# jamesfer/datafusion-parallelism

Measured on AMD Instinct MI355X. Metric: probe Mrows/s + build ms, 10^8-row int64 inner join; 1/2/4/8 GPUs, higher is better.
Workload: dtype int64; 1 GPU; C2: 10^8-probe x 10^7-build int64 inner equi-join, uniform keys; build_rows=10000000, probe_rows=100000000, matches=49999816, parallelism=single-gpu

## Files before the change

### datafusion-parallelism_amd/csrc/hj_api.cpp

```cpp
#include <hip/hip_runtime.h>
#include <math.h>
#include <stdint.h>
#include <stdio.h>
#include <stdlib.h>
#include <string.h>

#include <algorithm>
#include <atomic>
#include <chrono>
#include <condition_variable>
#include <deque>
#include <map>
#include <mutex>
#include <string>
#include <thread>
#include <tuple>
#include <unordered_map>
#include <vector>

#include "../../include/hj.h"
#include "hj_device.h"
#include "hj_host.h"
#include "hj_launch.h"

using namespace dfp;

struct MultiTable;

namespace {

thread_local std::string g_err;

hj_status fail(hj_status st, const std::string& msg) {
    g_err = msg;
    return st;
}

#define HIP_TRY(expr)                                                                    \
    do {                                                                                 \
        hipError_t e_ = (expr);                                                          \
        if (e_ != hipSuccess)                                                            \
            return fail(HJ_ERR_HIP, std::string(#expr ": ") + hipGetErrorString(e_));    \
    } while (0)

struct ThreadStreams {
    std::unordered_map<int, hipStream_t> m;
    ~ThreadStreams() {
        for (auto& kv : m) (void)hipStreamDestroy(kv.second);
    }
};
thread_local ThreadStreams g_streams;

hipStream_t thread_stream(int dev) {
    auto it = g_streams.m.find(dev);
    if (it != g_streams.m.end()) return it->second;
    hipStream_t s = nullptr;
    if (hipStreamCreateWithFlags(&s, hipStreamNonBlocking) != hipSuccess) return nullptr;
    g_streams.m[dev] = s;
    return s;
}

struct BuildResources {
    hipStream_t stream = nullptr;
    hipEvent_t ev0 = nullptr, ev1 = nullptr;
    hipEvent_t evp = nullptr;
    int64_t* h_minmax = nullptr;
    int64_t* d_mbox = nullptr;
    int64_t mb_seq = 0;
};
std::mutex g_pool_mu;
std::unordered_map<int, std::vector<BuildResources>> g_pool;

int ev_scope() {
    static const int v = [] {
        const char* e = getenv("DFP_HJ_EV_SCOPE");
        return e ? atoi(e) : 0;
    }();
    return v;
}
unsigned probe_ev_flags() { return hipEventDisableTiming | (ev_scope() >= 1 ? hipEventReleaseToDevice : 0u); }
unsigned build_ev_flags() { return ev_scope() >= 2 ? hipEventReleaseToDevice : hipEventDefault; }

bool acquire_resources(int dev, BuildResources* r) {
    {
        std::lock_guard<std::mutex> g(g_pool_mu);
        auto& v = g_pool[dev];
        if (!v.empty()) {
            *r = v.back();
            v.pop_back();
            return true;
        }
    }
    return hipStreamCreateWithFlags(&r->stream, hipStreamNonBlocking) == hipSuccess &&
           hipEventCreateWithFlags(&r->ev0, build_ev_flags()) == hipSuccess &&
           hipEventCreateWithFlags(&r->ev1, build_ev_flags()) == hipSuccess &&
           hipEventCreateWithFlags(&r->evp, probe_ev_flags()) == hipSuccess &&
           hipHostMalloc((void**)&r->h_minmax, 4 * sizeof(int64_t), hipHostMallocCoherent | hipHostMallocMapped) ==
               hipSuccess &&
           hipHostGetDevicePointer((void**)&r->d_mbox, r->h_minmax, 0) == hipSuccess;
}

void release_resources(int dev, const BuildResources& r) {
    std::lock_guard<std::mutex> g(g_pool_mu);
    g_pool[dev].push_back(r);
}

struct DevCache {
    std::mutex mu;
    std::map<uint64_t, std::vector<void*>> bins;
    std::unordered_map<void*, size_t> cls;
    size_t cached_bytes = 0;
};
DevCache g_cache;

size_t size_class(size_t bytes) {
    if (bytes <= 4096) return 4096;
    if (bytes <= (1u << 20)) {
        size_t c = 4096;
        while (c < bytes) c <<= 1;
        return c;
    }
    const size_t step = bytes <= (256u << 20) ? (2u << 20) : (32u << 20);
    return (bytes + step - 1) / step * step;
}

constexpr size_t kBestFitMin = size_t(64) << 20;

void* cache_alloc(int dev, size_t bytes, hipError_t* err) {
    const size_t c = size_class(bytes);
    const uint64_t key = ((uint64_t)dev << 48) | c;
    {
        std::lock_guard<std::mutex> g(g_cache.mu);
        auto it = g_cache.bins.find(key);
        if ((it == g_cache.bins.end() || it->second.empty()) && c >= kBestFitMin) {
            for (it = g_cache.bins.lower_bound(key);
                 it != g_cache.bins.end() && (it->first >> 48) == (uint64_t)dev &&
                 (it->first & ((1ull << 48) - 1)) <= c + c / 4;
                 ++it)
                if (!it->second.empty()) break;
            if (it != g_cache.bins.end() && ((it->first >> 48) != (uint64_t)dev ||
                                             (it->first & ((1ull << 48) - 1)) > c + c / 4))
                it = g_cache.bins.end();
        }
        if (it != g_cache.bins.end() && !it->second.empty()) {
            void* p = it->second.back();
            it->second.pop_back();
            const size_t bc = (size_t)(it->first & ((1ull << 48) - 1));
            g_cache.cached_bytes -= bc;
            g_cache.cls[p] = bc;
            *err = hipSuccess;
            return p;
        }
    }
    void* p = nullptr;
    static const bool alog = [] {
        const char* e = getenv("DFP_HJ_ALLOC_LOG");
        return e != nullptr && e[0] == '1';
    }();
    if (alog) fprintf(stderr, "[dfp alloc] miss dev %d bytes %zu class %zu cached %zu\n", dev, bytes, c, g_cache.cached_bytes);
    *err = hipMalloc(&p, c);
    if (*err != hipSuccess) {
        (void)hipGetLastError();
        std::lock_guard<std::mutex> g(g_cache.mu);
        if (alog) fprintf(stderr, "[dfp alloc] hipMalloc %zu failed with %zu cached bytes\n", c, g_cache.cached_bytes);
        for (auto it = g_cache.bins.lower_bound(key); it != g_cache.bins.end() && (it->first >> 48) == (uint64_t)dev;
             ++it) {
            if (it->second.empty()) continue;
            void* q = it->second.back();
            it->second.pop_back();
            (void)hipFree(q);
            g_cache.cached_bytes -= (size_t)(it->first & ((1ull << 48) - 1));
            *err = hipMalloc(&p, c);
            if (*err == hipSuccess) {
                if (alog) fprintf(stderr, "[dfp alloc] released one cached block of %zu bytes: ok\n",
                                  (size_t)(it->first & ((1ull << 48) - 1)));
                g_cache.cls[p] = c;
                return p;
            }
            (void)hipGetLastError();
            break;
        }
        size_t freed = 0;
        for (;;) {
            auto lo = g_cache.bins.lower_bound((uint64_t)dev << 48);
            auto hi = g_cache.bins.lower_bound((uint64_t)(dev + 1) << 48);
            auto big = g_cache.bins.end();
            for (auto it = hi; it != lo;) {
                --it;
                if (!it->second.empty()) {
                    big = it;
                    break;
                }
            }
            if (big == g_cache.bins.end()) break;
            void* q = big->second.back();
            big->second.pop_back();
            (void)hipFree(q);
            const size_t qc = (size_t)(big->first & ((1ull << 48) - 1));
            g_cache.cached_bytes -= qc;
            freed += qc;
            if (freed >= c) {
                *err = hipMalloc(&p, c);
                if (*err == hipSuccess) break;
                (void)hipGetLastError();
            }
        }
        if (*err != hipSuccess) *err = hipMalloc(&p, c);
        if (alog) fprintf(stderr, "[dfp alloc] released %zu bytes: %s\n", freed, *err == hipSuccess ? "ok" : "failed");
        if (*err == hipSuccess) {
            g_cache.cls[p] = c;
            return p;
        }
    }
    if (*err != hipSuccess) return nullptr;
    std::lock_guard<std::mutex> g(g_cache.mu);
    g_cache.cls[p] = c;
    return p;
}

void cache_free(int dev, void* p, size_t bytes) {
    if (p == nullptr) return;
    std::lock_guard<std::mutex> g(g_cache.mu);
    size_t c = size_class(bytes);
    auto it = g_cache.cls.find(p);
    if (it != g_cache.cls.end()) {
        c = it->second;
        g_cache.cls.erase(it);
    }
    g_cache.bins[((uint64_t)dev << 48) | c].push_back(p);
    g_cache.cached_bytes += c;
}

int device_count() {
    int n = 0;
    if (hipGetDeviceCount(&n) != hipSuccess) return 0;
    return n;
}

bool is_device_ptr(const void* p) {
    if (p == nullptr) return true;
    hipPointerAttribute_t a;
    if (hipPointerGetAttributes(&a, p) != hipSuccess) {
        (void)hipGetLastError();
        return false;
    }
    return a.type == hipMemoryTypeDevice || a.type == hipMemoryTypeManaged;
}

constexpr double kDefaultLoadFactor = 0.5;

std::atomic<int> g_build_mode{-1};
int build_mode_raw() {
    int m = g_build_mode.load(std::memory_order_relaxed);
    if (m < 0) {
        const char* e = getenv("DFP_HJ_DENSE");
        m = (e && e[0] == '0') ? 1 : 0;
        const char* f = getenv("DFP_HJ_FRAG_BUILD");
        if (m == 0 && f && f[0] == '0') m = 2;
        g_build_mode.store(m, std::memory_order_relaxed);
    }
    return m;
}
int build_mode() { return build_mode_raw() == 1 ? 1 : 0; }
bool frag_build_mode() { return build_mode_raw() == 0; }
std::atomic<int64_t> g_budget{-1};
int64_t device_budget() {
    int64_t b = g_budget.load(std::memory_order_relaxed);
    if (b < 0) {
        const char* e = getenv("DFP_HJ_DEVICE_BUDGET_BYTES");
        b = e ? std::max<int64_t>(0, atoll(e)) : 0;
        int64_t unset = -1;
        g_budget.compare_exchange_strong(unset, b, std::memory_order_relaxed);
        b = g_budget.load(std::memory_order_relaxed);
    }
    return b;
}
bool spec_build_on() {
    static const bool v = [] {
        const char* e = getenv("DFP_HJ_SPEC_BUILD");
        return !(e != nullptr && e[0] == '0');
    }();
    return v;
}
double load_factor() {
    const char* e = getenv("DFP_HJ_LOAD_FACTOR");
    double lf = e ? atof(e) : kDefaultLoadFactor;
    if (!(lf > 0.05 && lf <= 0.95)) lf = kDefaultLoadFactor;
    return lf;
}

struct HostSeg {
    const void* keys = nullptr;
    const uint8_t* valid = nullptr;
    int64_t voff = 0;
    const uint64_t* ids = nullptr;
    int64_t n = 0;
    std::vector<void*> owned;
    hipEvent_t ready = nullptr;
};

}

struct hj_table {
    int device = 0;
    int parallelism = 1;
    hj_key_type kt = HJ_INT64;
    int key_bytes = 8;

    std::mutex mu;
    std::condition_variable cv;
    std::vector<std::vector<HostSeg>> parts;
    std::vector<char> finished;
    int arrived = 0;
    bool built = false;
    bool sync_finish = false;
    mutable std::mutex probe_mu;
    mutable std::vector<std::pair<hipStream_t, hipEvent_t>> probe_evs;
    hj_status build_st = HJ_OK;
    std::string build_err;
    bool has_ids = false, has_no_ids = false;
    bool ids_u31 = true;

    std::vector<int64_t> part_off;
    int64_t total_rows = 0;

    Bucket* tbl = nullptr;
    uint32_t nb = 0, clog2 = 10, nchunks = 0;
    uint32_t* dup_rows = nullptr;
    BuildCounters* ctr = nullptr;
    bool wrapped = false;
    uint64_t* row_ids = nullptr;
    uint32_t* dense = nullptr;
    bool packed = false;
    int64_t dmin = 0;
    uint64_t drange = 0;
    bool has_range = false;
    bool force_dense = false;
    int64_t range_lo = 0, range_hi = 0;
    bool has_base = false;
    int64_t key_base = 0;
    BuildResources res;
    hipStream_t bstream = nullptr;
    hipStream_t app_stream = nullptr;
    int app_streams = 0;
    int64_t build_ns = 0;
    std::vector<std::pair<void*, size_t>> allocs;
    std::vector<std::pair<void*, size_t>> scratch;
    MultiTable* multi = nullptr;
    std::vector<std::tuple<int, void*, size_t>> multi_bufs;
    int64_t live_bytes = 0, peak_bytes = 0;
    std::vector<hj_table*> owned_tables;
    hipEvent_t ext_ev0 = nullptr;
    std::atomic<bool> spec_pending{false};
    std::mutex spec_mu;
    int64_t spec_seq = 0;
    uint32_t spec_cap = 0;
    const int64_t* spec_mm = nullptr;
    std::vector<Segment> spec_segs;
    bool mm_known = false;
    int64_t mm_lo = 0, mm_hi = 0;
};

namespace dfp {
namespace host {
hj_status set_error(hj_status st, const std::string& msg) { return fail(st, msg); }
void* dev_block(int dev, size_t bytes) {
    hipError_t e;
    return cache_alloc(dev, bytes ? bytes : 64, &e);
}
void free_block(int dev, void* p, size_t bytes) { cache_free(dev, p, bytes ? bytes : 64); }
void table_adopt_block(hj_table* t, int dev, void* p, size_t bytes) {
    t->multi_bufs.emplace_back(dev, p, bytes ? bytes : 64);
}
void table_adopt_table(hj_table* t, hj_table* other) { t->owned_tables.push_back(other); }
void table_set_start_event(hj_table* t, hipEvent_t ev) {
    if (t->ext_ev0) (void)hipEventDestroy(t->ext_ev0);
    t->ext_ev0 = ev;
    t->build_ns = -1;
}
}
}

namespace {

hipError_t wait_mailbox(int64_t* mm, int64_t seq, const int64_t* d_minmax, hipStream_t s) {
    for (uint32_t i = 1;; ++i) {
        if (__atomic_load_n(&mm[2], __ATOMIC_ACQUIRE) == seq) return hipSuccess;
        if ((i & 4095) == 0) {
            const hipError_t q = hipStreamQuery(s);
            if (q == hipErrorNotReady) continue;
            if (q != hipSuccess) return q;
            if (__atomic_load_n(&mm[2], __ATOMIC_ACQUIRE) == seq) return hipSuccess;
            return hipMemcpy(mm, d_minmax, 2 * sizeof(int64_t), hipMemcpyDeviceToHost);
        }
        __builtin_ia32_pause();
    }
}

hj_status dev_alloc(hj_table* t, std::vector<std::pair<void*, size_t>>& list, void** p, size_t bytes) {
    if (bytes == 0) bytes = 64;
    const int64_t budget = device_budget();
    if (budget > 0 && t->live_bytes + (int64_t)bytes > budget)
        return fail(HJ_ERR_OOM, "device budget: this build needs more than " + std::to_string(budget) +
                                    " bytes of one device (DFP_HJ_DEVICE_BUDGET_BYTES / hj_set_device_budget); "
                                    "shard it over several GPUs (hj_build_begin_multi, radix plan)");
    hipError_t e;
    *p = cache_alloc(t->device, bytes, &e);
    if (*p == nullptr) return fail(HJ_ERR_OOM, std::string("device allocation: ") + hipGetErrorString(e));
    list.emplace_back(*p, bytes);
    t->live_bytes += (int64_t)bytes;
    t->peak_bytes = std::max(t->peak_bytes, t->live_bytes);
    return HJ_OK;
}

void free_list(hj_table* t, std::vector<std::pair<void*, size_t>>& list) {
    for (auto& pb : list) {
        cache_free(t->device, pb.first, pb.second);
        t->live_bytes -= (int64_t)pb.second;
    }
    list.clear();
}

hipDeviceProp_t* device_props(int dev) {
    static std::mutex mu;
    static std::unordered_map<int, hipDeviceProp_t> cache;
    std::lock_guard<std::mutex> g(mu);
    auto it = cache.find(dev);
    if (it == cache.end()) {
        hipDeviceProp_t p;
        if (hipGetDeviceProperties(&p, dev) != hipSuccess) return nullptr;
        it = cache.emplace(dev, p).first;
    }
    return &it->second;
}

hj_status build_attempt(hj_table* t, const std::vector<Segment>& segs, double lf, bool* retry) {
    *retry = false;
    const int64_t total = t->total_rows;
    hj_status st;
    void* p;
    hipStream_t s = t->bstream;
    Segment* d_segs;
    BuildCounters* ctr;
    int64_t* d_minmax;
    if ((st = dev_alloc(t, t->scratch, &p, sizeof(Segment) * std::max<size_t>(segs.size(), 1))) != HJ_OK) return st;
    d_segs = (Segment*)p;
    if ((st = dev_alloc(t, t->allocs, &p, sizeof(BuildCounters))) != HJ_OK) return st;
    ctr = (BuildCounters*)p;
    t->ctr = ctr;
    if ((st = dev_alloc(t, t->scratch, &p, (2 + 2 * kMinmaxMaxBlocks) * sizeof(int64_t))) != HJ_OK) return st;
    d_minmax = (int64_t*)p;
    const bool need_range = total > 0 && build_mode() == 0 && !t->has_range;
    const bool minmax = need_range && !t->mm_known;
    const bool by_arg = minmax && segs.size() <= (size_t)kArgSegs;
    if (!by_arg) {
        if (!segs.empty())
            HIP_TRY(hipMemcpyAsync(d_segs, segs.data(), sizeof(Segment) * segs.size(), hipMemcpyHostToDevice, s));
        HIP_TRY(hipMemsetAsync(ctr, 0, sizeof(BuildCounters), s));
    }

    std::vector<int64_t> seg_n(segs.size());
    for (size_t i = 0; i < segs.size(); ++i) seg_n[i] = segs[i].n;
    const int64_t ftiles = frag_build_tiles(seg_n.data(), (int)segs.size());
    const bool packed_ok = (uint64_t)(2 * total + 2) < (1ull << 27);
    const uint32_t spec_cap =
        (uint32_t)std::min<uint64_t>(kMaxLevel1Bins, (kDenseFactor * (uint64_t)total + kDenseBlockValues - 1) /
                                                         kDenseBlockValues);
    const ChunkGeom spec_g{0, 0, spec_cap << kDenseBlockShift, kDenseShift, 0, 1, packed_ok ? 1 : 0};
    const bool spec = minmax && spec_build_on() && !t->has_base && !t->force_dense && t->multi == nullptr &&
                      device_budget() <= 0 && frag_build_mode() && spec_cap > 0 && frag_build_ok(spec_g, ftiles);
    ChunkGeom g{};
    bool dense = false;
    if (need_range || (t->has_range && total > 0 && (build_mode() == 0 || t->force_dense))) {
        int64_t mm[2] = {t->range_lo, t->range_hi};
        if (t->mm_known) {
            mm[0] = t->mm_lo;
            mm[1] = t->mm_hi;
        }
        if (minmax) {
            int64_t* mb = t->res.h_minmax;
            const int64_t seq = ++t->res.mb_seq;
            HIP_TRY(launch_key_minmax(t->key_bytes, segs.data(), d_segs, (int)segs.size(), by_arg ? ctr : nullptr,
                                      total, d_minmax, t->res.d_mbox, seq, s));
            if (spec) {
                t->spec_seq = seq;
                t->spec_cap = spec_cap;
                t->spec_mm = d_minmax;
                t->spec_segs = segs;
                mm[0] = 1;
                mm[1] = 0;
            } else {
                HIP_TRY(wait_mailbox(mb, seq, d_minmax, s));
                mm[0] = mb[0];
                mm[1] = mb[1];
            }
        }
        if (spec) {
            dense = true;
            g = spec_g;
            t->dmin = 0;
            t->drange = 0;
        } else if (mm[0] <= mm[1]) {
            const uint64_t range = (uint64_t)mm[1] - (uint64_t)mm[0] + 1;
            const uint64_t nch = (range + (1u << kDenseShift) - 1) >> kDenseShift;
            if (range != 0 && (range <= kDenseFactor * (uint64_t)total || t->force_dense) &&
                nch <= (uint64_t)kMaxChunks) {
                dense = true;
                g = ChunkGeom{0, 0, (uint32_t)nch, kDenseShift, mm[0], 1, packed_ok ? 1 : 0};
                t->dmin = mm[0];
                t->drange = range;
            }
        }
    }
    if (!dense && t->has_base && total > 0)
        return fail(HJ_ERR_INVALID, "hj_build_key_base: the build keys do not make a direct-addressed table "
                                    "(key range > 8 x rows); build from int64 keys instead");
    if (!dense) {
        const double want = (double)total / (kSlots * lf);
        uint32_t clog2 = 9;
        uint64_t nchunks = (uint64_t)(want / (1u << clog2)) + 1;
        while (nchunks > (uint64_t)kMaxChunks && clog2 < 11) {
            ++clog2;
            nchunks = (uint64_t)(want / (1u << clog2)) + 1;
        }
        if (nchunks > (uint64_t)kMaxChunks) {
            const double full = (double)kMaxChunks * (1u << clog2) * kSlots;
            if ((double)total / full > 0.8)
                return fail(HJ_ERR_INVALID, "build side too large for one device table; shard it (hj_radix_partition)");
            nchunks = kMaxChunks;
        }
        g = ChunkGeom{(uint32_t)(nchunks << clog2), clog2, (uint32_t)nchunks, 0, 0, 0, 0};
        t->dmin = 0;
        t->drange = 0;
    }
    t->clog2 = g.clog2;
    t->nchunks = g.nchunks;
    t->packed = g.packed != 0;
    t->nb = g.nb;
    const uint64_t nchunks = g.nchunks;
    const bool frag = dense && total > 0 && frag_build_mode() && frag_build_ok(g, ftiles);
    const int64_t hftiles = frag_build_tiles(seg_n.data(), (int)segs.size(), hashed_build_tile_log());
    const bool hfrag = !dense && total > 0 && build_mode_raw() != 2 && hashed_frag_ok(g, hftiles);
    hipDeviceProp_t* prop0 = device_props(t->device);
    const int64_t ntiles = build_tiles(total, prop0 ? prop0->multiProcessorCount : 256);
    const int64_t tile_rows = build_tile_rows(total, ntiles);
    const int64_t hlen = (int64_t)(nchunks + 1) * ntiles;

    t->tbl = nullptr;
    t->dense = nullptr;
    if (dense) {
        const uint64_t dchunks = dense_one_level((uint32_t)nchunks)
                                     ? (uint64_t)dense_blocks((uint32_t)nchunks) << kDenseBlockShift
                                     : nchunks;
        if ((st = dev_alloc(t, t->allocs, &p, sizeof(uint32_t) * (size_t)(dchunks << kDenseShift))) != HJ_OK)
            return st;
        t->dense = (uint32_t*)p;
    } else {
        if ((st = dev_alloc(t, t->allocs, &p, (size_t)(t->nb + 1) * sizeof(Bucket))) != HJ_OK) return st;
        t->tbl = (Bucket*)p;
    }
    if ((st = dev_alloc(t, t->allocs, &p, sizeof(uint32_t) * (size_t)(2 * total + 2))) != HJ_OK) return st;
    t->dup_rows = (uint32_t*)p;
    const bool ids_as_rows = t->has_ids && t->ids_u31;
    if (t->has_ids && !ids_as_rows) {
        if ((st = dev_alloc(t, t->allocs, &p, sizeof(uint64_t) * (size_t)std::max<int64_t>(total, 1))) != HJ_OK)
            return st;
        t->row_ids = (uint64_t*)p;
    }
    if (frag || hfrag) {
        void* fscr;
        uint32_t* d_tb;
        uint64_t* ids32 = nullptr;
        BigSeg* fbig;
        const int64_t fbytes =
            frag ? frag_build_scratch_bytes(g, ftiles, total) : hashed_frag_scratch_bytes(g, hftiles, total);
        if ((st = dev_alloc(t, t->scratch, &fscr, (size_t)fbytes)) != HJ_OK) return st;
        if ((st = dev_alloc(t, t->scratch, &p, sizeof(uint32_t) * (size_t)(frag ? ftiles : hftiles))) != HJ_OK)
            return st;
        d_tb = (uint32_t*)p;
        if ((st = dev_alloc(t, t->scratch, &p, sizeof(BigSeg) * (size_t)(total / (kSmallSeg + 1) + 2))) != HJ_OK)
            return st;
        fbig = (BigSeg*)p;
        if (t->has_ids) {
            uint64_t* dst = t->row_ids;
            if (ids_as_rows && segs.size() == 1) {
                ids32 = const_cast<uint64_t*>(segs[0].ids);
                dst = nullptr;
            } else if (ids_as_rows) {
                if ((st = dev_alloc(t, t->scratch, &p, sizeof(uint64_t) * (size_t)total)) != HJ_OK) return st;
                dst = ids32 = (uint64_t*)p;
            }
            if (dst != nullptr)
                for (const Segment& sg : segs)
                    HIP_TRY(hipMemcpyAsync(dst + sg.row_base, sg.ids, sizeof(uint64_t) * (size_t)sg.n,
                                           hipMemcpyDefault, s));
        }
        hipDeviceProp_t* prop = device_props(t->device);
        const int cus = prop ? prop->multiProcessorCount : 256;
        if (frag) {
            HIP_TRY(launch_build_frag(t->key_bytes, segs.data(), (int)segs.size(), g, ftiles, fscr, d_tb, ids32,
                                      t->dense, t->dup_rows, fbig, ctr, d_segs, total, ids_as_rows, cus,
                                      spec ? SpecGeo{(const long long*)d_minmax, (uint64_t)total, spec_cap}
                                           : SpecGeo{nullptr, 0, 0},
                                      s));
            if (spec) t->spec_pending.store(true, std::memory_order_release);
            return HJ_OK;
        }
        HIP_TRY(launch_build_hashed_frag(t->key_bytes, segs.data(), (int)segs.size(), g, hftiles, fscr, d_tb, ids32,
                                         t->tbl, t->dup_rows, fbig, ctr, d_segs, total, ids_as_rows, cus, s));
        BuildCounters hc;
        HIP_TRY(hipMemcpyAsync(&hc, ctr, sizeof(hc), hipMemcpyDeviceToHost, s));
        HIP_TRY(hipStreamSynchronize(s));
        free_list(t, t->scratch);
        if (hc.err & ~3ull)
            return fail(HJ_ERR_HIP, "hashed build: internal check failed (error bits " + std::to_string(hc.err) + ")");
        if (hc.err) {
            *retry = true;
            free_list(t, t->allocs);
            t->row_ids = nullptr;
        }
        return HJ_OK;
    }
    uint32_t *hist, *hist1, *srows, *trows;
    unsigned long long *skeys, *tkeys;
    BigSeg* big;
    void* scan;
    if ((st = dev_alloc(t, t->scratch, &p, sizeof(uint32_t) * (size_t)std::max<int64_t>(hlen, 1))) != HJ_OK) return st;
    hist = (uint32_t*)p;
    if ((st = dev_alloc(t, t->scratch, &p, sizeof(uint32_t) * (size_t)std::max<int64_t>(kMaxLevel1Bins * ntiles, 1))) !=
        HJ_OK)
        return st;
    hist1 = (uint32_t*)p;
    uint32_t* chunk_starts;
    if ((st = dev_alloc(t, t->scratch, &p, sizeof(uint32_t) * (size_t)(nchunks + 2))) != HJ_OK) return st;
    chunk_starts = (uint32_t*)p;
    if ((st = dev_alloc(t, t->scratch, &p, (size_t)scan_scratch_bytes(std::max<int64_t>(hlen, kMaxLevel1Bins * ntiles)))) !=
        HJ_OK)
        return st;
    scan = p;
    if ((st = dev_alloc(t, t->scratch, &p, 8 * (size_t)std::max<int64_t>(total, 1))) != HJ_OK) return st;
    skeys = (unsigned long long*)p;
    if ((st = dev_alloc(t, t->scratch, &p, 4 * (size_t)std::max<int64_t>(total, 1))) != HJ_OK) return st;
    srows = (uint32_t*)p;
    if ((st = dev_alloc(t, t->scratch, &p, 8 * (size_t)std::max<int64_t>(total, 1))) != HJ_OK) return st;
    tkeys = (unsigned long long*)p;
    if ((st = dev_alloc(t, t->scratch, &p, 4 * (size_t)std::max<int64_t>(total, 1))) != HJ_OK) return st;
    trows = (uint32_t*)p;
    if ((st = dev_alloc(t, t->scratch, &p, sizeof(BigSeg) * (size_t)(total / (kSmallSeg + 1) + 2))) != HJ_OK)
        return st;
    big = (BigSeg*)p;

    if (total == 0) HIP_TRY(hipMemsetAsync(t->tbl, 0, (size_t)(t->nb + 1) * sizeof(Bucket), s));
    hipDeviceProp_t* prop = device_props(t->device);
    const int cus = prop ? prop->multiProcessorCount : 256;
    HIP_TRY(launch_build(t->key_bytes, d_segs, (int)segs.size(), total, g, hist, hist1, chunk_starts, ntiles, tile_rows,
                         scan, tkeys, trows, skeys, srows, t->row_ids, ids_as_rows, t->tbl, t->dense, t->dup_rows, big,
                         ctr, cus, s));
    if (dense) return HJ_OK;
    BuildCounters hc;
    HIP_TRY(hipMemcpyAsync(&hc, ctr, sizeof(hc), hipMemcpyDeviceToHost, s));
    HIP_TRY(hipStreamSynchronize(s));
    free_list(t, t->scratch);
    if (hc.err) {
        *retry = true;
        free_list(t, t->allocs);
        t->row_ids = nullptr;
    }
    return HJ_OK;
}

hj_status run_multi_build_entry(hj_table* t, const std::vector<Segment>& segs, const std::vector<HostSeg*>& hsegs);

hj_status build_attempts(hj_table* t, const std::vector<Segment>& segs) {
    double lf = load_factor();
    for (int attempt = 0;; ++attempt) {
        bool retry = false;
        hj_status st = build_attempt(t, segs, lf, &retry);
        if (st != HJ_OK) return st;
        if (!retry) return HJ_OK;
        if (attempt >= 4) return fail(HJ_ERR_INVALID, "build: a table chunk overflowed at every load factor");
        lf *= 0.5;
        HIP_TRY(hipEventRecord(t->res.ev0, t->bstream));
    }
}

hj_status ensure_geometry(const hj_table* ct) {
    hj_table* t = const_cast<hj_table*>(ct);
    auto settled = [t]() { return t->build_st == HJ_OK ? HJ_OK : fail(t->build_st, t->build_err); };
    if (!t->spec_pending.load(std::memory_order_acquire)) return settled();
    std::lock_guard<std::mutex> g(t->spec_mu);
    if (!t->spec_pending.load(std::memory_order_relaxed)) return settled();
    HIP_TRY(hipSetDevice(t->device));
    int64_t* mb = t->res.h_minmax;
    HIP_TRY(wait_mailbox(mb, t->spec_seq, t->spec_mm, t->bstream));
    const int64_t mn = mb[0], mx = mb[1];
    if (spec_dense_blocks(mn, mx, (uint64_t)t->total_rows, t->spec_cap) != 0) {
        const uint64_t range = (uint64_t)mx - (uint64_t)mn + 1;
        t->dmin = mn;
        t->drange = range;
        t->nchunks = (uint32_t)((range + (1u << kDenseShift) - 1) >> kDenseShift);
        t->spec_pending.store(false, std::memory_order_release);
        return HJ_OK;
    }
    HIP_TRY(hipStreamSynchronize(t->bstream));
    HIP_TRY(hipEventRecord(t->res.ev0, t->bstream));
    free_list(t, t->allocs);
    free_list(t, t->scratch);
    t->dense = nullptr;
    t->tbl = nullptr;
    t->dup_rows = nullptr;
    t->row_ids = nullptr;
    t->ctr = nullptr;
    t->mm_known = true;
    t->mm_lo = mn;
    t->mm_hi = mx;
    hj_status st = build_attempts(t, t->spec_segs);
    if (st == HJ_OK && hipEventRecord(t->res.ev1, t->bstream) != hipSuccess)
        st = fail(HJ_ERR_HIP, "hipEventRecord failed");
    t->build_ns = -1;
    if (st != HJ_OK) {
        (void)hipStreamSynchronize(t->bstream);
        t->build_st = st;
        t->build_err = g_err;
    }
    t->spec_pending.store(false, std::memory_order_release);
    return st;
}

struct Settler {
    std::mutex mu;
    std::condition_variable cv;
    std::deque<hj_table*> q;
    hj_table* busy = nullptr;
};
Settler& settler() {
    static Settler* s = [] {
        Settler* st = new Settler();
        std::thread([st] {
            for (;;) {
                hj_table* t;
                {
                    std::unique_lock<std::mutex> g(st->mu);
                    st->cv.wait(g, [st] { return !st->q.empty(); });
                    t = st->q.front();
                    st->q.pop_front();
                    st->busy = t;
                }
                (void)ensure_geometry(t);
                {
                    std::lock_guard<std::mutex> g(st->mu);
                    st->busy = nullptr;
                }
                st->cv.notify_all();
            }
        }).detach();
        return st;
    }();
    return *s;
}
bool settler_on() {
    static const bool v = [] {
        const char* e = getenv("DFP_HJ_SETTLE");
        return !(e && e[0] == '0');
    }();
    return v;
}
void settler_enqueue(hj_table* t) {
    Settler& st = settler();
    {
        std::lock_guard<std::mutex> g(st.mu);
        st.q.push_back(t);
    }
    st.cv.notify_all();
}
void settler_forget(hj_table* t) {
    if (!settler_on()) return;
    Settler& st = settler();
    std::unique_lock<std::mutex> g(st.mu);
    for (auto it = st.q.begin(); it != st.q.end();)
        it = *it == t ? st.q.erase(it) : it + 1;
    st.cv.wait(g, [&st, t] { return st.busy != t; });
}

hj_status run_build(hj_table* t) {
    HIP_TRY(hipSetDevice(t->device));
    std::vector<Segment> segs;
    std::vector<HostSeg*> hsegs;
    t->part_off.assign(t->parallelism, 0);
    int64_t row = 0;
    for (int p = 0; p < t->parallelism; ++p) {
        t->part_off[p] = row;
        for (auto& hs : t->parts[p]) {
            if (hs.n == 0) continue;
            segs.push_back(Segment{hs.keys, hs.valid, hs.voff, hs.ids, hs.n, row});
            hsegs.push_back(&hs);
            row += hs.n;
        }
    }
    t->total_rows = row;
    if (t->multi) return run_multi_build_entry(t, segs, hsegs);
    if (row > 0x7FFFFFF0ll) return fail(HJ_ERR_INVALID, "build side exceeds 2^31-16 rows on one device; shard it");
    if (t->has_ids && t->has_no_ids)
        return fail(HJ_ERR_INVALID, "explicit build ids must be given for every batch or none");
    t->bstream = t->app_streams == 1 ? t->app_stream : t->res.stream;
    hipStream_t s = t->bstream;
    for (int p = 0; p < t->parallelism; ++p)
        for (auto& hs : t->parts[p])
            if (hs.ready) HIP_TRY(hipStreamWaitEvent(s, hs.ready, 0));
    HIP_TRY(hipEventRecord(t->res.ev0, s));
    hj_status bst = build_attempts(t, segs);
    if (bst != HJ_OK) return bst;
    HIP_TRY(hipEventRecord(t->res.ev1, s));
    t->build_ns = -1;
    if (t->has_base) {
        if (t->dense != nullptr) t->dmin += t->key_base;
        t->kt = HJ_INT64;
        t->key_bytes = 8;
    }
    return HJ_OK;
}

int64_t build_time_ns(hj_table* t) {
    if (t->build_ns < 0) {
        float ms = 0;
        if (hipEventSynchronize(t->res.ev1) != hipSuccess ||
            hipEventElapsedTime(&ms, t->ext_ev0 ? t->ext_ev0 : t->res.ev0, t->res.ev1) != hipSuccess)
            return -1;
        t->build_ns = (int64_t)(ms * 1e6);
    }
    return t->build_ns;
}

hj_status wait_built(const hj_table* t, hipStream_t s) {
    if (s != t->bstream) HIP_TRY(hipStreamWaitEvent(s, t->res.ev1, 0));
    return HJ_OK;
}

hj_status check_table(const hj_table* t) {
    if (t == nullptr) return fail(HJ_ERR_INVALID, "null table");
    if (!t->built) return fail(HJ_ERR_INVALID, "table is not built: every partition must call hj_build_finish");
    if (t->build_st != HJ_OK) return fail(t->build_st, t->build_err);
    return ensure_geometry(t);
}

TableView view_of(const hj_table* t) {
    return TableView{t->tbl, t->dup_rows, t->row_ids, t->nb, t->clog2, t->dense, t->dmin, t->drange,
                     t->packed ? kPackedMask : kFullMask};
}

struct TmpInput {
    void* keys = nullptr;
    uint8_t* valid = nullptr;
    hipStream_t s = nullptr;
    ~TmpInput() {
        if (keys) (void)hipFreeAsync(keys, s);
        if (valid) (void)hipFreeAsync(valid, s);
    }
};

hj_status stage_input(int key_bytes, const void* keys, const uint8_t* valid, int64_t voff, int64_t n, uint32_t flags,
                      hipStream_t s, TmpInput& tmp, const void** dkeys, const uint8_t** dvalid, int64_t* dvoff) {
    if (flags & HJ_INPUT_DEVICE) {
        if (!is_device_ptr(keys) || !is_device_ptr(valid))
            return fail(HJ_ERR_INVALID, "HJ_INPUT_DEVICE given but a pointer is not device memory");
        *dkeys = keys;
        *dvalid = valid;
        *dvoff = voff;
        return HJ_OK;
    }
    tmp.s = s;
    if (n > 0) {
        HIP_TRY(hipMallocAsync(&tmp.keys, (size_t)n * key_bytes, s));
        HIP_TRY(hipMemcpyAsync(tmp.keys, keys, (size_t)n * key_bytes, hipMemcpyDefault, s));
    }
    *dkeys = tmp.keys;
    *dvalid = nullptr;
    *dvoff = 0;
    if (valid && n > 0) {
        const int64_t b0 = voff >> 3;
        const int64_t nbytes = ((voff & 7) + n + 7) >> 3;
        HIP_TRY(hipMallocAsync((void**)&tmp.valid, (size_t)nbytes, s));
        HIP_TRY(hipMemcpyAsync(tmp.valid, valid + b0, (size_t)nbytes, hipMemcpyDefault, s));
        *dvalid = tmp.valid;
        *dvoff = voff & 7;
    }
    return HJ_OK;
}

hj_status note_probe(const hj_table* t, hipStream_t s) {
    std::lock_guard<std::mutex> g(t->probe_mu);
    for (auto& se : t->probe_evs)
        if (se.first == s) {
            HIP_TRY(hipEventRecord(se.second, s));
            return HJ_OK;
        }
    hipEvent_t ev = t->res.evp;
    if (!t->probe_evs.empty()) HIP_TRY(hipEventCreateWithFlags(&ev, probe_ev_flags()));
    t->probe_evs.emplace_back(s, ev);
    HIP_TRY(hipEventRecord(ev, s));
    return HJ_OK;
}

hj_status check_probe_args(int64_t n, uint32_t pbase, int64_t cap, const void* ws) {
    if (n < 0 || n > 0xFFFFFFFFll) return fail(HJ_ERR_INVALID, "probe batch must have < 2^32 rows");
    if ((int64_t)pbase + n > 0x100000000ll) return fail(HJ_ERR_INVALID, "probe_base + rows exceeds 2^32");
    if (cap < 0) return fail(HJ_ERR_INVALID, "negative capacity");
    if (reinterpret_cast<uintptr_t>(ws) & 7) return fail(HJ_ERR_INVALID, "workspace must be 8-byte aligned");
    return HJ_OK;
}

hj_status probe_impl(const hj_table* t, const void* keys, const uint8_t* valid, int64_t voff,
                     const uint32_t* probe_ids, uint32_t pbase, int64_t n, uint64_t* out_b, uint32_t* out_p,
                     int64_t cap, int64_t* d_total, void* ws, hipStream_t s) {
    hj_status st = check_probe_args(n, pbase, cap, ws);
    if (st == HJ_OK) st = ensure_geometry(t);
    if (st != HJ_OK) return st;
    HIP_TRY(launch_probe(t->key_bytes, view_of(t), keys, valid, voff, probe_ids, pbase, n, out_b, out_p, cap, d_total, ws,
                         s != t->bstream ? t->res.ev1 : nullptr, s));
    return note_probe(t, s);
}

}

struct MultiTable {
    int plan = HJ_MULTI_AUTO;
    std::vector<int> devices;
    std::vector<hj_table*> shards;
    std::vector<hipStream_t> streams;
    std::mutex probe_mu;
    int64_t total_rows = 0;
    ~MultiTable() {
        for (size_t g = 0; g < shards.size(); ++g) hj_table_free(shards[g]);
        for (size_t g = 0; g < streams.size(); ++g) {
            (void)hipSetDevice(devices[g]);
            (void)hipStreamDestroy(streams[g]);
        }
    }
};

namespace {

int ptr_device(const void* p, int dflt) {
    hipPointerAttribute_t a;
    if (p == nullptr || hipPointerGetAttributes(&a, p) != hipSuccess) {
        (void)hipGetLastError();
        return dflt;
    }
    return (a.type == hipMemoryTypeDevice || a.type == hipMemoryTypeManaged) ? a.device : dflt;
}

void drain_multi(const MultiTable* m);
struct TmpBufs {
    std::vector<std::tuple<int, void*, size_t>> v;
    const MultiTable* m = nullptr;
    std::vector<std::pair<int, hipStream_t>> streams;
    ~TmpBufs() {
        if (m != nullptr) drain_multi(m);
        for (auto& ds : streams) {
            (void)hipSetDevice(ds.first);
            (void)hipStreamSynchronize(ds.second);
        }
        for (auto& b : v) cache_free(std::get<0>(b), std::get<1>(b), std::get<2>(b));
    }
    void* get(int dev, size_t bytes) {
        hipError_t e;
        (void)hipSetDevice(dev);
        void* p = cache_alloc(dev, bytes ? bytes : 64, &e);
        if (p) v.emplace_back(dev, p, bytes ? bytes : 64);
        return p;
    }
};

#define MT_ALLOC(var, type, dev, bytes)                                                   \
    type var = (type)tmp.get((dev), (bytes));                                             \
    if (var == nullptr) return fail(HJ_ERR_OOM, "multi-GPU table: device allocation failed")

hj_status sync_streams(const MultiTable* m) {
    for (size_t g = 0; g < m->streams.size(); ++g) {
        HIP_TRY(hipSetDevice(m->devices[g]));
        HIP_TRY(hipStreamSynchronize(m->streams[g]));
    }
    return HJ_OK;
}

void drain_multi(const MultiTable* m) {
    for (size_t g = 0; g < m->streams.size(); ++g) {
        (void)hipSetDevice(m->devices[g]);
        (void)hipStreamSynchronize(m->streams[g]);
    }
    for (const hj_table* sh : m->shards)
        if (sh != nullptr && sh->built && sh->build_st == HJ_OK) {
            (void)hipSetDevice(sh->device);
            (void)hipEventSynchronize(sh->res.ev1);
        }
}

bool force_stage() {
    const char* e = getenv("DFP_HJ_MULTI_STAGE");
    return e != nullptr && e[0] == '1';
}

int owner_of(int64_t key, int G) { return (int)(mix64((uint64_t)key) & (uint64_t)(G - 1)); }
// ... 257 lines not shown
            if (!P.ws) P.ws = tmp.get(dev, (size_t)hj_probe_workspace_bytes(P.n));
            if (!P.ob || !P.op || !P.dt || !P.ws) return fail(HJ_ERR_OOM, "multi-GPU probe: device allocation failed");
            st = P.ids ? hj_probe_async_ids(m->shards[g], P.k, P.v, P.voff, P.ids, P.n, P.ob, P.op, P.cap, P.dt, P.ws,
                                            m->streams[g])
                       : hj_probe_async_base(m->shards[g], P.k, P.v, P.voff, P.n, P.base, P.ob, P.op, P.cap, P.dt,
                                             P.ws, m->streams[g]);
            if (st != HJ_OK) return st;
            HIP_TRY(hipMemcpyAsync(&P.total, P.dt, 8, hipMemcpyDeviceToHost, m->streams[g]));
            again = true;
        }
        if (!again) break;
        if ((st = sync_streams(m)) != HJ_OK) return st;
    }
    int64_t total = 0;
    unsigned long long err = 0;
    for (auto& P : parts) {
        total += P.total;
        unsigned long long e = 0;
        HIP_TRY(hipMemcpy(&e, (char*)P.ws + 8, 8, hipMemcpyDeviceToHost));
        err |= e;
    }
    HIP_TRY(hipSetDevice(d));
    if (workspace) HIP_TRY(hipMemcpyAsync((char*)workspace + 8, &err, 8, hipMemcpyHostToDevice, s));
    if (m->plan == HJ_MULTI_BROADCAST) {
        int64_t at = 0;
        for (auto& P : parts) {
            const int64_t c = std::min<int64_t>(P.total, std::max<int64_t>(cap - at, 0));
            HIP_TRY(copy_to(out_b + at, P.ob, 8 * (size_t)c, s));
            HIP_TRY(copy_to(out_p + at, P.op, 4 * (size_t)c, s));
            at += P.total;
        }
    } else if (total > 0) {
        MT_ALLOC(cb, uint64_t*, d, 8 * (size_t)total);
        MT_ALLOC(cp, uint32_t*, d, 4 * (size_t)total);
        int64_t at = 0;
        for (auto& P : parts) {
            HIP_TRY(copy_to(cb + at, P.ob, 8 * (size_t)P.total, s));
            HIP_TRY(copy_to(cp + at, P.op, 4 * (size_t)P.total, s));
            at += P.total;
        }
        MT_ALLOC(mw, void*, d, (size_t)merge_pairs_workspace(n));
        HIP_TRY(launch_merge_pairs(cb, cp, total, n, out_b, out_p, cap, mw, s));
        if (probe_ids)
            HIP_TRY(launch_gather_fixed(probe_ids, nullptr, 0, 4, out_p, 4, std::min(total, cap), out_p, nullptr, s));
        else if (pbase)
            HIP_TRY(launch_add_u32(out_p, std::min(total, cap), pbase, s));
    }
    HIP_TRY(hipMemcpyAsync(d_total, &total, 8, hipMemcpyHostToDevice, s));
    HIP_TRY(hipStreamSynchronize(s));
    return HJ_OK;
}

}

namespace {
hj_status run_multi_build_entry(hj_table* t, const std::vector<Segment>& segs, const std::vector<HostSeg*>& hsegs) {
    return run_multi_build(t, segs, hsegs);
}
}

extern "C" {

const char* hj_last_error(void) { return g_err.c_str(); }

const char* hj_version(void) { return "dfp-hj 0.2 (gfx950)"; }

int hj_device_count(void) { return device_count(); }

hj_status hj_build_begin(int device, int parallelism, hj_key_type key_type, int64_t expected_rows, hj_table** out) {
    (void)expected_rows;
    if (out == nullptr) return fail(HJ_ERR_INVALID, "null out");
    *out = nullptr;
    if (parallelism < 1) return fail(HJ_ERR_INVALID, "parallelism must be >= 1");
    if (key_type != HJ_INT32 && key_type != HJ_INT64) return fail(HJ_ERR_INVALID, "unsupported key type");
    const int nd = device_count();
    if (nd == 0) return fail(HJ_ERR_NO_DEVICE, "no GPU visible: the HIP path cannot run (no CPU fallback)");
    if (device < 0 || device >= nd) return fail(HJ_ERR_INVALID, "bad device ordinal");
    HIP_TRY(hipSetDevice(device));
    hj_table* t = new hj_table();
    t->device = device;
    t->parallelism = parallelism;
    t->kt = key_type;
    t->key_bytes = key_type == HJ_INT64 ? 8 : 4;
    t->parts.resize(parallelism);
    t->finished.assign(parallelism, 0);
    if (!acquire_resources(device, &t->res)) {
        delete t;
        return fail(HJ_ERR_HIP, "stream/event creation failed");
    }
    static std::once_flag pool_once[64];
    if (device < 64)
        std::call_once(pool_once[device], [device] {
            hipMemPool_t pool;
            if (hipDeviceGetDefaultMemPool(&pool, device) == hipSuccess) {
                uint64_t thr = UINT64_MAX;
                (void)hipMemPoolSetAttribute(pool, hipMemPoolAttrReleaseThreshold, &thr);
            }
        });
    *out = t;
    return HJ_OK;
}

hj_status hj_build_begin_multi(int ngpu, const int* devices, int parallelism, hj_key_type key_type,
                               int64_t expected_rows, int plan, hj_table** out) {
    if (out == nullptr) return fail(HJ_ERR_INVALID, "null out");
    *out = nullptr;
    if (ngpu < 1 || ngpu > 64 || devices == nullptr) return fail(HJ_ERR_INVALID, "ngpu must be 1..64 with a device list");
    if (plan != HJ_MULTI_AUTO && plan != HJ_MULTI_BROADCAST && plan != HJ_MULTI_RADIX)
        return fail(HJ_ERR_INVALID, "unknown multi-GPU plan");
    if (plan == HJ_MULTI_RADIX && (ngpu & (ngpu - 1)))
        return fail(HJ_ERR_INVALID, "the radix plan shards over a power-of-two number of GPUs");
    const int nd = device_count();
    if (nd == 0) return fail(HJ_ERR_NO_DEVICE, "no GPU visible: the HIP path cannot run (no CPU fallback)");
    for (int g = 0; g < ngpu; ++g)
        if (devices[g] < 0 || devices[g] >= nd) return fail(HJ_ERR_INVALID, "bad device ordinal");
    hj_status st = hj_build_begin(devices[0], parallelism, key_type, expected_rows, out);
    if (st != HJ_OK) return st;
    hj_table* t = *out;
    MultiTable* m = new MultiTable();
    m->plan = plan;
    m->devices.assign(devices, devices + ngpu);
    for (int g = 0; g < ngpu; ++g) {
        hipStream_t s = nullptr;
        if (hipSetDevice(devices[g]) != hipSuccess || hipStreamCreateWithFlags(&s, hipStreamNonBlocking) != hipSuccess) {
            delete m;
            hj_table_free(t);
            *out = nullptr;
            return fail(HJ_ERR_HIP, "multi-GPU table: stream creation failed");
        }
        m->streams.push_back(s);
        for (int q = 0; q < ngpu; ++q)
            if (devices[q] != devices[g]) {
                (void)hipDeviceEnablePeerAccess(devices[q], 0);
                (void)hipGetLastError();
            }
    }
    (void)hipSetDevice(devices[0]);
    t->multi = m;
    return HJ_OK;
}

hj_status hj_build_append(hj_table* t, int partition, const void* keys, const uint8_t* validity,
                          int64_t validity_offset, const uint64_t* ids, int64_t n, uint32_t flags, void* stream) {
    if (t == nullptr) return fail(HJ_ERR_INVALID, "null table");
    if (partition < 0 || partition >= t->parallelism) return fail(HJ_ERR_INVALID, "bad partition");
    if (n < 0 || validity_offset < 0) return fail(HJ_ERR_INVALID, "negative length/offset");
    if (n > 0 && keys == nullptr) return fail(HJ_ERR_INVALID, "null keys");
    {
        std::lock_guard<std::mutex> g(t->mu);
        if (t->finished[partition])
            return fail(HJ_ERR_INVALID, "State already consumed for partition " + std::to_string(partition));
        if (n > 0) {
            if (ids) {
                t->has_ids = true;
                if (!(flags & HJ_IDS_U31)) t->ids_u31 = false;
            } else {
                t->has_no_ids = true;
            }
        }
    }
    HIP_TRY(hipSetDevice(t->device));
    HostSeg hs;
    hs.n = n;
    if (n == 0) return HJ_OK;
    {
        std::lock_guard<std::mutex> g(t->mu);
        if (t->app_streams == 0) {
            t->app_stream = (hipStream_t)stream;
            t->app_streams = 1;
        } else if (t->app_stream != (hipStream_t)stream) {
            t->app_streams = 2;
        }
    }
    hipStream_t s = (hipStream_t)stream;
    const bool dev_in = (flags & HJ_INPUT_DEVICE) != 0;
    if (dev_in && (!is_device_ptr(keys) || !is_device_ptr(validity) || !is_device_ptr(ids)))
        return fail(HJ_ERR_INVALID, "HJ_INPUT_DEVICE given but a pointer is not device memory");
    if (dev_in && (flags & HJ_BORROW)) {
        if (!(flags & HJ_BORROW_KEEP)) {
            std::lock_guard<std::mutex> g(t->mu);
            t->sync_finish = true;
        }
        HIP_TRY(hipEventCreateWithFlags(&hs.ready, hipEventDisableTiming));
        HIP_TRY(hipEventRecord(hs.ready, s));
        hs.keys = keys;
        hs.valid = validity;
        hs.voff = validity_offset;
        hs.ids = ids;
    } else {
        const int64_t staged = n * t->key_bytes + (validity ? (((validity_offset & 7) + n + 7) >> 3) : 0) +
                               (ids ? n * 8 : 0);
        {
            std::lock_guard<std::mutex> g(t->mu);
            const int64_t budget = device_budget();
            if (budget > 0 && t->live_bytes + staged > budget)
                return fail(HJ_ERR_OOM, "device budget: staging this build input exceeds " + std::to_string(budget) +
                                            " bytes of one device (DFP_HJ_DEVICE_BUDGET_BYTES); shard the build");
            t->live_bytes += staged;
            t->peak_bytes = std::max(t->peak_bytes, t->live_bytes);
        }
        void* dk = nullptr;
        HIP_TRY(hipMalloc(&dk, (size_t)n * t->key_bytes));
        hs.owned.push_back(dk);
        HIP_TRY(hipMemcpyAsync(dk, keys, (size_t)n * t->key_bytes, hipMemcpyDefault, s));
        hs.keys = dk;
        if (validity) {
            const int64_t b0 = validity_offset >> 3;
            const int64_t nbytes = ((validity_offset & 7) + n + 7) >> 3;
            void* dv = nullptr;
            HIP_TRY(hipMalloc(&dv, (size_t)nbytes));
            hs.owned.push_back(dv);
            HIP_TRY(hipMemcpyAsync(dv, validity + b0, (size_t)nbytes, hipMemcpyDefault, s));
            hs.valid = (const uint8_t*)dv;
            hs.voff = validity_offset & 7;
        }
        if (ids) {
            void* di = nullptr;
            HIP_TRY(hipMalloc(&di, (size_t)n * 8));
            hs.owned.push_back(di);
            HIP_TRY(hipMemcpyAsync(di, ids, (size_t)n * 8, hipMemcpyDefault, s));
            hs.ids = (const uint64_t*)di;
        }
        HIP_TRY(hipStreamSynchronize(s));
    }
    std::lock_guard<std::mutex> g(t->mu);
    t->parts[partition].push_back(std::move(hs));
    return HJ_OK;
}

hj_status hj_build_finish(hj_table* t, int partition) {
    if (t == nullptr) return fail(HJ_ERR_INVALID, "null table");
    if (partition < 0 || partition >= t->parallelism) return fail(HJ_ERR_INVALID, "bad partition");
    std::unique_lock<std::mutex> g(t->mu);
    if (t->finished[partition])
        return fail(HJ_ERR_INVALID, "State already consumed for partition " + std::to_string(partition));
    t->finished[partition] = 1;
    t->arrived++;
    if (t->arrived == t->parallelism) {
        hj_status st = run_build(t);
        if (st == HJ_OK && t->sync_finish) st = ensure_geometry(t);
        if (st != HJ_OK) (void)hipStreamSynchronize(t->bstream);
        if (st == HJ_OK && t->sync_finish && hipEventSynchronize(t->res.ev1) != hipSuccess)
            st = fail(HJ_ERR_HIP, "build failed on the device");
        t->build_st = st;
        t->build_err = st == HJ_OK ? "" : g_err;
        t->built = true;
        t->cv.notify_all();
        if (st == HJ_OK && t->spec_pending.load(std::memory_order_acquire) && settler_on()) settler_enqueue(t);
    } else {
        const char* e = getenv("DFP_HJ_BARRIER_TIMEOUT_S");
        const double secs = e ? atof(e) : 300.0;
        if (!t->cv.wait_for(g, std::chrono::duration<double>(secs), [t] { return t->built; }))
            return fail(HJ_ERR_INVALID, "Possible deadlock: partition " + std::to_string(partition) +
                                            " waited for the build barrier; every partition must call "
                                            "hj_build_finish concurrently");
    }
    if (t->build_st != HJ_OK) return fail(t->build_st, t->build_err);
    return HJ_OK;
}

hj_status hj_build_key_range(hj_table* t, int64_t key_lo, int64_t key_hi) {
    if (t == nullptr) return fail(HJ_ERR_INVALID, "null table");
    if (key_lo > key_hi) return fail(HJ_ERR_INVALID, "hj_build_key_range: key_lo > key_hi");
    if (t->key_bytes == 4 && (key_lo < INT32_MIN || key_hi > INT32_MAX))
        return fail(HJ_ERR_INVALID, "hj_build_key_range: outside the int32 key domain");
    std::lock_guard<std::mutex> g(t->mu);
    if (t->built || t->arrived > 0) return fail(HJ_ERR_INVALID, "hj_build_key_range: after the barrier started");
    t->has_range = true;
    t->range_lo = key_lo;
    t->range_hi = key_hi;
    return HJ_OK;
}

hj_status hj_build_dense(hj_table* t) {
    if (t == nullptr) return fail(HJ_ERR_INVALID, "null table");
    if (t->multi != nullptr) return fail(HJ_ERR_INVALID, "hj_build_dense: not for a multi-GPU table");
    std::lock_guard<std::mutex> g(t->mu);
    if (t->built || t->arrived > 0) return fail(HJ_ERR_INVALID, "hj_build_dense: after the barrier started");
    if (!t->has_range) return fail(HJ_ERR_INVALID, "hj_build_dense: needs hj_build_key_range first");
    if ((uint64_t)t->range_hi - (uint64_t)t->range_lo >= ((uint64_t)kMaxChunks << kDenseShift))
        return fail(HJ_ERR_INVALID, "hj_build_dense: key range beyond the direct-addressed layout");
    t->force_dense = true;
    return HJ_OK;
}

hj_status hj_build_key_base(hj_table* t, int64_t key_base) {
    if (t == nullptr) return fail(HJ_ERR_INVALID, "null table");
    if (t->multi != nullptr) return fail(HJ_ERR_INVALID, "hj_build_key_base: not for a multi-GPU table");
    if (t->kt != HJ_INT32) return fail(HJ_ERR_INVALID, "hj_build_key_base: the build keys must be int32 offsets");
    std::lock_guard<std::mutex> g(t->mu);
    if (t->built || t->arrived > 0) return fail(HJ_ERR_INVALID, "hj_build_key_base: after the barrier started");
    t->has_base = true;
    t->key_base = key_base;
    return HJ_OK;
}

hj_status hj_table_dense_piece(const hj_table* t, uint32_t** refs, uint64_t* nvalues, int64_t* key_min,
                               uint32_t** dup_rows, const uint64_t** dup_used, int* packed) {
    hj_status st = check_table(t);
    if (st != HJ_OK) return st;
    if (!refs || !nvalues || !key_min || !dup_rows || !dup_used || !packed) return fail(HJ_ERR_INVALID, "null out");
    if (t->multi != nullptr || t->dense == nullptr || t->ctr == nullptr || t->wrapped)
        return fail(HJ_ERR_INVALID, "hj_table_dense_piece: not a built direct-addressed single-device table");
    *refs = t->dense;
    *nvalues = t->drange;
    *key_min = t->dmin;
    *dup_rows = t->dup_rows;
    *dup_used = reinterpret_cast<const uint64_t*>(&t->ctr->dup_used);
    *packed = t->packed ? 1 : 0;
    return HJ_OK;
}

hj_status hj_table_dense_export(const hj_table* t, uint32_t* refs_dst, uint64_t v0, uint64_t n, uint32_t* dup_dst,
                                uint64_t dup_n, uint64_t* dup_used_dst, void* stream) {
    hj_status st = check_table(t);
    if (st != HJ_OK) return st;
    if (t->multi != nullptr || t->dense == nullptr || t->ctr == nullptr || t->wrapped)
        return fail(HJ_ERR_INVALID, "hj_table_dense_export: not a built direct-addressed single-device table");
    if (refs_dst != nullptr && (v0 > t->drange || n > t->drange - v0))
        return fail(HJ_ERR_INVALID, "hj_table_dense_export: refs range past the table's key range");
    if (dup_dst != nullptr && dup_n > (uint64_t)(2 * t->total_rows + 2))
        return fail(HJ_ERR_INVALID, "hj_table_dense_export: more segment words than the table holds");
    HIP_TRY(hipSetDevice(t->device));
    hipStream_t s = (hipStream_t)stream;
    if (s != t->bstream) HIP_TRY(hipStreamWaitEvent(s, t->res.ev1, 0));
    if (refs_dst != nullptr && n > 0)
        HIP_TRY(hipMemcpyAsync(refs_dst, t->dense + v0, n * sizeof(uint32_t), hipMemcpyDeviceToDevice, s));
    if (dup_dst != nullptr && dup_n > 0)
        HIP_TRY(hipMemcpyAsync(dup_dst, t->dup_rows, dup_n * sizeof(uint32_t), hipMemcpyDeviceToDevice, s));
    if (dup_used_dst != nullptr)
        HIP_TRY(hipMemcpyAsync(dup_used_dst, &t->ctr->dup_used, sizeof(uint64_t), hipMemcpyDeviceToDevice, s));
    return note_probe(t, s);
}

hj_status hj_table_wrap_dense(int device, hj_key_type probe_key_type, int64_t key_min, uint64_t nvalues,
                              const uint32_t* refs, const uint32_t* dup_rows, int packed, void* stream,
                              hj_table** out) {
    if (out == nullptr) return fail(HJ_ERR_INVALID, "null out");
    *out = nullptr;
    if (probe_key_type != HJ_INT32 && probe_key_type != HJ_INT64) return fail(HJ_ERR_INVALID, "unsupported key type");
    if (refs == nullptr || dup_rows == nullptr || nvalues == 0)
        return fail(HJ_ERR_INVALID, "hj_table_wrap_dense: null arrays or an empty key range");
    if (nvalues > ((uint64_t)kMaxChunks << kDenseShift))
        return fail(HJ_ERR_INVALID, "hj_table_wrap_dense: key range beyond the direct-addressed layout");
    const int nd = device_count();
    if (nd == 0) return fail(HJ_ERR_NO_DEVICE, "no GPU visible: the HIP path cannot run (no CPU fallback)");
    if (device < 0 || device >= nd) return fail(HJ_ERR_INVALID, "bad device ordinal");
    HIP_TRY(hipSetDevice(device));
    hj_table* t = new hj_table();
    t->device = device;
    t->kt = probe_key_type;
    t->key_bytes = probe_key_type == HJ_INT64 ? 8 : 4;
    t->parts.resize(1);
    t->finished.assign(1, 1);
    t->arrived = 1;
    if (!acquire_resources(device, &t->res)) {
        delete t;
        return fail(HJ_ERR_HIP, "stream/event creation failed");
    }
    t->wrapped = true;
    t->dense = const_cast<uint32_t*>(refs);
    t->dup_rows = const_cast<uint32_t*>(dup_rows);
    t->dmin = key_min;
    t->drange = nvalues;
    t->packed = packed != 0;
    t->bstream = (hipStream_t)stream;
    if (hipEventRecord(t->res.ev0, t->bstream) != hipSuccess || hipEventRecord(t->res.ev1, t->bstream) != hipSuccess) {
        release_resources(device, t->res);
        delete t;
        return fail(HJ_ERR_HIP, "hipEventRecord failed");
    }
    t->built = true;
    *out = t;
    return HJ_OK;
}

hj_status hj_dense_rebase_dups(uint32_t* refs, uint64_t n, uint32_t base, int packed, void* stream) {
    if (n > 0 && refs == nullptr) return fail(HJ_ERR_INVALID, "null refs");
    if (device_count() == 0) return fail(HJ_ERR_NO_DEVICE, "no GPU visible");
    const uint32_t mask = packed ? kPackedMask : kFullMask;
    if (base > mask) return fail(HJ_ERR_INVALID, "hj_dense_rebase_dups: base beyond the offset field");
    HIP_TRY(launch_dense_rebase(refs, n, base, mask, (hipStream_t)stream));
    return HJ_OK;
}

hj_status hj_build_partition_offset(const hj_table* t, int partition, int64_t* out) {
    hj_status st = check_table(t);
    if (st != HJ_OK) return st;
    if (partition < 0 || partition >= t->parallelism || out == nullptr) return fail(HJ_ERR_INVALID, "bad args");
    *out = t->part_off[partition];
    return HJ_OK;
}

hj_status hj_table_stats_get(const hj_table* t, hj_table_stats* out) {
    hj_status st = check_table(t);
    if (st != HJ_OK) return st;
    if (out == nullptr) return fail(HJ_ERR_INVALID, "null out");
    if (t->multi) {
        const MultiTable* m = t->multi;
        memset(out, 0, sizeof(*out));
        for (size_t g = 0; g < m->shards.size(); ++g) {
            hj_table_stats s;
            if ((st = hj_table_stats_get(m->shards[g], &s)) != HJ_OK) return st;
            if (m->plan == HJ_MULTI_BROADCAST && g > 0) {
                out->build_ns = std::max(out->build_ns, s.build_ns);
                continue;
            }
            out->inserted_rows += s.inserted_rows;
            out->distinct_keys += s.distinct_keys;
            out->dup_keys += s.dup_keys;
            out->dup_rows += s.dup_rows;
            out->max_key_rows = std::max(out->max_key_rows, s.max_key_rows);
            out->buckets += s.buckets;
            out->table_bytes += s.table_bytes;
            out->build_ns = std::max(out->build_ns, s.build_ns);
        }
        out->build_rows = t->total_rows;
        return HJ_OK;
    }
    HIP_TRY(hipSetDevice(t->device));
    hipStream_t s = thread_stream(t->device);
    unsigned long long* d = nullptr;
    HIP_TRY(hipMallocAsync((void**)&d, 4 * sizeof(unsigned long long), s));
    HIP_TRY(hipMemsetAsync(d, 0, 4 * sizeof(unsigned long long), s));
    if (wait_built(t, s) != HJ_OK) return HJ_ERR_HIP;
    HIP_TRY(launch_table_stats(view_of(t), d, s));
    unsigned long long h[4];
    HIP_TRY(hipMemcpyAsync(h, d, sizeof(h), hipMemcpyDeviceToHost, s));
    HIP_TRY(hipFreeAsync(d, s));
    HIP_TRY(hipStreamSynchronize(s));
    out->build_rows = t->total_rows;
    out->distinct_keys = (int64_t)h[0];
    out->dup_keys = (int64_t)h[1];
    out->dup_rows = (int64_t)h[2];
    out->max_key_rows = (int64_t)h[3];
    out->inserted_rows = (int64_t)h[0] - (int64_t)h[1] + (int64_t)h[2];
    out->buckets = t->dense ? 0 : t->nb;
    out->table_bytes = t->dense ? (int64_t)sizeof(uint32_t) * ((int64_t)t->nchunks << kDenseShift)
                                : (int64_t)(t->nb + 1) * (int64_t)sizeof(Bucket);
    out->build_ns = build_time_ns(const_cast<hj_table*>(t));
    return HJ_OK;
}

int64_t hj_table_build_ns(const hj_table* t) {
    if (t == nullptr || !t->built || t->build_st != HJ_OK) return -1;
    if (t->multi == nullptr && ensure_geometry(t) != HJ_OK) return -1;
    if (t->multi) {
        int64_t ns = 0;
        for (hj_table* sh : t->multi->shards) ns = std::max(ns, hj_table_build_ns(sh));
        return ns;
    }
    return build_time_ns(const_cast<hj_table*>(t));
}

int64_t hj_probe_workspace_bytes(int64_t n) { return probe_workspace(n); }

int hj_set_build_mode(int mode) {
    if (mode < 0 || mode > 2) return -1;
    const int old = build_mode_raw();
    g_build_mode.store(mode, std::memory_order_relaxed);
    return old;
}

int64_t hj_set_device_budget(int64_t bytes) {
    const int64_t old = device_budget();
    g_budget.store(bytes < 0 ? 0 : bytes, std::memory_order_relaxed);
    return old;
}

hj_status hj_table_device_bytes(const hj_table* t, int64_t* peak_per_device) {
    if (t == nullptr || peak_per_device == nullptr) return fail(HJ_ERR_INVALID, "null table/out");
    if (t->multi) {
        int64_t mx = 0;
        for (const hj_table* sh : t->multi->shards)
            if (sh != nullptr) mx = std::max(mx, sh->peak_bytes);
        *peak_per_device = mx;
        return HJ_OK;
    }
    *peak_per_device = t->peak_bytes;
    return HJ_OK;
}

int hj_set_probe_mode(int mode) {
    if (mode != 0 && mode != 3 && mode != 4) return -1;
    const int old = get_probe_mode();
    set_probe_mode(mode);
    return old;
}

int hj_set_probe_tile_log(int tile_log) {
    if (tile_log != 0 && tile_log != 14 && tile_log != 15) return -1;
    return set_probe_tile_log(tile_log);
}

hj_status hj_probe_async(const hj_table* t, const void* keys, const uint8_t* validity, int64_t validity_offset,
                         int64_t n, uint64_t* out_build, uint32_t* out_probe, int64_t capacity, int64_t* d_total,
                         void* workspace, void* stream) {
    hj_status st = check_table(t);
    if (st != HJ_OK) return st;
    if (d_total == nullptr || workspace == nullptr) return fail(HJ_ERR_INVALID, "null d_total/workspace");
    if (n > 0 && keys == nullptr) return fail(HJ_ERR_INVALID, "null keys");
    HIP_TRY(hipSetDevice(t->device));
    if (t->multi)
        return multi_probe(t, keys, validity, validity_offset, nullptr, 0, n, out_build, out_probe, capacity, d_total,
                           workspace, (hipStream_t)stream);
    return probe_impl(t, keys, validity, validity_offset, nullptr, 0, n, out_build, out_probe, capacity, d_total,
                      workspace, (hipStream_t)stream );
}

hj_status hj_probe_async_base(const hj_table* t, const void* keys, const uint8_t* validity, int64_t validity_offset,
                              int64_t n, uint32_t probe_base, uint64_t* out_build, uint32_t* out_probe,
                              int64_t capacity, int64_t* d_total, void* workspace, void* stream) {
    hj_status st = check_table(t);
    if (st != HJ_OK) return st;
    if (d_total == nullptr || workspace == nullptr) return fail(HJ_ERR_INVALID, "null d_total/workspace");
    if (n > 0 && keys == nullptr) return fail(HJ_ERR_INVALID, "null keys");
    HIP_TRY(hipSetDevice(t->device));
    if (t->multi)
        return multi_probe(t, keys, validity, validity_offset, nullptr, probe_base, n, out_build, out_probe, capacity,
                           d_total, workspace, (hipStream_t)stream);
    return probe_impl(t, keys, validity, validity_offset, nullptr, probe_base, n, out_build, out_probe, capacity,
                      d_total, workspace, (hipStream_t)stream);
}

hj_status hj_probe_async_ids(const hj_table* t, const void* keys, const uint8_t* validity, int64_t validity_offset,
                             const uint32_t* probe_ids, int64_t n, uint64_t* out_build, uint32_t* out_probe,
                             int64_t capacity, int64_t* d_total, void* workspace, void* stream) {
    hj_status st = check_table(t);
    if (st != HJ_OK) return st;
    if (d_total == nullptr || workspace == nullptr) return fail(HJ_ERR_INVALID, "null d_total/workspace");
    HIP_TRY(hipSetDevice(t->device));
    if (t->multi)
        return multi_probe(t, keys, validity, validity_offset, probe_ids, 0, n, out_build, out_probe, capacity,
                           d_total, workspace, (hipStream_t)stream);
    return probe_impl(t, keys, validity, validity_offset, probe_ids, 0, n, out_build, out_probe, capacity, d_total,
                      workspace, (hipStream_t)stream );
}


namespace {
uint64_t match_claim_bits(const hj_table* t) {
    return t->dense != nullptr ? t->drange : ((uint64_t)(2 * t->total_rows + 2) >> 3) + 1;
}
const char* const kMatchMulti = "the match probe is not defined for a multi-GPU table (probe its pairs instead)";
}

int64_t hj_probe_match_workspace_bytes(const hj_table* t, int64_t n) {
    if (check_table(t) != HJ_OK) return -1;
    if (t->multi) {
        (void)fail(HJ_ERR_INVALID, kMatchMulti);
        return -1;
    }
    if (check_probe_args(n, 0, 0, nullptr) != HJ_OK) return -1;
    return probe_match_workspace(match_claim_bits(t));
}

hj_status hj_probe_match(const hj_table* t, const void* keys, const uint8_t* validity, int64_t validity_offset,
                         int64_t n, uint8_t* out_bitmap, uint32_t* out_counts, uint8_t* build_flags, int64_t nflags,
                         int64_t* d_stats, void* workspace, void* stream) {
    hj_status st = check_table(t);
    if (st != HJ_OK) return st;
    if (t->multi) return fail(HJ_ERR_INVALID, kMatchMulti);
    if (workspace == nullptr) return fail(HJ_ERR_INVALID, "null workspace");
    if ((st = check_probe_args(n, 0, 0, workspace)) != HJ_OK) return st;
    if (n > 0 && keys == nullptr) return fail(HJ_ERR_INVALID, "null keys");
    if (nflags < 0 || (nflags > 0 && build_flags == nullptr)) return fail(HJ_ERR_INVALID, "bad build_flags / nflags");
    if (reinterpret_cast<uintptr_t>(out_bitmap) & 7) return fail(HJ_ERR_INVALID, "out_bitmap must be 8-byte aligned");
    if ((reinterpret_cast<uintptr_t>(out_counts) & 3) || (reinterpret_cast<uintptr_t>(d_stats) & 7))
        return fail(HJ_ERR_INVALID, "out_counts must be 4-byte and d_stats 8-byte aligned");
    HIP_TRY(hipSetDevice(t->device));
    hipStream_t s = (hipStream_t)stream;
    if ((st = wait_built(t, s)) != HJ_OK) return st;
    HIP_TRY(launch_probe_match(t->key_bytes, view_of(t), keys, validity, validity_offset, n, out_bitmap, out_counts,
                               build_flags, nflags, d_stats, workspace, match_claim_bits(t), s));
    return note_probe(t, s);
}

hj_status hj_probe(const hj_table* t, const void* keys, const uint8_t* validity, int64_t validity_offset, int64_t n,
                   uint32_t flags, void* stream, hj_pairs* out) {
    hj_status st = check_table(t);
    if (st != HJ_OK) return st;
    if (out == nullptr) return fail(HJ_ERR_INVALID, "null out");
    memset(out, 0, sizeof(*out));
    if (n < 0) return fail(HJ_ERR_INVALID, "negative length");
    if (n > 0 && keys == nullptr) return fail(HJ_ERR_INVALID, "null keys");
    HIP_TRY(hipSetDevice(t->device));
    hipStream_t s = (hipStream_t)stream;
    TmpInput tmp;
    const void* dk;
    const uint8_t* dv;
    int64_t dvo;
    if ((st = stage_input(t->key_bytes, keys, validity, validity_offset, n, flags, s, tmp, &dk, &dv, &dvo)) != HJ_OK)
        return st;
    void* ws = nullptr;
    int64_t* d_total = nullptr;
    HIP_TRY(hipMallocAsync(&ws, (size_t)hj_probe_workspace_bytes(n), s));
    HIP_TRY(hipMallocAsync((void**)&d_total, sizeof(int64_t), s));
    int64_t cap = std::max<int64_t>(n, 1);
    uint64_t* ob = nullptr;
    uint32_t* op = nullptr;
    int64_t total = 0;
    for (int attempt = 0; attempt < 2; ++attempt) {
        HIP_TRY(hipMalloc((void**)&ob, (size_t)cap * 8));
        HIP_TRY(hipMalloc((void**)&op, (size_t)cap * 4));
        if (t->multi) st = multi_probe(t, dk, dv, dvo, nullptr, 0, n, ob, op, cap, d_total, ws, s);
        else st = probe_impl(t, dk, dv, dvo, nullptr, 0, n, ob, op, cap, d_total, ws, s);
        if (st != HJ_OK) break;
        uint64_t werr = 0;
        HIP_TRY(hipMemcpyAsync(&total, d_total, 8, hipMemcpyDeviceToHost, s));
        HIP_TRY(hipMemcpyAsync(&werr, (char*)ws + 8, 8, hipMemcpyDeviceToHost, s));
        HIP_TRY(hipStreamSynchronize(s));
        if (werr != 0) {
            st = fail(HJ_ERR_HIP, "probe: tile look-back gave up (results invalid)");
            break;
        }
        if (total <= cap) break;
        (void)hipFree(ob);
        (void)hipFree(op);
        ob = nullptr;
        op = nullptr;
        cap = total;
    }
    (void)hipFreeAsync(ws, s);
    (void)hipFreeAsync(d_total, s);
    if (st != HJ_OK) {
        if (ob) (void)hipFree(ob);
        if (op) (void)hipFree(op);
        (void)hipStreamSynchronize(s);
        return st;
    }
// ... 630 lines not shown
```

### datafusion-parallelism_amd/csrc/hj_device.h

```cpp
#pragma once
#include <stdint.h>

namespace dfp {

constexpr uint64_t kSign = 0x8000000000000000ull;
constexpr int kSlots = 5;
constexpr unsigned kDupFlag = 0x80000000u;
constexpr unsigned kMiss = 0xFFFFFFFFu;
constexpr int kSmallSeg = 16;
constexpr unsigned kInlineCount = 63;
constexpr unsigned kCountUnknown = 0xFFFFFFFFu;

struct alignas(64) Bucket {
    unsigned long long key[kSlots];
    unsigned int ref[kSlots];
    unsigned int meta;
};
static_assert(sizeof(Bucket) == 64, "bucket must be one 64-byte line");

struct Segment {
    const void* keys;
    const uint8_t* valid;
    int64_t voff;
    const uint64_t* ids;
    int64_t n;
    int64_t row_base;
};

struct BuildCounters {
    unsigned long long n_valid;
    unsigned long long dup_used;
    unsigned long long n_big;
    unsigned long long err;
    unsigned long long spill_used;
};

struct BigSeg {
    unsigned long long key;
    unsigned int off;
    unsigned int pad;
};

__host__ __device__ inline uint64_t mix64(uint64_t k) {
    k ^= k >> 33;
    k *= 0xff51afd7ed558ccdull;
    k ^= k >> 33;
    k *= 0xc4ceb9fe1a85ec53ull;
    k ^= k >> 33;
    return k;
}

__host__ __device__ constexpr uint64_t inv_odd(uint64_t a) {
    uint64_t x = a;
    for (int i = 0; i < 5; ++i) x *= 2 - a * x;
    return x;
}
__host__ __device__ inline uint64_t unmix64(uint64_t k) {
    k ^= k >> 33;
    k *= inv_odd(0xc4ceb9fe1a85ec53ull);
    k ^= k >> 33;
    k *= inv_odd(0xff51afd7ed558ccdull);
    k ^= k >> 33;
    return k;
}
static_assert(inv_odd(0xff51afd7ed558ccdull) * 0xff51afd7ed558ccdull == 1, "inverse multiplier");

__host__ __device__ inline unsigned long long stored_key(int64_t key) { return mix64((uint64_t)key); }

__host__ __device__ inline uint32_t bucket_of(uint64_t h, uint32_t nbuckets) {
    return (uint32_t)(((h >> 32) * (uint64_t)nbuckets) >> 32);
}

struct TableView {
    const struct Bucket* tbl;
    const uint32_t* dup_rows;
    const uint64_t* row_ids;
    uint32_t nb;
    uint32_t clog2;
    const uint32_t* dense;
    int64_t dmin;
    uint64_t drange;
    uint32_t off_mask;
};
constexpr uint32_t kFullMask = 0x7FFFFFFFu;
constexpr uint32_t kPackedMask = 0x07FFFFFFu;

constexpr uint32_t kRunMaxRows = 9;
__host__ __device__ inline bool run_ref(uint32_t r, uint32_t off_mask) {
    return off_mask == kPackedMask && (r >> 27) == 0x11u;
}
__host__ __device__ inline uint32_t run_ref_count(uint32_t r) { return ((r >> 24) & 7u) + 2u; }
__host__ __device__ inline uint32_t make_run_ref(uint32_t top, uint32_t c) {
    return kDupFlag | (1u << 27) | ((c - 2u) << 24) | top;
}
__host__ __device__ inline uint32_t ref_count_inline(uint32_t r, uint32_t off_mask) {
    const uint32_t c4 = off_mask == kPackedMask ? ((r >> 27) & 15u) : 0u;
    const uint32_t run = 0u - (uint32_t)(c4 == 1u);
    const uint32_t dup = (run_ref_count(r) & run) | ((c4 != 0u ? c4 : kCountUnknown) & ~run);
    const uint32_t c = (r & kDupFlag) ? dup : 1u;
    return r == kMiss ? 0u : c;
}
__host__ __device__ inline uint32_t dup_ref_row(const uint32_t* dup_rows, uint32_t r, uint32_t off_mask, uint32_t j) {
    return run_ref(r, off_mask) ? (r & 0xFFFFFFu) - j : dup_rows[(r & off_mask) + 1 + j];
}

constexpr uint32_t kDenseShift = 11;
struct ChunkGeom {
    uint32_t nb, clog2, nchunks, dshift;
    int64_t dmin;
    int dense;
    int packed;
};

constexpr uint64_t kDenseFactor = 8;
constexpr uint64_t kDenseBlockValues = 8192;

struct SpecGeo {
    const long long* mm;
    uint64_t rows;
    uint32_t cap;
};
__host__ __device__ inline uint32_t spec_dense_blocks(int64_t mn, int64_t mx, uint64_t rows, uint32_t cap) {
    if (mn > mx) return 0u;
    const uint64_t range = (uint64_t)mx - (uint64_t)mn + 1;
    if (range == 0 || range > kDenseFactor * rows) return 0u;
    const uint64_t nblk = (range + kDenseBlockValues - 1) / kDenseBlockValues;
    return nblk <= cap ? (uint32_t)nblk : 0u;
}

}
```

### datafusion-parallelism_amd/csrc/hj_kernels.hip

```cpp
#include <hip/hip_runtime.h>
#include <stdint.h>
#include <stdlib.h>

#include <algorithm>
#include <atomic>
#include <climits>
#include <type_traits>

#include "hj_device.h"
#include "hj_launch.h"
#include "hj_util.h"

namespace dfp {

template <typename K>
__device__ __forceinline__ int64_t ld_key(const void* keys, int64_t i) {
    return (int64_t)(reinterpret_cast<const K*>(keys)[i]);
}

__device__ __forceinline__ int64_t seg_key(const Segment& sg, int64_t i, int key_bytes) {
    return key_bytes == 8 ? ld_key<int64_t>(sg.keys, i) : ld_key<int32_t>(sg.keys, i);
}

__device__ __forceinline__ int find_seg(const Segment* segs, int nseg, int64_t r) {
// ... 870 lines not shown
        int64_t k[4];
        load4<K, NT>(keys, row0, n, vec, k);
        uint32_t r[4];
#pragma unroll
        for (int q = 0; q < 4; ++q) {
            const bool in = (row0 + q < n) && (!HAS_VALID || bit_valid(valid, voff, row0 + q));
            const uint64_t idx = (uint64_t)k[q] - (uint64_t)tv.dmin;
            r[q] = (in && idx < tv.drange) ? tv.dense[idx] : kMiss;
        }
#pragma unroll
        for (int q = 0; q < 4; ++q) {
            ref[q] = r[q];
            cnt[q] = ref_count_inline(r[q], tv.off_mask);
        }
        return;
    }
    const Bucket* __restrict__ tbl = tv.tbl;
    const uint32_t cmask = (1u << tv.clog2) - 1;
    int64_t k[4];
    load4<K, NT>(keys, row0, n, vec, k);
    bool in[4];
    unsigned long long sk[4];
    uint32_t b[4];
    uint4 L0[4], L1[4], L2[4], L3[4];
#pragma unroll
    for (int q = 0; q < 4; ++q) {
        in[q] = (row0 + q < n) && (!HAS_VALID || bit_valid(valid, voff, row0 + q));
        sk[q] = stored_key(k[q]);
        b[q] = (in[q] && sk[q] != 0) ? stored_bucket(sk[q], tv.nb) : tv.nb;
    }
#pragma unroll
    for (int q = 0; q < 4; ++q) {
        const uint4* p = reinterpret_cast<const uint4*>(tbl + b[q]);
        L0[q] = p[0]; L1[q] = p[1]; L2[q] = p[2]; L3[q] = p[3];
    }
    bool more[4];
#pragma unroll
    for (int q = 0; q < 4; ++q) {
        ref[q] = scan_line(L0[q], L1[q], L2[q], L3[q], sk[q], &more[q], &cnt[q]);
        if (sk[q] == 0) {
            ref[q] = L3[q].w ? L2[q].z : kMiss;
            cnt[q] = L3[q].w;
            more[q] = false;
        }
        if (!in[q]) { ref[q] = kMiss; cnt[q] = 0; more[q] = false; }
    }
#pragma unroll
    for (int q = 0; q < 4; ++q) {
        uint32_t bb = b[q];
        for (uint32_t probes = 0; more[q] && probes < cmask; ++probes) {
            bb = (bb & ~cmask) | ((bb + 1) & cmask);
            const uint4* p = reinterpret_cast<const uint4*>(tbl + bb);
            ref[q] = scan_line(p[0], p[1], p[2], p[3], sk[q], &more[q], &cnt[q]);
        }
    }
}

__device__ __forceinline__ uint32_t resolve_count(const uint32_t* dup_rows, uint32_t ref, uint32_t cnt,
                                                  uint32_t off_mask) {
    return cnt == kCountUnknown ? dup_rows[ref & off_mask] : cnt;
}

template <bool HAS_ROW_IDS, bool HAS_PROBE_IDS>
__device__ __forceinline__ void emit4(const TableView& tv, const uint32_t* __restrict__ probe_ids, uint32_t pbase,
                                      int64_t row0,
                                      const uint32_t (&ref)[4], const uint32_t (&cnt)[4], unsigned long long pos,
                                      uint64_t* __restrict__ out_b, uint32_t* __restrict__ out_p, int64_t cap) {
#pragma unroll
    for (int q = 0; q < 4; ++q) {
        const uint32_t c = cnt[q];
        if (c == 0) continue;
        const int64_t prow = row0 + q;
        const uint32_t pidx = HAS_PROBE_IDS ? probe_ids[prow] : (uint32_t)prow + pbase;
        const uint32_t r = ref[q];
        if (c == 1) {
            if (pos < (unsigned long long)cap) {
                const uint32_t br = (r & kDupFlag) ? dup_ref_row(tv.dup_rows, r, tv.off_mask, 0) : r;
                out_b[pos] = HAS_ROW_IDS ? tv.row_ids[br] : (uint64_t)br;
                out_p[pos] = pidx;
            }
        } else {
            for (uint32_t t = 0; t < c; ++t) {
                if (pos + t < (unsigned long long)cap) {
                    const uint32_t br = dup_ref_row(tv.dup_rows, r, tv.off_mask, t);
                    out_b[pos + t] = HAS_ROW_IDS ? tv.row_ids[br] : (uint64_t)br;
                    out_p[pos + t] = pidx;
                }
            }
        }
        pos += c;
    }
}

constexpr unsigned long long kFlagAgg = 1ull << 62;
constexpr unsigned long long kFlagIncl = 2ull << 62;
constexpr unsigned long long kFlagVal = (1ull << 62) - 1;
constexpr unsigned kLookbackSpinLimit = 1u << 22;
constexpr int kStage = 2048;
constexpr int kStageMaxWindows = 8;

__device__ __forceinline__ unsigned long long flag_load(const unsigned long long* p) {
    return __hip_atomic_load(p, __ATOMIC_RELAXED, __HIP_MEMORY_SCOPE_AGENT);
}
__device__ __forceinline__ void flag_store(unsigned long long* p, unsigned long long v) {
    __hip_atomic_store(p, v, __ATOMIC_RELAXED, __HIP_MEMORY_SCOPE_AGENT);
}

__device__ unsigned long long lookback(unsigned long long* flags, int64_t t, unsigned long long* err) {
    const int lane = threadIdx.x & 63;
    unsigned long long excl = 0;
    int64_t j = t - 1;
    unsigned spins = 0;
    while (true) {
        const int64_t idx = j - lane;
        const unsigned long long f = idx >= 0 ? flag_load(flags + idx) : kFlagIncl;
        const unsigned long long st = f >> 62;
        const unsigned long long incl_mask = __ballot(st == 2);
        const unsigned long long zero_mask = __ballot(st == 0);
        const int first = incl_mask ? __ffsll((long long)incl_mask) - 1 : 63;
        const unsigned long long need = (2ull << first) - 1;
        if (zero_mask & need) {
            if (++spins > kLookbackSpinLimit) {
                if (lane == 0) atomicOr(err, 1ull);
                return excl;
            }
            __builtin_amdgcn_s_sleep(1);
            continue;
        }
        excl += wave_sum<unsigned long long>(lane <= first ? (f & kFlagVal) : 0ull);
        if (incl_mask) return excl;
        j -= 64;
    }
}

template <typename K, bool HAS_VALID, bool HAS_ROW_IDS, bool HAS_PROBE_IDS>
__global__ void __launch_bounds__(kProbeThreads)
probe_fused_kernel(TableView tv, const void* __restrict__ keys, const uint8_t* __restrict__ valid, int64_t voff,
                   const uint32_t* __restrict__ probe_ids, uint32_t pbase, int64_t n, bool vec,
                   unsigned long long* flags, unsigned long long* err, uint64_t* __restrict__ out_b,
                   uint32_t* __restrict__ out_p, int64_t cap, int64_t* __restrict__ d_total, int nt) {
    __shared__ __attribute__((aligned(16))) uint32_t s_ref[kProbeTile];
    __shared__ uint64_t s_b[kStage];
    __shared__ unsigned long long s_w[kGroups][kProbeThreads / 64];
    __shared__ unsigned long long s_excl;
    const int lane = threadIdx.x & 63, wave = threadIdx.x >> 6;
    const int64_t tile0 = (int64_t)blockIdx.x * kProbeTile;
#pragma unroll
    for (int g = 0; g < kGroups; ++g) {
        const int64_t row0 = tile0 + (int64_t)g * (kProbeThreads * 4) + (int64_t)threadIdx.x * 4;
        uint32_t ref[4] = {kMiss, kMiss, kMiss, kMiss}, cnt[4] = {0, 0, 0, 0};
        if (row0 < n) {
            if (nt & 1) lookup4<K, HAS_VALID, true>(tv, keys, valid, voff, n, vec, row0, ref, cnt);
            else lookup4<K, HAS_VALID, false>(tv, keys, valid, voff, n, vec, row0, ref, cnt);
        }
        *reinterpret_cast<uint4*>(s_ref + g * (kProbeThreads * 4) + threadIdx.x * 4) =
            make_uint4(ref[0], ref[1], ref[2], ref[3]);
        unsigned long long s = 0;
#pragma unroll
        for (int q = 0; q < 4; ++q) s += resolve_count(tv.dup_rows, ref[q], cnt[q], tv.off_mask);
        const unsigned long long ws = wave_sum<unsigned long long>(s);
        if (lane == 0) s_w[g][wave] = ws;
    }
    __syncthreads();
    if (wave == 0) {
        unsigned long long tile_total = 0;
#pragma unroll
        for (int g = 0; g < kGroups; ++g)
            for (int w = 0; w < kProbeThreads / 64; ++w) tile_total += s_w[g][w];
        unsigned long long excl = 0;
        if (blockIdx.x == 0) {
            if (lane == 0) flag_store(flags, kFlagIncl | tile_total);
        } else {
            if (lane == 0) flag_store(flags + blockIdx.x, kFlagAgg | tile_total);
            excl = lookback(flags, blockIdx.x, err);
            if (lane == 0) flag_store(flags + blockIdx.x, kFlagIncl | (excl + tile_total));
        }
        if (lane == 0) {
            s_excl = excl;
            if (blockIdx.x == gridDim.x - 1) *d_total = (int64_t)(excl + tile_total);
        }
    }
    __syncthreads();
    uint32_t ref[kGroups][4];
#pragma unroll
    for (int g = 0; g < kGroups; ++g) {
        const uint4 r4 = *reinterpret_cast<const uint4*>(s_ref + g * (kProbeThreads * 4) + threadIdx.x * 4);
        ref[g][0] = r4.x; ref[g][1] = r4.y; ref[g][2] = r4.z; ref[g][3] = r4.w;
    }
    __syncthreads();
    uint32_t* s_p = s_ref;
    unsigned long long gbase = s_excl;
#pragma unroll
    for (int g = 0; g < kGroups; ++g) {
        const int64_t row0 = tile0 + (int64_t)g * (kProbeThreads * 4) + (int64_t)threadIdx.x * 4;
        uint32_t cnt[4];
        unsigned long long c_sum = 0;
#pragma unroll
        for (int q = 0; q < 4; ++q) {
            cnt[q] = ref_count(tv.dup_rows, ref[g][q], tv.off_mask);
            c_sum += cnt[q];
        }
        unsigned long long lpos = wave_incl_scan<unsigned long long>(c_sum) - c_sum;
        unsigned long long gt = 0;
        for (int w = 0; w < kProbeThreads / 64; ++w) {
            if (w < wave) lpos += s_w[g][w];
            gt += s_w[g][w];
        }
        if (gt > (unsigned long long)kStage * kStageMaxWindows) {
            if (row0 < n)
                emit4<HAS_ROW_IDS, HAS_PROBE_IDS>(tv, probe_ids, pbase, row0, ref[g], cnt, gbase + lpos, out_b, out_p, cap);
        } else {
            for (unsigned long long w0 = 0; w0 < gt; w0 += kStage) {
                const unsigned long long w1 = w0 + kStage;
                unsigned long long p = lpos;
#pragma unroll
                for (int q = 0; q < 4; ++q) {
                    const uint32_t c = cnt[q];
                    const unsigned long long a = p > w0 ? p : w0;
                    const unsigned long long b = (p + c) < w1 ? (p + c) : w1;
                    if (a < b) {
                        const uint32_t r = ref[g][q];
                        const uint32_t pidx = HAS_PROBE_IDS ? probe_ids[row0 + q] : (uint32_t)(row0 + q) + pbase;
                        const bool dup = (r & kDupFlag) != 0;
                        for (unsigned long long t = a; t < b; ++t) {
                            const uint32_t br = dup ? dup_ref_row(tv.dup_rows, r, tv.off_mask, (uint32_t)(t - p)) : r;
                            s_b[t - w0] = HAS_ROW_IDS ? tv.row_ids[br] : (uint64_t)br;
                            s_p[t - w0] = pidx;
                        }
                    }
                    p += c;
                }
                __syncthreads();
                const unsigned long long len = (gt - w0) < (unsigned long long)kStage ? (gt - w0) : kStage;
                const unsigned long long o = gbase + w0;
                for (unsigned i = threadIdx.x; i < len; i += kProbeThreads) {
                    if (o + i < (unsigned long long)cap) {
                        if (nt & 2) {
                            __builtin_nontemporal_store(s_b[i], out_b + o + i);
                            __builtin_nontemporal_store(s_p[i], out_p + o + i);
                        } else {
                            out_b[o + i] = s_b[i];
                            out_p[o + i] = s_p[i];
                        }
                    }
                }
                __syncthreads();
            }
        }
        gbase += gt;
    }
}

constexpr int kSlThreads = 1024;
constexpr int kSlTileLog = 14;
constexpr int kSlTile = 1 << kSlTileLog;
constexpr int kSlGroups = kSlTile / (kSlThreads * 4);
constexpr int kSlWidthLogMax = 15;
constexpr int kSlHistBins = 4096;
constexpr int kSlMaxSlices = kSlHistBins - 1;
constexpr int kSlOwnWin = 2048;
constexpr int kSlOwnWinHashed = 1024;
constexpr int kSlOwnWinHashed15 = 1152;
template <int TL> constexpr int hs_own_win() { return TL == 15 ? kSlOwnWinHashed15 : kSlOwnWinHashed; }
constexpr int kSlRanges = 8;
constexpr int kSlRangeRows = kSlTile / kSlRanges;
template <int TL> struct SlT {
    static_assert(TL == 14 || TL == 15, "probe tiles of 2^14 or 2^15 rows");
    static constexpr int kRows = 1 << TL;
    static constexpr int kGroups = kRows / (kSlThreads * 4);
    static constexpr int kRanges = kRows / kSlRangeRows;
    static constexpr int kEmitThreads = kRanges * 64;
};
static_assert(kSlWidthLogMax + kSlTileLog <= 32, "entry = offset << tile bits | row");
static_assert(kSlWidthLogMax <= 16 && kSlTileLog <= 16, "key offsets and rows leave as u16");

static_assert(kSlHistBins == 4 * kSlThreads, "four bins per thread");
__device__ __forceinline__ void hist_excl_scan(uint32_t* s_hist, uint32_t* s_w, uint32_t* tot) {
    const uint32_t b0 = threadIdx.x * 4;
    const uint4 h = *reinterpret_cast<const uint4*>(s_hist + b0);
    const uint32_t ex = block_excl_scan<uint32_t>(h.x + h.y + h.z + h.w, s_w, tot);
    *reinterpret_cast<uint4*>(s_hist + b0) = make_uint4(ex, ex + h.x, ex + h.x + h.y, ex + h.x + h.y + h.z);
    __syncthreads();
}

constexpr int kSlPrefetch15 = 3;
__device__ __forceinline__ void hist_excl_scan_lanes(uint32_t* s_hist, uint32_t* s_w, uint32_t* tot) {
    static_assert(kSlThreads / 64 <= 64, "wave totals in one wave's lanes");
    const uint32_t b0 = threadIdx.x * 4;
    const uint4 h = *reinterpret_cast<const uint4*>(s_hist + b0);
    const uint32_t v = h.x + h.y + h.z + h.w;
    const uint32_t incl = wave_incl_scan_dpp(v);
    const int lane = threadIdx.x & 63;
    const int wave = __builtin_amdgcn_readfirstlane((int)(threadIdx.x >> 6));
    if (lane == 63) s_w[wave] = incl;
    __syncthreads();
    const uint32_t wt = wave_incl_scan_dpp(lane < kSlThreads / 64 ? s_w[lane] : 0u);
    const uint32_t off = wave > 0 ? (uint32_t)__builtin_amdgcn_readlane((int)wt, wave - 1) : 0u;
    *tot = (uint32_t)__builtin_amdgcn_readlane((int)wt, kSlThreads / 64 - 1);
    const uint32_t ex = off + incl - v;
    *reinterpret_cast<uint4*>(s_hist + b0) = make_uint4(ex, ex + h.x, ex + h.x + h.y, ex + h.x + h.y + h.z);
    __syncthreads();
}

template <typename K, bool HAS_VALID, int TL = kSlTileLog>
__global__ void __launch_bounds__(kSlThreads, TL == 14 ? 8 : 4)
sl_partition_kernel(int64_t dmin, uint64_t drange, uint32_t wlog, uint32_t nslices, const void* __restrict__ keys,
                    const uint8_t* __restrict__ valid, int64_t voff, int64_t n, bool vec,
                    uint16_t* __restrict__ ko, uint16_t* __restrict__ rl, uint16_t* __restrict__ toff, int nt,
                    int64_t tile_off, int64_t row_base, uint32_t* __restrict__ tile_base,
                    unsigned long long* __restrict__ hdr,
                    unsigned long long* __restrict__ tcnt,
                    uint32_t* __restrict__ tent,
                    uint16_t* __restrict__ wcnt,
                    SpecGeo sg) {
    using T = SlT<TL>;
    __shared__ __attribute__((aligned(16))) uint32_t s_ent[T::kRows];
    if (sg.mm != nullptr) {
        const long long mn = sg.mm[0], mx = sg.mm[1];
        const uint32_t nb = spec_dense_blocks(mn, mx, sg.rows, sg.cap);
        if (nb == 0) return;
        dmin = mn;
        nslices = nb;
        drange = (uint64_t)nb << wlog;
    }
    __shared__ __attribute__((aligned(16))) uint32_t s_hist[kSlHistBins];
    uint32_t* s_w = s_ent;
    uint32_t* s_wc = s_ent + kSlThreads / 64;
    const int64_t tile = blockIdx.x;
    const int64_t gtile = tile + tile_off;
    const int64_t tile0 = tile * T::kRows;
    const uint32_t nbins = nslices + 1;
    const uint32_t ebase = (tent != nullptr && hdr == nullptr) ? tent[gtile] : 0u;
    for (uint32_t b = threadIdx.x; b < kSlHistBins; b += kSlThreads) s_hist[b] = 0;
    if (threadIdx.x < T::kRanges) s_wc[threadIdx.x] = 0;
    if (hdr != nullptr && blockIdx.x == 0 && threadIdx.x == 0) {
        hdr[0] = hdr[1] = 0;
        tcnt[gridDim.x] = 0;
    }
    __syncthreads();
    uint32_t e[T::kGroups][4], sr[T::kGroups][4];
    auto groups = [&](auto full_tag) {
        constexpr bool FULL = decltype(full_tag)::value;
        auto load_group = [&](int g, int64_t (&dst)[4]) {
            const int loc0 = g * (kSlThreads * 4) + threadIdx.x * 4;
            if constexpr (FULL && sizeof(K) == 8) {
                const v2i64* p = reinterpret_cast<const v2i64*>(reinterpret_cast<const K*>(keys) + tile0 + loc0);
                const v2i64 a = p[0], b = p[1];
                dst[0] = a.x; dst[1] = a.y; dst[2] = b.x; dst[3] = b.y;
            } else if constexpr (FULL) {
                const int4 a = *reinterpret_cast<const int4*>(reinterpret_cast<const K*>(keys) + tile0 + loc0);
                dst[0] = a.x; dst[1] = a.y; dst[2] = a.z; dst[3] = a.w;
            } else if (nt & 1) {
                load4<K, true>(keys, tile0 + loc0, n, vec, dst);
            } else {
                load4<K>(keys, tile0 + loc0, n, vec, dst);
            }
        };
        constexpr int D = TL == 14 ? 1 : kSlPrefetch15;
        int64_t kr[D + 1][4];
#pragma unroll
        for (int g = 0; g < D && g < T::kGroups; ++g) load_group(g, kr[g]);
#pragma unroll
        for (int g = 0; g < T::kGroups; ++g) {
            const int loc0 = g * (kSlThreads * 4) + threadIdx.x * 4;
            int64_t k[4];
#pragma unroll
            for (int q = 0; q < 4; ++q) k[q] = kr[g % (D + 1)][q];
            if (g + D < T::kGroups) load_group(g + D, kr[(g + D) % (D + 1)]);
#pragma unroll
            for (int q = 0; q < 4; ++q) {
                const int64_t row = tile0 + loc0 + q;
                const uint64_t idx = (uint64_t)k[q] - (uint64_t)dmin;
                const bool ok = row < n && (!HAS_VALID || bit_valid(valid, voff, row)) && idx < drange;
                const uint32_t sl = (uint32_t)(idx >> wlog);
                e[g][q] = ((uint32_t)(idx & ((1u << wlog) - 1)) << TL) | (uint32_t)(loc0 + q);
                sr[g][q] = ok ? (sl << TL) | atomicAdd(&s_hist[sl], 1u) : 0xFFFFFFFFu;
            }
            if (wcnt != nullptr) {
                uint32_t ws = 0;
#pragma unroll
                for (int q = 0; q < 4; ++q) ws += (uint32_t)__popcll(__ballot(sr[g][q] != 0xFFFFFFFFu));
                if ((threadIdx.x & 63) == 0 && ws) atomicAdd(&s_wc[(g * (kSlThreads * 4) + threadIdx.x * 4) / kSlRangeRows], ws);
            }
        }
    };
    if (vec && tile0 + T::kRows <= n && !(nt & 1)) groups(std::true_type{});
    else groups(std::false_type{});
    __syncthreads();
    const uint32_t my_wc = (wcnt != nullptr && threadIdx.x < T::kRanges) ? s_wc[threadIdx.x] : 0u;
    uint32_t tot;
    hist_excl_scan(s_hist, s_w, &tot);
    if (wcnt != nullptr && threadIdx.x < T::kRanges) {
        uint16_t* wc = wcnt + gtile * T::kRanges + threadIdx.x;
        *wc = (uint16_t)((ebase ? *wc : 0u) + my_wc);
    }
    uint16_t* to = toff + gtile * (int64_t)nbins;
    for (uint32_t b = threadIdx.x; b < nbins; b += kSlThreads) to[b] = (uint16_t)(ebase + s_hist[b]);
    if (tile_base != nullptr && threadIdx.x == 0) tile_base[gtile] = (uint32_t)(row_base + tile0);
    if (tcnt != nullptr && threadIdx.x == 0) tcnt[gtile] = (ebase ? tcnt[gtile] : 0ull) + tot;
    if (tent != nullptr && threadIdx.x == 0) tent[gtile] = ebase + tot;
#pragma unroll
    for (int g = 0; g < T::kGroups; ++g)
#pragma unroll
        for (int q = 0; q < 4; ++q)
            if (sr[g][q] != 0xFFFFFFFFu)
                s_ent[s_hist[sr[g][q] >> TL] + (sr[g][q] & (T::kRows - 1))] = e[g][q];
    __syncthreads();
    uint16_t* dst = ko + gtile * T::kRows;
    uint16_t* dsr = rl + gtile * T::kRows;
    if (ebase != 0) {
        for (uint32_t i = threadIdx.x; i < tot; i += kSlThreads) {
            const uint32_t v = s_ent[i];
            dst[ebase + i] = (uint16_t)(v >> TL);
            dsr[ebase + i] = (uint16_t)(v & (T::kRows - 1));
        }
        return;
    }
    const uint32_t n4 = tot & ~3u;
    for (uint32_t i = threadIdx.x * 4; i < n4; i += kSlThreads * 4) {
        const uint4 v = *reinterpret_cast<const uint4*>(s_ent + i);
        constexpr uint32_t m = T::kRows - 1;
        *reinterpret_cast<uint2*>(dst + i) = make_uint2((v.x >> TL) | ((v.y >> TL) << 16),
                                                        (v.z >> TL) | ((v.w >> TL) << 16));
        *reinterpret_cast<uint2*>(dsr + i) = make_uint2((v.x & m) | ((v.y & m) << 16), (v.z & m) | ((v.w & m) << 16));
    }
    if (threadIdx.x < (tot & 3u)) {
        const uint32_t v = s_ent[n4 + threadIdx.x];
        dst[n4 + threadIdx.x] = (uint16_t)(v >> TL);
        dsr[n4 + threadIdx.x] = (uint16_t)(v & (T::kRows - 1));
    }
}

constexpr int kSlTrChunk = 64;
__global__ void __launch_bounds__(256)
sl_toff_transpose_kernel(const uint16_t* __restrict__ toff, uint32_t nbins, int64_t ntiles,
                         uint16_t* __restrict__ toffT, SpecGeo sg) {
    __shared__ uint16_t s_t[64][kSlTrChunk + 2];
    if (sg.mm != nullptr) {
        const uint32_t nb = spec_dense_blocks(sg.mm[0], sg.mm[1], sg.rows, sg.cap);
        if (nb == 0) return;
        nbins = nb + 1;
    }
    const uint32_t nch = (nbins + kSlTrChunk - 1) / kSlTrChunk;
    const int64_t b = blockIdx.x / nch;
    if (b * 64 >= ntiles) return;
    const uint32_t c0 = (blockIdx.x % nch) * kSlTrChunk;
    const uint32_t cw = min<uint32_t>(kSlTrChunk, nbins - c0);
    for (uint32_t i = threadIdx.x; i < 64 * kSlTrChunk; i += 256) {
        const uint32_t j = i / kSlTrChunk, c = i % kSlTrChunk;
        const int64_t t = b * 64 + j;
        if (c < cw) s_t[j][c] = t < ntiles ? toff[t * nbins + c0 + c] : (uint16_t)0;
    }
    __syncthreads();
    for (uint32_t i = threadIdx.x; i < 64 * kSlTrChunk; i += 256) {
        const uint32_t c = i / 64, j = i % 64;
        if (c < cw) toffT[(b * nbins + c0 + c) * 64 + j] = s_t[j][c];
    }
}

__device__ __forceinline__ uint32_t xcd_item(uint32_t b, uint32_t grid) {
    const uint32_t x = b & 7, local = b >> 3, q = grid >> 3, r = grid & 7;
    return x < r ? x * (q + 1) + local : r * (q + 1) + (x - r) * q + local;
}

constexpr int kFragMaxTiles = 2048;
static_assert(kSlTile == kFragTileRows, "build tiles are the probe's tiles");

template <int T, int RR>
__global__ void __launch_bounds__(T)
dense_frag_build_kernel(ChunkGeom g, uint32_t nblk, int64_t ntiles, const uint16_t* __restrict__ toffT,
                        const uint16_t* __restrict__ ko, const uint16_t* __restrict__ rl,
                        const uint32_t* __restrict__ tile_base, const uint64_t* __restrict__ ids32,
                        uint32_t* __restrict__ dense, uint32_t* __restrict__ dup_rows, BigSeg* __restrict__ big,
                        BuildCounters* ctr, unsigned long long* __restrict__ spill, uint32_t run, SpecGeo sg) {
    constexpr uint32_t GV = kDenseSub << kDenseBlockShift;
    static_assert(GV == kDenseBlockValues, "frag-build blocks");
    constexpr uint32_t NSUB = GV / kDenseSub;
    __shared__ uint32_t refs[GV];
    if (sg.mm != nullptr) {
        const uint32_t nb = spec_dense_blocks(sg.mm[0], sg.mm[1], sg.rows, sg.cap);
        if (blockIdx.x >= nb) return;
        g.dmin = sg.mm[0];
        nblk = nb;
    }
    __shared__ uint32_t d_off[kDenseSub], d_cur[kDenseSub], d_cnt[kDenseSub];
    __shared__ uint32_t s_to[kFragMaxTiles + 1];
    __shared__ uint32_t s_pb[kFragMaxTiles];
    __shared__ unsigned s_ndup, s_dup[NSUB];
    __shared__ unsigned long long s_w[T / 64];
    __shared__ unsigned long long s_base, s_sp;
    __shared__ uint32_t s_carry;
    __shared__ uint32_t s_qo[NSUB + 1], s_qc[NSUB];
    const uint32_t c = [&] {
        const uint32_t b = blockIdx.x, grp = 8u * run;
        if (run <= 1 || b >= nblk / grp * grp) return b;
        const uint32_t l = b >> 3;
        return (l / run) * grp + (b & 7u) * run + l % run;
    }();
    const uint64_t cbase = (uint64_t)c * GV;
    const uint32_t nbins = nblk + 1;
    for (uint32_t i = threadIdx.x; i < GV; i += T) refs[i] = kMiss;
    if (threadIdx.x == 0) s_carry = 0;
    __syncthreads();
    for (int64_t t0 = 0; t0 < ntiles; t0 += T) {
        const int64_t t = t0 + threadIdx.x;
        uint32_t st = 0, len = 0;
        if (t < ntiles) {
            const uint16_t* to = toffT + ((t >> 6) * nbins + c) * 64 + (t & 63);
            st = to[0];
            len = (uint32_t)to[64] - st;
        }
        uint32_t tot;
        const uint32_t ex = block_excl_scan<uint32_t>(len, reinterpret_cast<uint32_t*>(s_w), &tot) + s_carry;
        if (t < ntiles) {
            s_to[t] = ex;
            s_pb[t] = (uint32_t)t * kSlTile + st - ex;
        }
        __syncthreads();
        if (threadIdx.x == 0) s_carry += tot;
        __syncthreads();
    }
    const uint32_t R = s_carry;
    if (threadIdx.x == 0) {
        s_to[ntiles] = R;
        if (R) atomicAdd(&ctr->n_valid, (unsigned long long)R);
    }
    __syncthreads();
    auto gather = [&](uint32_t r0, int (&gi)[RR], uint32_t (&gr)[RR]) {
        int own[RR];
#pragma unroll
        for (int u = 0; u < RR; ++u) own[u] = 0;
        int top = 1;
        while (top < (int)ntiles) top <<= 1;
        for (int step = top >> 1; step > 0; step >>= 1) {
#pragma unroll
            for (int u = 0; u < RR; ++u) {
                const uint32_t r = r0 + u * T + threadIdx.x;
                const int cand = own[u] + step;
                const uint32_t v = s_to[min(cand, (int)ntiles)];
                own[u] = v <= r ? cand : own[u];
            }
        }
        uint32_t pos[RR], tb[RR];
#pragma unroll
        for (int u = 0; u < RR; ++u) {
            const uint32_t r = r0 + u * T + threadIdx.x;
            const uint32_t in = 0u - (uint32_t)(r < R);
            const int o = (int)((uint32_t)own[u] & in);
            pos[u] = (s_pb[o] + r) & in;
            tb[u] = tile_base[o];
        }
#pragma unroll
        for (int u = 0; u < RR; ++u) {
            const uint32_t r = r0 + u * T + threadIdx.x;
            const int i = (int)ko[pos[u]];
            const uint32_t rw = tb[u] + rl[pos[u]];
            gi[u] = r < R ? i : -1;
            gr[u] = rw;
        }
        if (ids32 != nullptr) {
#pragma unroll
            for (int u = 0; u < RR; ++u) gr[u] = gi[u] >= 0 ? (uint32_t)ids32[gr[u]] : 0u;
        }
    };
    const bool in_regs = R <= (uint32_t)(T * RR);
    if (threadIdx.x < NSUB) s_dup[threadIdx.x] = in_regs ? 0u : 1u;
    if (threadIdx.x == 0 && !in_regs) s_sp = atomicAdd(&ctr->spill_used, 2ull * R);
    if (threadIdx.x <= NSUB) s_qo[threadIdx.x] = 0;
    __syncthreads();
    unsigned long long* sp = spill + (in_regs ? 0ull : s_sp);
    if (!in_regs) {
        const int lane = threadIdx.x & 63;
        uint32_t qn[NSUB];
#pragma unroll
        for (uint32_t q = 0; q < NSUB; ++q) qn[q] = 0;
        for (uint32_t r0 = 0; r0 < R; r0 += T * RR) {
            int gi[RR];
            uint32_t gr[RR];
            gather(r0, gi, gr);
#pragma unroll
            for (int u = 0; u < RR; ++u) {
                if (gi[u] >= 0) sp[r0 + u * T + threadIdx.x] = ((unsigned long long)(uint32_t)gi[u] << 32) | gr[u];
#pragma unroll
                for (uint32_t q = 0; q < NSUB; ++q) qn[q] += (uint32_t)(gi[u] >= 0 && (uint32_t)gi[u] / kDenseSub == q);
            }
        }
#pragma unroll
        for (uint32_t q = 0; q < NSUB; ++q)
            if (qn[q]) atomicAdd(&s_qo[q + 1], qn[q]);
        __syncthreads();
        if (threadIdx.x == 0) {
            for (uint32_t q = 0; q < NSUB; ++q) {
                s_qo[q + 1] += s_qo[q];
                s_qc[q] = s_qo[q];
            }
        }
        __syncthreads();
        unsigned long long* sp2 = sp + R;
        for (uint32_t r0 = 0; r0 < R; r0 += T) {
            const uint32_t r = r0 + threadIdx.x;
            const unsigned long long v = r < R ? sp[r] : 0ull;
            const uint32_t q = (uint32_t)(v >> 32) / kDenseSub;
#pragma unroll
            for (uint32_t qq = 0; qq < NSUB; ++qq) {
                const unsigned long long m = __ballot(r < R && q == qq);
                if (m == 0) continue;
                uint32_t base = 0;
                if (lane == 0) base = atomicAdd(&s_qc[qq], (uint32_t)__popcll(m));
                base = (uint32_t)__shfl((int)base, 0, 64);
                if (r < R && q == qq)
                    sp2[base + __builtin_amdgcn_mbcnt_hi((uint32_t)(m >> 32), __builtin_amdgcn_mbcnt_lo((uint32_t)m, 0u))] = v;
            }
        }
        __syncthreads();
        sp = sp2;
    }
    uint32_t rrow[RR];
    int ridx[RR];
    if (in_regs) {
        gather(0, ridx, rrow);
#pragma unroll
        for (int u = 0; u < RR; ++u)
            if (ridx[u] >= 0 && atomicExch(&refs[ridx[u]], rrow[u]) != kMiss) s_dup[ridx[u] / kDenseSub] = 1u;
    }
    __syncthreads();
    for (uint32_t q = 0; q < NSUB; ++q) {
        if (!s_dup[q]) continue;
        const int lo = (int)(q * kDenseSub), hi = lo + (int)kDenseSub;
        uint32_t* img = refs + lo;
        if (threadIdx.x == 0) s_ndup = 0;
        for (uint32_t i = threadIdx.x; i < kDenseSub; i += T) img[i] = 0;
        __syncthreads();
        if (in_regs) {
#pragma unroll
            for (int u = 0; u < RR; ++u)
                if (ridx[u] >= lo && ridx[u] < hi) atomicAdd(&refs[ridx[u]], 1u);
        } else {
            for (uint32_t r = s_qo[q] + threadIdx.x; r < s_qo[q + 1]; r += T) atomicAdd(&refs[(int)(sp[r] >> 32)], 1u);
        }
        __syncthreads();
        for (uint32_t i = threadIdx.x; i < kDenseSub; i += T) {
            const uint32_t cnt = img[i];
            if (cnt == 0) {
                img[i] = kMiss;
            } else if (cnt > 1) {
                const unsigned li = atomicAdd(&s_ndup, 1u);
                d_cnt[li] = cnt;
                d_cur[li] = 0;
                img[i] = kDupFlag | li;
            }
        }
        __syncthreads();
        const unsigned ndup = s_ndup;
        unsigned long long carry = 0;
        for (unsigned b0 = 0; b0 < ndup; b0 += T) {
            const unsigned li = b0 + threadIdx.x;
            const unsigned long long v = li < ndup ? (unsigned long long)d_cnt[li] + 1 : 0;
            unsigned long long tot;
            const unsigned long long ex = block_excl_scan<unsigned long long>(v, s_w, &tot);
            if (li < ndup) d_off[li] = (uint32_t)(carry + ex);
            carry += tot;
        }
        if (threadIdx.x == 0) s_base = carry ? atomicAdd(&ctr->dup_used, carry) : 0;
        __syncthreads();
        for (unsigned li = threadIdx.x; li < ndup; li += T) {
            d_off[li] += (uint32_t)s_base;
            dup_rows[d_off[li]] = d_cnt[li];
        }
        __syncthreads();
        auto place = [&](int i, uint32_t row) {
            const uint32_t rv = refs[i];
            if (rv & kDupFlag) {
                const unsigned li = rv & ~kDupFlag;
                dup_rows[d_off[li] + 1 + atomicAdd(&d_cur[li], 1u)] = row;
            } else {
                refs[i] = row;
            }
        };
        if (in_regs) {
#pragma unroll
            for (int u = 0; u < RR; ++u)
                if (ridx[u] >= lo && ridx[u] < hi) place(ridx[u], rrow[u]);
        } else {
            for (uint32_t r = s_qo[q] + threadIdx.x; r < s_qo[q + 1]; r += T) {
                const unsigned long long v = sp[r];
                place((int)(v >> 32), (uint32_t)v);
            }
        }
        __syncthreads();
        for (unsigned li = threadIdx.x; li < ndup; li += T) {
            const unsigned n = d_cnt[li], off = d_off[li];
            d_cur[li] = 0;
            if (n <= (unsigned)kSmallSeg) {
                uint32_t v[16];
#pragma unroll
                for (int i = 0; i < 16; ++i) v[i] = (i < (int)n) ? dup_rows[off + 1 + i] : 0u;
                sort16_desc(v);
#pragma unroll
                for (int i = 0; i < 16; ++i)
                    if (i < (int)n) dup_rows[off + 1 + i] = v[i];
                bool run = g.packed && n <= kRunMaxRows && v[0] < (1u << 24);
#pragma unroll
                for (int i = 1; i < (int)kRunMaxRows; ++i) run &= i >= (int)n || v[i] == v[0] - (uint32_t)i;
                if (run) d_cur[li] = make_run_ref(v[0], n);
            }
        }
        __syncthreads();
        for (uint32_t i = threadIdx.x; i < kDenseSub; i += T) {
            const uint32_t rv = img[i];
            if (rv != kMiss && (rv & kDupFlag)) {
                const unsigned li = rv & ~kDupFlag;
                if (d_cnt[li] > (unsigned)kSmallSeg) {
                    const unsigned bi = (unsigned)atomicAdd(&ctr->n_big, 1ull);
                    big[bi] = BigSeg{(unsigned long long)((uint64_t)g.dmin + cbase + lo + i), d_off[li], 0u};
                }
                const uint32_t c4 = (g.packed && d_cnt[li] <= 15u) ? d_cnt[li] : 0u;
                img[i] = d_cur[li] ? d_cur[li] : kDupFlag | (c4 << 27) | d_off[li];
            }
        }
        __syncthreads();
    }
    uint4* dst = reinterpret_cast<uint4*>(dense + cbase);
    const uint4* src = reinterpret_cast<const uint4*>(refs);
    for (uint32_t i = threadIdx.x; i < GV / 4; i += T) dst[i] = src[i];
}

constexpr int kHbSliceLog = 10;
constexpr uint32_t kHbSideSlot = (1u << kHbSliceLog) * kSlots;

template <int T, int RR, int TL = kSlTileLog>
__global__ void __launch_bounds__(T)
hashed_frag_build_kernel(uint32_t nb, uint32_t clog2, uint32_t s0, uint32_t nsl, int64_t ntiles,
                         const uint16_t* __restrict__ toffT, const unsigned long long* __restrict__ ko,
                         const uint16_t* __restrict__ rl, const uint32_t* __restrict__ tile_base,
                         const uint64_t* __restrict__ ids32, Bucket* __restrict__ tbl, uint32_t* __restrict__ dup_rows,
                         BigSeg* __restrict__ big, BuildCounters* ctr, unsigned long long* __restrict__ spill,
                         uint32_t dupcap, uint64_t dup_cap, uint64_t spill_cap) {
    constexpr uint32_t SB = 1u << kHbSliceLog;
    extern __shared__ __attribute__((aligned(16))) unsigned char smem[];
    Bucket* img = reinterpret_cast<Bucket*>(smem);
    uint32_t* s_to = reinterpret_cast<uint32_t*>(smem + (size_t)(SB + 1) * sizeof(Bucket));
    uint32_t* s_pb = s_to + ntiles + 1;
    uint32_t* s_dir = s_pb + ntiles;
    __shared__ unsigned s_ndup, s_dup;
    __shared__ uint32_t* s_dirp;
    __shared__ unsigned long long s_w[T / 64];
    __shared__ unsigned long long s_base, s_sp;
    __shared__ uint32_t s_carry;
    const uint32_t c = blockIdx.x;
    const uint32_t b0 = (s0 + c) << kHbSliceLog;
    const uint32_t nimg = min(SB, nb - b0);
    const uint32_t cmask = (1u << clog2) - 1;
    const uint32_t nbins = nsl + 1;
    const bool has_side = (s0 + c) == 0;
    {
        uint4* p = reinterpret_cast<uint4*>(img);
        for (uint32_t k = threadIdx.x; k < (SB + 1) * 4; k += T) p[k] = make_uint4(0, 0, 0, 0);
        if (threadIdx.x == 0) {
            s_ndup = 0;
            s_dup = 0;
            s_carry = 0;
        }
    }
    __syncthreads();
    for (int64_t t0 = 0; t0 < ntiles; t0 += T) {
        const int64_t t = t0 + threadIdx.x;
        uint32_t st = 0, len = 0;
        if (t < ntiles) {
            const uint16_t* to = toffT + ((t >> 6) * nbins + c) * 64 + (t & 63);
            st = to[0];
            len = (uint32_t)to[64] - st;
        }
        uint32_t tot;
        const uint32_t ex = block_excl_scan<uint32_t>(len, reinterpret_cast<uint32_t*>(s_w), &tot) + s_carry;
        if (t < ntiles) {
            s_to[t] = ex;
            s_pb[t] = (uint32_t)t * SlT<TL>::kRows + st - ex;
        }
        __syncthreads();
        if (threadIdx.x == 0) s_carry += tot;
        __syncthreads();
    }
    const uint32_t R = s_carry;
    if (threadIdx.x == 0) {
        s_to[ntiles] = R;
// ... 1491 lines not shown

__device__ __forceinline__ uint64_t splitmix64(uint64_t x) {
    uint64_t z = x + 0x9E3779B97F4A7C15ull;
    z = (z ^ (z >> 30)) * 0xBF58476D1CE4E5B9ull;
    z = (z ^ (z >> 27)) * 0x94D049BB133111EBull;
    return z ^ (z >> 31);
}

__global__ void gen_perm_kernel(int64_t* out, int64_t n, int64_t mul, int64_t range) {
    for (int64_t i = (int64_t)blockIdx.x * blockDim.x + threadIdx.x; i < n; i += (int64_t)gridDim.x * blockDim.x)
        out[i] = (int64_t)(((uint64_t)i * (uint64_t)mul) % (uint64_t)range);
}

__global__ void gen_uniform_kernel(int64_t* out, int64_t n, uint64_t seed, int64_t range) {
    for (int64_t i = (int64_t)blockIdx.x * blockDim.x + threadIdx.x; i < n; i += (int64_t)gridDim.x * blockDim.x)
        out[i] = (int64_t)(splitmix64(seed + (uint64_t)i) % (uint64_t)range);
}

int64_t build_tiles(int64_t total, int cus) {
    const int64_t by_rows = (total + kMinBuildTile - 1) / kMinBuildTile;
    return std::max<int64_t>(std::min<int64_t>(by_rows, std::max(cus, 1)), total > 0 ? 1 : 0);
}
int64_t build_tile_rows(int64_t total, int64_t ntiles) { return ntiles ? (total + ntiles - 1) / ntiles : 0; }

int64_t scan_scratch_bytes(int64_t len) { return 8 * ((len + kScanSeg - 1) / kScanSeg + 2); }

template <typename T>
static hipError_t launch_scan(T* a, int64_t len, unsigned long long* bsum, unsigned long long* total,
                              hipStream_t s) {
    const int64_t nblk = (len + kScanSeg - 1) / kScanSeg;
    if (nblk == 0) return hipSuccess;
    scan_reduce_kernel<T><<<(unsigned)nblk, kScanThreads, 0, s>>>(a, len, bsum);
    scan_top_kernel<<<1, 1024, 0, s>>>(bsum, nblk, total);
    scan_down_kernel<T><<<(unsigned)nblk, kScanThreads, 0, s>>>(a, len, bsum);
    return hipGetLastError();
}

static hipError_t set_stage_lds() {
    static const bool lds_ok = [] {
        return hipFuncSetAttribute((const void*)coarse_scatter_staged_kernel<int64_t>,
                                   hipFuncAttributeMaxDynamicSharedMemorySize, (int)kStageLds) == hipSuccess &&
               hipFuncSetAttribute((const void*)coarse_scatter_staged_kernel<int32_t>,
                                   hipFuncAttributeMaxDynamicSharedMemorySize, (int)kStageLds) == hipSuccess &&
               hipFuncSetAttribute((const void*)fine_scatter_staged_kernel,
                                   hipFuncAttributeMaxDynamicSharedMemorySize, (int)kStageLds) == hipSuccess;
    }();
    return lds_ok ? hipSuccess : hipErrorInvalidConfiguration;
}

uint32_t dense_blocks(uint32_t nchunks) { return (nchunks + (1u << kDenseBlockShift) - 1) >> kDenseBlockShift; }
bool dense_one_level(uint32_t nchunks) { return dense_blocks(nchunks) <= (uint32_t)kMaxLevel1Bins; }

uint32_t coarse_shift(uint32_t nchunks) {
    uint32_t sh = 0;
    while ((nchunks >> sh) + 1 > (uint32_t)kCoarseBins) ++sh;
    return sh;
}

hipError_t launch_scan_u64(unsigned long long* a, int64_t len, void* scratch, unsigned long long* total,
                           hipStream_t s) {
    if (len <= 0) return total ? hipMemsetAsync(total, 0, 8, s) : hipSuccess;
    return launch_scan<unsigned long long>(a, len, (unsigned long long*)scratch, total, s);
}

#ifndef DFP_MM_THREADS
#define DFP_MM_THREADS 1024
#endif
#ifndef DFP_MM_BLOCKS
#define DFP_MM_BLOCKS 256
#endif
constexpr int kMinmaxThreads = DFP_MM_THREADS;
constexpr unsigned kMinmaxBlocks = DFP_MM_BLOCKS;
__device__ __forceinline__ unsigned long long mm_ord(long long v) { return (unsigned long long)v ^ (1ull << 63); }
__device__ __forceinline__ long long mm_val(unsigned long long u) { return (long long)(u ^ (1ull << 63)); }
template <typename K>
__global__ void __launch_bounds__(kMinmaxThreads)
key_minmax_kernel(const Segment* __restrict__ segs, SegArgs sa, int nseg, int64_t total, long long* out,
                  BuildCounters* __restrict__ ctr, unsigned long long* acc, long long* mbox, long long seq,
                  long long* res) {
    __shared__ long long s_mn[kMinmaxThreads / 64], s_mx[kMinmaxThreads / 64];
    long long mn = LLONG_MAX, mx = LLONG_MIN;
    const bool by_arg = ctr != nullptr;
    if (by_arg && blockIdx.x == 0) {
        if (threadIdx.x < (unsigned)nseg) const_cast<Segment*>(segs)[threadIdx.x] = sa.s[threadIdx.x];
        if (threadIdx.x == 0) *ctr = BuildCounters{};
    }
    for (int si = 0; si < nseg; ++si) {
        const Segment sg = by_arg ? sa.s[si] : segs[si];
        const int64_t stride = (int64_t)gridDim.x * blockDim.x;
        if (sizeof(K) == 8 && sg.valid == nullptr && (reinterpret_cast<uintptr_t>(sg.keys) & 15) == 0) {
            const v2i64* kp = reinterpret_cast<const v2i64*>(sg.keys);
            const int64_t n2 = sg.n >> 1;
            for (int64_t j0 = (int64_t)blockIdx.x * blockDim.x + threadIdx.x; j0 < n2; j0 += 16 * stride) {
                v2i64 v[16];
                bool in[16];
#pragma unroll
                for (int u = 0; u < 16; ++u) {
                    const int64_t j = j0 + u * stride;
                    in[u] = j < n2;
                    v[u] = in[u] ? kp[j] : v2i64{0, 0};
                }
#pragma unroll
                for (int u = 0; u < 16; ++u) {
                    if (!in[u]) continue;
                    const long long a = v[u].x, b = v[u].y;
                    mn = min(mn, min(a, b));
                    mx = max(mx, max(a, b));
                }
            }
            if ((sg.n & 1) && blockIdx.x == 0 && threadIdx.x == 0) {
                const long long k = (long long)ld_key<K>(sg.keys, sg.n - 1);
                mn = min(mn, k);
                mx = max(mx, k);
            }
            continue;
        }
        for (int64_t i0 = (int64_t)blockIdx.x * blockDim.x + threadIdx.x; i0 < sg.n; i0 += 4 * stride) {
            long long k[4];
            bool ok[4];
#pragma unroll
            for (int u = 0; u < 4; ++u) {
                const int64_t i = i0 + u * stride;
                ok[u] = i < sg.n && bit_valid(sg.valid, sg.voff, i);
                k[u] = i < sg.n ? (long long)ld_key<K>(sg.keys, i) : 0;
            }
#pragma unroll
            for (int u = 0; u < 4; ++u) {
                if (!ok[u]) continue;
                mn = k[u] < mn ? k[u] : mn;
                mx = k[u] > mx ? k[u] : mx;
            }
        }
    }
    auto block_reduce = [&]() {
#pragma unroll
        for (int d = 32; d >= 1; d >>= 1) {
            const long long x = __shfl_xor(mn, d, 64), y = __shfl_xor(mx, d, 64);
            mn = x < mn ? x : mn;
            mx = y > mx ? y : mx;
        }
        if ((threadIdx.x & 63) == 0) {
            s_mn[threadIdx.x >> 6] = mn;
            s_mx[threadIdx.x >> 6] = mx;
        }
        __syncthreads();
        for (int w = 0; w < kMinmaxThreads / 64; ++w) {
            mn = s_mn[w] < mn ? s_mn[w] : mn;
            mx = s_mx[w] > mx ? s_mx[w] : mx;
        }
    };
    block_reduce();
    if (threadIdx.x != 0) return;
    const unsigned long long r0 = atomicMax(&acc[0], ~mm_ord(mn));
    const unsigned long long r1 = atomicMax(&acc[1], mm_ord(mx));
    asm volatile("" ::"v"(r0), "v"(r1));
    if (atomicAdd(&acc[2], 1ull) != (unsigned long long)gridDim.x - 1) return;
    const long long rmn = mm_val(~atomicExch(&acc[0], 0ull));
    const long long rmx = mm_val(atomicExch(&acc[1], 0ull));
    atomicExch(&acc[2], 0ull);
    out[0] = rmn;
    out[1] = rmx;
    if (res != nullptr) {
        res[0] = rmn;
        res[1] = rmx;
    }
    if (mbox != nullptr) {
        mbox[0] = rmn;
        mbox[1] = rmx;
        __hip_atomic_store(&mbox[2], seq, __ATOMIC_RELEASE, __HIP_MEMORY_SCOPE_SYSTEM);
    }
}

hipError_t launch_key_minmax_one(int key_bytes, const Segment* h_segs, Segment* d_segs, int nseg, BuildCounters* ctr,
                                 int64_t total, int64_t* out, unsigned long long* done, int64_t* mbox, int64_t seq,
                                 hipStream_t s, int64_t* res) {
    const int64_t cap = total <= (int64_t)1 << 24 ? kMinmaxBlocks / 2 : kMinmaxBlocks;
    const unsigned grid = (unsigned)std::max<int64_t>(1, std::min<int64_t>((total + 4095) / 4096, cap));
    SegArgs sa{};
    if (ctr != nullptr) {
        if (nseg > kArgSegs) return hipErrorInvalidValue;
        for (int i = 0; i < nseg; ++i) sa.s[i] = h_segs[i];
    }
    if (key_bytes == 8)
        key_minmax_kernel<int64_t><<<grid, kMinmaxThreads, 0, s>>>(d_segs, sa, nseg, total, (long long*)out, ctr, done,
                                                                   (long long*)mbox, (long long)seq, (long long*)res);
    else
        key_minmax_kernel<int32_t><<<grid, kMinmaxThreads, 0, s>>>(d_segs, sa, nseg, total, (long long*)out, ctr, done,
                                                                   (long long*)mbox, (long long)seq, (long long*)res);
    return hipGetLastError();
}

template <typename K>
__global__ void __launch_bounds__(256)
key_minmax_part_kernel(const Segment* __restrict__ segs, SegArgs sa, int nseg, int64_t total, long long* out,
                  BuildCounters* __restrict__ ctr) {
    __shared__ long long s_mn[4], s_mx[4];
    long long mn = LLONG_MAX, mx = LLONG_MIN;
    const bool by_arg = ctr != nullptr;
    if (by_arg && blockIdx.x == 0) {
        if (threadIdx.x < (unsigned)nseg) const_cast<Segment*>(segs)[threadIdx.x] = sa.s[threadIdx.x];
        if (threadIdx.x == 0) *ctr = BuildCounters{};
    }
    for (int si = 0; si < nseg; ++si) {
        const Segment sg = by_arg ? sa.s[si] : segs[si];
        const int64_t stride = (int64_t)gridDim.x * blockDim.x;
        if (sizeof(K) == 8 && sg.valid == nullptr && (reinterpret_cast<uintptr_t>(sg.keys) & 15) == 0) {
            const v2i64* kp = reinterpret_cast<const v2i64*>(sg.keys);
            const int64_t n2 = sg.n >> 1;
            for (int64_t j0 = (int64_t)blockIdx.x * blockDim.x + threadIdx.x; j0 < n2; j0 += 8 * stride) {
                v2i64 v[8];
                bool in[8];
#pragma unroll
                for (int u = 0; u < 8; ++u) {
                    const int64_t j = j0 + u * stride;
                    in[u] = j < n2;
                    v[u] = in[u] ? kp[j] : v2i64{0, 0};
                }
#pragma unroll
                for (int u = 0; u < 8; ++u) {
                    if (!in[u]) continue;
                    const long long a = v[u].x, b = v[u].y;
                    mn = min(mn, min(a, b));
                    mx = max(mx, max(a, b));
                }
            }
            if ((sg.n & 1) && blockIdx.x == 0 && threadIdx.x == 0) {
                const long long k = (long long)ld_key<K>(sg.keys, sg.n - 1);
                mn = min(mn, k);
                mx = max(mx, k);
            }
            continue;
        }
        for (int64_t i0 = (int64_t)blockIdx.x * blockDim.x + threadIdx.x; i0 < sg.n; i0 += 4 * stride) {
            long long k[4];
            bool ok[4];
#pragma unroll
            for (int u = 0; u < 4; ++u) {
                const int64_t i = i0 + u * stride;
                ok[u] = i < sg.n && bit_valid(sg.valid, sg.voff, i);
                k[u] = i < sg.n ? (long long)ld_key<K>(sg.keys, i) : 0;
            }
#pragma unroll
            for (int u = 0; u < 4; ++u) {
                if (!ok[u]) continue;
                mn = k[u] < mn ? k[u] : mn;
                mx = k[u] > mx ? k[u] : mx;
            }
        }
    }
#pragma unroll
    for (int d = 32; d >= 1; d >>= 1) {
        const long long a = __shfl_xor(mn, d, 64), b = __shfl_xor(mx, d, 64);
        mn = a < mn ? a : mn;
        mx = b > mx ? b : mx;
    }
    if ((threadIdx.x & 63) == 0) {
        s_mn[threadIdx.x >> 6] = mn;
        s_mx[threadIdx.x >> 6] = mx;
    }
    __syncthreads();
    if (threadIdx.x == 0) {
        for (int w = 1; w < 4; ++w) {
            mn = s_mn[w] < mn ? s_mn[w] : mn;
            mx = s_mx[w] > mx ? s_mx[w] : mx;
        }
        out[2 + 2 * blockIdx.x] = mn;
        out[3 + 2 * blockIdx.x] = mx;
    }
}

__global__ void __launch_bounds__(1024) minmax_final_kernel(long long* out, unsigned nblk, long long* mbox,
                                                            long long seq) {
    __shared__ long long s_mn[16], s_mx[16];
    long long mn = LLONG_MAX, mx = LLONG_MIN;
    for (unsigned b = threadIdx.x; b < nblk; b += blockDim.x) {
        mn = min(mn, out[2 + 2 * b]);
        mx = max(mx, out[3 + 2 * b]);
    }
#pragma unroll
    for (int d = 32; d >= 1; d >>= 1) {
        mn = min(mn, (long long)__shfl_xor(mn, d, 64));
        mx = max(mx, (long long)__shfl_xor(mx, d, 64));
    }
    if ((threadIdx.x & 63) == 0) {
        s_mn[threadIdx.x >> 6] = mn;
        s_mx[threadIdx.x >> 6] = mx;
    }
    __syncthreads();
    if (threadIdx.x == 0) {
        for (int w = 1; w < (int)(blockDim.x >> 6); ++w) {
            mn = min(mn, s_mn[w]);
            mx = max(mx, s_mx[w]);
        }
        out[0] = mn;
        out[1] = mx;
        if (mbox != nullptr) {
            mbox[0] = mn;
            mbox[1] = mx;
            __hip_atomic_store(&mbox[2], seq, __ATOMIC_RELEASE, __HIP_MEMORY_SCOPE_SYSTEM);
        }
    }
}

hipError_t launch_key_minmax(int key_bytes, const Segment* h_segs, Segment* d_segs, int nseg, BuildCounters* ctr,
                             int64_t total, int64_t* out, int64_t* mbox, int64_t seq, hipStream_t s) {
    const unsigned grid =
        (unsigned)std::max<int64_t>(1, std::min<int64_t>((total + 4095) / 4096, kMinmaxMaxBlocks));
    SegArgs sa{};
    if (ctr != nullptr) {
        if (nseg > kArgSegs) return hipErrorInvalidValue;
        for (int i = 0; i < nseg; ++i) sa.s[i] = h_segs[i];
    }
    if (key_bytes == 8)
        key_minmax_part_kernel<int64_t><<<grid, 256, 0, s>>>(d_segs, sa, nseg, total, (long long*)out, ctr);
    else
        key_minmax_part_kernel<int32_t><<<grid, 256, 0, s>>>(d_segs, sa, nseg, total, (long long*)out, ctr);
    minmax_final_kernel<<<1, 1024, 0, s>>>((long long*)out, grid, (long long*)mbox, (long long)seq);
    return hipGetLastError();
}

int64_t frag_build_tiles(const int64_t* seg_n, int nseg, int tl) {
    const int64_t tile = (int64_t)1 << tl;
    int64_t t = 0;
    for (int i = 0; i < nseg; ++i) t += (seg_n[i] + tile - 1) / tile;
    return t;
}
int hashed_build_tile_log() {
    static const int v = [] {
        const char* e = getenv("DFP_HJ_HB_TILE_LOG");
        return e && atoi(e) == 14 ? 14 : 15;
    }();
    return v;
}
bool frag_build_ok(const ChunkGeom& g, int64_t ftiles) {
    return g.dense && dense_one_level(g.nchunks) && dense_blocks(g.nchunks) <= (uint32_t)kSlMaxSlices &&
           ftiles <= kFragMaxTiles;
}
int64_t frag_build_scratch_bytes(const ChunkGeom& g, int64_t ftiles, int64_t total) {
    const int64_t nbins = dense_blocks(g.nchunks) + 1;
    return 2 * ftiles * kSlTile + 2 * ftiles * kSlTile + 2 * ftiles * nbins + 2 * ((ftiles + 63) & ~(int64_t)63) * nbins +
           16 * total + 6 * 256;
}

uint32_t frag_run() {
    static const uint32_t v = [] {
        const char* e = getenv("DFP_HJ_FRAG_RUN");
        return e ? (uint32_t)std::max(1, atoi(e)) : 4u;
    }();
    return v;
}
uint32_t frag_threads() {
    const char* e = getenv("DFP_HJ_FRAG_T");
    return e && atoi(e) == 1024 ? 1024u : 512u;
}
hipError_t launch_build_frag(int key_bytes, const Segment* h_segs, int nseg, const ChunkGeom& g, int64_t ftiles,
                             void* scratch, uint32_t* tile_base, const uint64_t* ids32, uint32_t* dense,
                             uint32_t* dup_rows, BigSeg* big, BuildCounters* ctr, const Segment* d_segs, int64_t total,
                             bool ids_as_rows, int big_grid, const SpecGeo& spec, hipStream_t s) {
    const uint32_t nblk = dense_blocks(g.nchunks), nbins = nblk + 1;
    constexpr uint32_t GV = kDenseSub << kDenseBlockShift;
    const uint32_t wlog = 31 - __builtin_clz(GV);
    auto a256 = [](uintptr_t x) { return (x + 255) & ~(uintptr_t)255; };
    uintptr_t p = a256((uintptr_t)scratch);
    uint16_t* ko = (uint16_t*)p;   p = a256(p + 2 * ftiles * kSlTile);
    uint16_t* rl = (uint16_t*)p;   p = a256(p + 2 * ftiles * kSlTile);
    uint16_t* toff = (uint16_t*)p; p = a256(p + 2 * ftiles * nbins);
    uint16_t* toffT = (uint16_t*)p; p = a256(p + 2 * ((ftiles + 63) & ~(int64_t)63) * nbins);
    unsigned long long* spill = (unsigned long long*)p;
    int64_t t0 = 0;
    for (int i = 0; i < nseg; ++i) {
        const Segment& sg = h_segs[i];
        const int64_t nt = (sg.n + kSlTile - 1) / kSlTile;
        if (nt == 0) continue;
        const bool vec = (reinterpret_cast<uintptr_t>(sg.keys) & 15) == 0;
        const uint64_t drange = (uint64_t)nblk * GV;
#define DFP_BLP(KT, HV)                                                                                          \
    sl_partition_kernel<KT, HV><<<(unsigned)nt, kSlThreads, 0, s>>>(g.dmin, drange, wlog, nblk, sg.keys, sg.valid, \
                                                                   sg.voff, sg.n, vec, ko, rl, toff, 0, t0,          \
                                                                   sg.row_base, tile_base, nullptr, nullptr, nullptr, \
                                                                   nullptr, spec)
        if (key_bytes == 8) {
            if (sg.valid) DFP_BLP(int64_t, true); else DFP_BLP(int64_t, false);
        } else {
            if (sg.valid) DFP_BLP(int32_t, true); else DFP_BLP(int32_t, false);
        }
#undef DFP_BLP
        t0 += nt;
    }
    sl_toff_transpose_kernel<<<(unsigned)((ftiles + 63) / 64 * ((nblk + kSlTrChunk) / kSlTrChunk)), 256, 0, s>>>(
        toff, nbins, ftiles, toffT, spec);
    if (frag_threads() != 1024)
        dense_frag_build_kernel<512, 16><<<nblk, 512, 0, s>>>(g, nblk, ftiles, toffT, ko, rl, tile_base,
                                                             ids_as_rows ? ids32 : nullptr, dense, dup_rows, big, ctr,
                                                             spill, frag_run(), spec);
    else
        dense_frag_build_kernel<1024, 8><<<nblk, 1024, 0, s>>>(g, nblk, ftiles, toffT, ko, rl, tile_base,
                                                               ids_as_rows ? ids32 : nullptr, dense, dup_rows, big, ctr,
                                                               spill, frag_run(), spec);
    dup_sort_big_kernel<<<big_grid, kBigThreads, 0, s>>>(dup_rows, big, ctr, d_segs, nseg, total, key_bytes,
                                                         ids_as_rows);
    return hipGetLastError();
}

bool hashed_frag_ok(const ChunkGeom& g, int64_t ftiles) {
    return !g.dense && g.clog2 <= (uint32_t)kHbSliceLog && ftiles <= kFragMaxTiles && ftiles > 0;
}
uint32_t hashed_frag_slices(const ChunkGeom& g) { return (g.nb + (1u << kHbSliceLog) - 1) >> kHbSliceLog; }
int64_t hashed_frag_scratch_bytes(const ChunkGeom& g, int64_t ftiles, int64_t total) {
    const int64_t nbins = std::min<uint32_t>(hashed_frag_slices(g), (uint32_t)kSlMaxSlices) + 1;
    const int64_t kSlTile = (int64_t)1 << hashed_build_tile_log();
    return 8 * ftiles * kSlTile + 2 * ftiles * kSlTile + 2 * ftiles * nbins + 2 * ((ftiles + 63) & ~(int64_t)63) * nbins +
           32 * total + 6 * 256;
}
template <int TL>
hipError_t launch_build_hashed_frag_tl(int key_bytes, const Segment* h_segs, int nseg, const ChunkGeom& g, int64_t ftiles,
                                    void* scratch, uint32_t* tile_base, const uint64_t* ids32, Bucket* tbl,
                                    uint32_t* dup_rows, BigSeg* big, BuildCounters* ctr, const Segment* d_segs,
                                    int64_t total, bool ids_as_rows, int cus, hipStream_t s) {
    constexpr int T = 512, RR = 8;
    constexpr int64_t kSlTile = SlT<TL>::kRows;
    const uint32_t nsl_all = hashed_frag_slices(g);
    const int64_t nbins_max = std::min<uint32_t>(nsl_all, (uint32_t)kSlMaxSlices) + 1;
    auto a256 = [](uintptr_t x) { return (x + 255) & ~(uintptr_t)255; };
    uintptr_t p = a256((uintptr_t)scratch);
    unsigned long long* ko = (unsigned long long*)p; p = a256(p + 8 * ftiles * kSlTile);
    uint16_t* rl = (uint16_t*)p;   p = a256(p + 2 * ftiles * kSlTile);
    uint16_t* toff = (uint16_t*)p; p = a256(p + 2 * ftiles * nbins_max);
    uint16_t* toffT = (uint16_t*)p; p = a256(p + 2 * ((ftiles + 63) & ~(int64_t)63) * nbins_max);
    unsigned long long* spill = (unsigned long long*)p;
    const size_t img = (size_t)((1u << kHbSliceLog) + 1) * sizeof(Bucket) + 8 * (size_t)ftiles + 4;
    const size_t budget = 80 * 1024 - 256;
    const uint32_t dupcap = img < budget ? (uint32_t)((budget - img) / 12) : 0u;
    const size_t lds = img + (size_t)dupcap * 12;
    const void* kfn = (const void*)hashed_frag_build_kernel<T, RR, TL>;
    hipError_t e = hipFuncSetAttribute(kfn, hipFuncAttributeMaxDynamicSharedMemorySize, (int)lds);
    if (e != hipSuccess) return e;
    static const bool dbg_sync = getenv("DFP_HJ_DEBUG_SYNC") != nullptr;
    auto chk = [&](const char* what) -> hipError_t {
        if (!dbg_sync) return hipSuccess;
        const hipError_t q = hipStreamSynchronize(s);
        if (q != hipSuccess) fprintf(stderr, "dfp-hj: %s failed: %s\n", what, hipGetErrorString(q));
        return q;
    };
    for (uint32_t s0 = 0; s0 < nsl_all; s0 += (uint32_t)kSlMaxSlices) {
        const uint32_t nsl = std::min<uint32_t>(nsl_all - s0, (uint32_t)kSlMaxSlices), nbins = nsl + 1;
        int64_t t0 = 0;
        for (int i = 0; i < nseg; ++i) {
            const Segment& sg = h_segs[i];
            const int64_t nt = (sg.n + kSlTile - 1) / kSlTile;
            if (nt == 0) continue;
            const bool vec = (reinterpret_cast<uintptr_t>(sg.keys) & 15) == 0;
            const unsigned pgrid = (unsigned)std::min<int64_t>(nt, cus);
#define DFP_HBP(KT, HV)                                                                                             \
    if (TL == 15)                                                                                                   \
        hs_partition32_kernel<KT, HV><<<pgrid, kSlThreads, 0, s>>>(g.nb, kHbSliceLog, s0, nsl, sg.keys, sg.valid,     \
                                                                  sg.voff, sg.n, nt, vec, ko, rl, toff, nullptr,     \
                                                                  nullptr, nullptr, t0, sg.row_base, tile_base);     \
    else                                                                                                            \
        hs_partition_kernel<KT, HV><<<pgrid, kSlThreads, 0, s>>>(g.nb, kHbSliceLog, s0, nsl, sg.keys, sg.valid,       \
                                                                sg.voff, sg.n, nt, vec, ko, rl, toff, nullptr, nullptr, \
                                                                nullptr, t0, sg.row_base, tile_base)
            if (key_bytes == 8) {
                if (sg.valid) DFP_HBP(int64_t, true); else DFP_HBP(int64_t, false);
            } else {
                if (sg.valid) DFP_HBP(int32_t, true); else DFP_HBP(int32_t, false);
            }
#undef DFP_HBP
            if ((e = chk("hs_partition (build)")) != hipSuccess) return e;
            t0 += nt;
        }
        sl_toff_transpose_kernel<<<(unsigned)((ftiles + 63) / 64 * ((nbins + kSlTrChunk - 1) / kSlTrChunk)), 256, 0,
                                   s>>>(toff, nbins, ftiles, toffT, SpecGeo{});
        if ((e = chk("toff transpose")) != hipSuccess) return e;
        hashed_frag_build_kernel<T, RR, TL><<<nsl, T, lds, s>>>(g.nb, g.clog2, s0, nsl, ftiles, toffT, ko, rl, tile_base,
                                                           ids_as_rows ? ids32 : nullptr, tbl, dup_rows, big, ctr,
                                                           spill, dupcap, (uint64_t)(2 * total + 2),
                                                           (uint64_t)(4 * total));
        if ((e = chk("hashed_frag_build")) != hipSuccess) return e;
    }
    dup_sort_big_kernel<<<cus, kBigThreads, 0, s>>>(dup_rows, big, ctr, d_segs, nseg, total, key_bytes, ids_as_rows);
    return hipGetLastError();
}

hipError_t launch_build_hashed_frag(int key_bytes, const Segment* h_segs, int nseg, const ChunkGeom& g, int64_t ftiles,
                                    void* scratch, uint32_t* tile_base, const uint64_t* ids32, Bucket* tbl,
                                    uint32_t* dup_rows, BigSeg* big, BuildCounters* ctr, const Segment* d_segs,
                                    int64_t total, bool ids_as_rows, int cus, hipStream_t s) {
    return hashed_build_tile_log() == 15
               ? launch_build_hashed_frag_tl<15>(key_bytes, h_segs, nseg, g, ftiles, scratch, tile_base, ids32, tbl,
                                                 dup_rows, big, ctr, d_segs, total, ids_as_rows, cus, s)
               : launch_build_hashed_frag_tl<14>(key_bytes, h_segs, nseg, g, ftiles, scratch, tile_base, ids32, tbl,
                                                 dup_rows, big, ctr, d_segs, total, ids_as_rows, cus, s);
}

hipError_t launch_build(int key_bytes, const Segment* d_segs, int nseg, int64_t total, const ChunkGeom& g,
                        uint32_t* hist, uint32_t* hist1, uint32_t* chunk_starts, int64_t ntiles,
                        int64_t tile_rows, void* scan_scratch,
                        unsigned long long* tkeys, uint32_t* trows, unsigned long long* skeys, uint32_t* srows,
                        uint64_t* row_ids, bool ids_as_rows, Bucket* tbl, uint32_t* dense, uint32_t* dup_rows,
                        BigSeg* big, BuildCounters* ctr, int big_grid, hipStream_t s) {
    const uint32_t nb = g.nb, clog2 = g.clog2, nchunks = g.nchunks;
    const int64_t hlen = (int64_t)(nchunks + 1) * ntiles;
    if (g.dense && dense_one_level(nchunks)) {
        const uint32_t gshift = kDenseBlockShift;
        const uint32_t nblk = dense_blocks(nchunks);
        if (ntiles > 0) {
            unsigned long long* scr = (unsigned long long*)scan_scratch;
            if (key_bytes == 8)
                coarse_hist_kernel<int64_t, kStageMaxBins, 4><<<(unsigned)ntiles, kHistThreads, 0, s>>>(
                    d_segs, nseg, total, g, gshift, nblk, hist1, ntiles, tile_rows);
            else
                coarse_hist_kernel<int32_t, kStageMaxBins, 4><<<(unsigned)ntiles, kHistThreads, 0, s>>>(
                    d_segs, nseg, total, g, gshift, nblk, hist1, ntiles, tile_rows);
            hipError_t e = launch_scan(hist1, (int64_t)nblk * ntiles, scr, &ctr->n_valid, s);
            if (e != hipSuccess) return e;
            if ((e = set_stage_lds()) != hipSuccess) return e;
            chunk_starts_kernel<<<(unsigned)std::min<uint32_t>((nblk + 1 + 255) / 256, 4096), 256, 0, s>>>(
                hist1, ntiles, nblk - 1, ctr, chunk_starts);
            if (key_bytes == 8)
                coarse_scatter_staged_kernel<int64_t><<<(unsigned)ntiles, kHistThreads, kStageLds, s>>>(
                    d_segs, nseg, total, g, gshift, nblk, hist1, ntiles, tkeys, trows, row_ids, ids_as_rows,
                    tile_rows);
            else
                coarse_scatter_staged_kernel<int32_t><<<(unsigned)ntiles, kHistThreads, kStageLds, s>>>(
                    d_segs, nseg, total, g, gshift, nblk, hist1, ntiles, tkeys, trows, row_ids, ids_as_rows,
                    tile_rows);
            dense_chunk_build_kernel<kDenseSub << kDenseBlockShift, 1024, 8><<<nblk, 1024, 0, s>>>(
                g, chunk_starts, tkeys, trows, dense, dup_rows, big, ctr);
            dup_sort_big_kernel<<<big_grid, kBigThreads, 0, s>>>(dup_rows, big, ctr, d_segs, nseg, total, key_bytes,
                                                                 ids_as_rows);
        }
        return hipGetLastError();
    }
    const uint32_t gshift = coarse_shift(nchunks);
    const uint32_t ngroups = (nchunks >> gshift) + 1;
    if (ntiles > 0) {
        unsigned long long* scr = (unsigned long long*)scan_scratch;
        if (key_bytes == 8)
            coarse_hist_kernel<int64_t, kCoarseBins, kHistThreads / 64><<<(unsigned)ntiles, kHistThreads, 0, s>>>(
                d_segs, nseg, total, g, gshift, ngroups, hist1, ntiles, tile_rows);
        else
            coarse_hist_kernel<int32_t, kCoarseBins, kHistThreads / 64><<<(unsigned)ntiles, kHistThreads, 0, s>>>(
                d_segs, nseg, total, g, gshift, ngroups, hist1, ntiles, tile_rows);
        hipError_t e = launch_scan(hist1, (int64_t)ngroups * ntiles, scr, &ctr->n_valid, s);
        if (e != hipSuccess) return e;
        if ((e = set_stage_lds()) != hipSuccess) return e;
        if (key_bytes == 8)
            coarse_scatter_staged_kernel<int64_t><<<(unsigned)ntiles, kHistThreads, kStageLds, s>>>(
                d_segs, nseg, total, g, gshift, ngroups, hist1, ntiles, tkeys, trows, row_ids,
                ids_as_rows, tile_rows);
        else
            coarse_scatter_staged_kernel<int32_t><<<(unsigned)ntiles, kHistThreads, kStageLds, s>>>(
                d_segs, nseg, total, g, gshift, ngroups, hist1, ntiles, tkeys, trows, row_ids,
                ids_as_rows, tile_rows);
        if ((e = hipMemsetAsync(hist, 0, sizeof(uint32_t) * (size_t)hlen, s)) != hipSuccess) return e;
        fine_hist_kernel<<<(unsigned)ntiles, kHistThreads, sizeof(uint32_t) * kFineLdsBins, s>>>(tkeys, ctr, g, gshift,
                                                                                         hist, ntiles, tile_rows);
        if ((e = launch_scan(hist, hlen, scr, &ctr->n_valid, s)) != hipSuccess) return e;
        chunk_starts_kernel<<<(unsigned)std::min<uint32_t>((nchunks + 2 + 255) / 256, 4096), 256, 0, s>>>(
            hist, ntiles, nchunks, ctr, chunk_starts);
        fine_scatter_staged_kernel<<<(unsigned)ntiles, kHistThreads, kStageLds, s>>>(
            tkeys, trows, ctr, g, gshift, hist, ntiles, skeys, srows, tile_rows);
    }
    if (g.dense) {
        if (ntiles > 0) {
            dense_chunk_build_kernel<kDenseSub, 512, 4><<<nchunks, 512, 0, s>>>(g, chunk_starts, skeys, srows, dense,
                                                                                dup_rows, big, ctr);
            dup_sort_big_kernel<<<big_grid, kBigThreads, 0, s>>>(dup_rows, big, ctr, d_segs, nseg, total, key_bytes,
                                                                 ids_as_rows);
        }
        return hipGetLastError();
    }
    const uint32_t CB = 1u << clog2;
    const size_t img = (size_t)CB * sizeof(Bucket);
    const size_t lds_cap = (CB <= 512 ? 40 * 1024 : CB <= 1024 ? 80 * 1024 : 160 * 1024) - 2048;
    uint32_t dupcap = (uint32_t)std::min<size_t>((size_t)CB * kSlots, (lds_cap - img) / 12);
    const size_t lds = img + (size_t)dupcap * 12;
    const void* kfn = CB <= 512 ? (const void*)chunk_build_kernel<512> : (const void*)chunk_build_kernel<1024>;
    hipError_t e = hipFuncSetAttribute(kfn, hipFuncAttributeMaxDynamicSharedMemorySize, (int)lds);
    if (e != hipSuccess) return e;
    if (ntiles > 0) {
        if (CB <= 512)
            chunk_build_kernel<512><<<nchunks + 1, 512, lds, s>>>(nb, clog2, nchunks, chunk_starts, skeys, srows,
                                                                 tbl, dup_rows, big, ctr, dupcap);
        else
            chunk_build_kernel<1024><<<nchunks + 1, 1024, lds, s>>>(nb, clog2, nchunks, chunk_starts, skeys, srows,
                                                                   tbl, dup_rows, big, ctr, dupcap);
        dup_sort_big_kernel<<<big_grid, kBigThreads, 0, s>>>(dup_rows, big, ctr, d_segs, nseg, total, key_bytes,
                                                             ids_as_rows);
    }
    return hipGetLastError();
}

int64_t probe_tiles(int64_t n) { return (n + kProbeTile - 1) / kProbeTile; }

namespace {
struct ProbeWs {
    unsigned long long* tcnt;
    int64_t bytes;
};
inline uintptr_t al256(uintptr_t x) { return (x + 255) & ~(uintptr_t)255; }
ProbeWs probe_ws_layout(void* base, int64_t n) {
    const int64_t nt = probe_tiles(n > 0 ? n : 0);
    ProbeWs w;
    uintptr_t p = (uintptr_t)base + 256;
    w.tcnt = (unsigned long long*)p; p = al256(p + 8 * (nt + 2));
    w.bytes = (int64_t)(p - (uintptr_t)base) + 256;
    return w;
}

struct SlicedWs {
    unsigned long long* tcnt;
    uint32_t* tent;
    uint16_t* toff;
    void* ko;
    uint16_t* rl;
    uint32_t* res;
    uint16_t* wcnt;
    int64_t bytes;
};
SlicedWs sliced_ws_layout(void* base, int64_t n, int tl) {
    const int64_t tile = (int64_t)1 << tl;
    const int64_t nt = (n + tile - 1) / tile;
    SlicedWs w;
    uintptr_t p = (uintptr_t)base + 256;
    w.tcnt = (unsigned long long*)p;  p = al256(p + 8 * (nt + 2));
    w.tent = (uint32_t*)p;            p = al256(p + 4 * (nt + 2));
    w.toff = (uint16_t*)p;            p = al256(p + 2 * nt * (kSlMaxSlices + 1));
    w.ko = (void*)p;                  p = al256(p + 8 * nt * tile);
    w.rl = (uint16_t*)p;              p = al256(p + 2 * nt * tile);
    w.res = (uint32_t*)p;             p = al256(p + 4 * nt * tile);
    w.wcnt = (uint16_t*)p;            p = al256(p + 2 * (tile / kSlRangeRows) * (nt + 2));
    w.bytes = (int64_t)(p - (uintptr_t)base) + 256;
    return w;
}

int env_probe_mode() {
    const char* e = getenv("DFP_HJ_PROBE_MODE");
    if (!e) return 0;
    if (e[0] == 'f') return 3;
    if (e[0] == 's') return 4;
    return 0;
}
std::atomic<int> g_probe_mode{-1};
int probe_mode() {
    int m = g_probe_mode.load(std::memory_order_relaxed);
    if (m < 0) {
        m = env_probe_mode();
        g_probe_mode.store(m, std::memory_order_relaxed);
    }
    return m;
}
}

void set_probe_mode(int mode) {
    g_probe_mode.store(mode == 3 || mode == 4 ? mode : 0, std::memory_order_relaxed);
}
int get_probe_mode() { return probe_mode(); }

int64_t probe_workspace(int64_t n) {
    return std::max(probe_ws_layout(nullptr, n).bytes,
                    std::max(sliced_ws_layout(nullptr, n, 14).bytes, sliced_ws_layout(nullptr, n, 15).bytes));
}

namespace {
uint32_t sl_wlog() {
    static const uint32_t w = [] {
        const char* e = getenv("DFP_HJ_SLICE_LOG");
        const int v = e ? atoi(e) : 15;
        return (uint32_t)std::min(std::max(v, 10), kSlWidthLogMax);
    }();
    return w;
}
int sl_num_cus() {
    static const int c = [] {
        int d = 0, v = 0;
        if (hipGetDevice(&d) != hipSuccess || hipDeviceGetAttribute(&v, hipDeviceAttributeMultiprocessorCount, d) !=
                                                  hipSuccess || v < 1)
            v = 256;
        return v;
    }();
    return c;
}
int sl_env_int(const char* name, int dflt) {
    const char* e = getenv(name);
    return e ? std::max(1, atoi(e)) : dflt;
}
int sl_emit_wgs_per_cu() {
    static const int v = sl_env_int("DFP_HJ_SL_EMIT_WGS", 2);
    return v;
// ... 547 lines not shown
```

### datafusion-parallelism_amd/csrc/hj_launch.h

```cpp
#pragma once
#include <hip/hip_runtime.h>
#include "hj_device.h"

namespace dfp {

constexpr int kMinBuildTile = 4096;
constexpr int kMaxChunks = 131071;

int64_t build_tiles(int64_t total, int cus);
int64_t build_tile_rows(int64_t total, int64_t ntiles);
int64_t scan_scratch_bytes(int64_t len);

constexpr int kCoarseBins = 128;
constexpr int kMaxLevel1Bins = 2048;
constexpr uint32_t kDenseBlockShift = 2;
uint32_t dense_blocks(uint32_t nchunks);
bool dense_one_level(uint32_t nchunks);

hipError_t launch_build(int key_bytes, const Segment* d_segs, int nseg, int64_t total,
                        const ChunkGeom& g, uint32_t* hist, uint32_t* hist1, uint32_t* chunk_starts,
                        int64_t ntiles, int64_t tile_rows, void* scan_scratch,
                        unsigned long long* tkeys, uint32_t* trows, unsigned long long* skeys,
                        uint32_t* srows, uint64_t* row_ids, bool ids_as_rows, Bucket* tbl,
                        uint32_t* dense, uint32_t* dup_rows, BigSeg* big, BuildCounters* ctr,
                        int big_grid, hipStream_t s);
constexpr int64_t kFragTileRows = 16384;
int64_t frag_build_tiles(const int64_t* seg_n, int nseg, int tile_log = 14);
int hashed_build_tile_log();
bool frag_build_ok(const ChunkGeom& g, int64_t ftiles);
int64_t frag_build_scratch_bytes(const ChunkGeom& g, int64_t ftiles, int64_t total);
hipError_t launch_build_frag(int key_bytes, const Segment* h_segs, int nseg, const ChunkGeom& g, int64_t ftiles,
                             void* scratch, uint32_t* tile_base, const uint64_t* ids32, uint32_t* dense,
                             uint32_t* dup_rows, BigSeg* big, BuildCounters* ctr, const Segment* d_segs, int64_t total,
                             bool ids_as_rows, int big_grid, const SpecGeo& spec, hipStream_t s);
bool hashed_frag_ok(const ChunkGeom& g, int64_t ftiles);
int64_t hashed_frag_scratch_bytes(const ChunkGeom& g, int64_t ftiles, int64_t total);
hipError_t launch_build_hashed_frag(int key_bytes, const Segment* h_segs, int nseg, const ChunkGeom& g, int64_t ftiles,
                                    void* scratch, uint32_t* tile_base, const uint64_t* ids32, Bucket* tbl,
                                    uint32_t* dup_rows, BigSeg* big, BuildCounters* ctr, const Segment* d_segs,
                                    int64_t total, bool ids_as_rows, int cus, hipStream_t s);
constexpr int kMinmaxMaxBlocks = 4096;
constexpr int kArgSegs = 16;
struct SegArgs {
    Segment s[kArgSegs];
};
hipError_t launch_key_minmax(int key_bytes, const Segment* h_segs, Segment* d_segs, int nseg, BuildCounters* ctr,
                             int64_t total, int64_t* out, int64_t* mbox, int64_t seq, hipStream_t s);
hipError_t launch_key_minmax_one(int key_bytes, const Segment* h_segs, Segment* d_segs, int nseg, BuildCounters* ctr,
                                 int64_t total, int64_t* out, unsigned long long* done, int64_t* mbox, int64_t seq,
                                 hipStream_t s, int64_t* res = nullptr);

void set_probe_mode(int mode);
int get_probe_mode();
int set_probe_tile_log(int tl);
int64_t probe_tiles(int64_t n);
int64_t probe_workspace(int64_t n);
hipError_t launch_probe(int key_bytes, const TableView& tv, const void* keys, const uint8_t* valid,
                        int64_t voff, const uint32_t* probe_ids, uint32_t probe_base, int64_t n, uint64_t* out_b,
                        uint32_t* out_p, int64_t cap, int64_t* d_total, void* workspace,
                        hipEvent_t built, hipStream_t s);

constexpr int64_t kMatchWsHeader = 16;
int64_t probe_match_workspace(uint64_t claim_bits);
hipError_t launch_probe_match(int key_bytes, const TableView& tv, const void* keys, const uint8_t* valid, int64_t voff,
                              int64_t n, uint8_t* out_bitmap, uint32_t* out_counts, uint8_t* flags, int64_t nflags,
                              int64_t* d_stats, void* workspace, uint64_t claim_bits, hipStream_t s);

hipError_t launch_dense_rebase(uint32_t* refs, uint64_t n, uint32_t base, uint32_t mask, hipStream_t s);
hipError_t launch_table_stats(const TableView& tv,
                              unsigned long long* out ,
                              hipStream_t s);
hipError_t launch_chain_links(const TableView& tv, int64_t* prev, int64_t nrows, hipStream_t s);

struct PartSpec {
    int64_t lo, hi;
    uint64_t mul;
    int by_range;
};
hipError_t launch_radix_partition(int key_bytes, const void* keys, const uint8_t* valid,
                                  int64_t voff, const uint64_t* ids, uint64_t id_base,
                                  int64_t n, int nparts, const PartSpec& spec, void* out_keys,
                                  int out_key_bytes, int64_t key_offset, void* out_ids, int id_bytes,
                                  int64_t* counts, void* workspace, hipStream_t s);
int64_t radix_partition_workspace(int64_t n, int nparts);
int64_t radix_regions_workspace(int64_t n, int nparts);
hipError_t launch_radix_regions(int key_bytes, const void* keys, const uint8_t* valid, int64_t voff,
                                const uint64_t* ids, uint64_t id_base, int64_t n, int nparts, const PartSpec& spec,
                                void* out_keys, int out_key_bytes, int64_t key_offset, void* out_ids, int id_bytes,
                                int64_t cap, int64_t* counts, void* workspace, hipStream_t s);

hipError_t launch_scan_u64(unsigned long long* a, int64_t len, void* scratch, unsigned long long* total,
                           hipStream_t s);

hipError_t launch_mark_rows(const void* idx, int idx_bytes, int64_t n, uint8_t* flags, int64_t nflags,
                            hipStream_t s);
int64_t select_workspace(int64_t n);
hipError_t launch_select_rows(const uint8_t* flags, int64_t n, uint8_t want, uint64_t* out, int64_t* d_count,
                              void* workspace, hipStream_t s);
int64_t select_bitmap_workspace(int64_t n);
hipError_t launch_select_bitmap(const uint8_t* bitmap, int64_t bit_offset, int64_t n, int want, uint32_t base,
                                uint32_t* out, int64_t* d_count, void* workspace, hipStream_t s);
hipError_t launch_gather_fixed(const void* src, const uint8_t* src_valid, int64_t src_voff, int elem_bytes,
                               const void* idx, int idx_bytes, int64_t n, void* dst, uint8_t* dst_valid,
                               hipStream_t s);
int64_t gather_var_workspace(int64_t n);
hipError_t launch_gather_var(const void* offsets, int offset_bytes, const uint8_t* values, const uint8_t* src_valid,
                             int64_t src_voff, const void* idx, int idx_bytes, int64_t n, void* out_offsets,
                             uint8_t* out_values, int64_t values_cap, uint8_t* dst_valid, int64_t* d_values_len,
                             void* workspace, hipStream_t s);

struct FilterView {
    unsigned long long* words;
    uint64_t nwords;
    int64_t lo;
    uint64_t span;
    bool range;
};
hipError_t launch_filter_add(const FilterView& f, int key_bytes, const void* keys, const uint8_t* valid, int64_t voff,
                             int64_t n, unsigned long long* dropped, hipStream_t s);
hipError_t launch_filter_test(const FilterView& f, int key_bytes, const void* keys, const uint8_t* valid, int64_t voff,
                              int64_t n, uint8_t* out_bitmap, int64_t* d_count, hipStream_t s);
int64_t filter_select_workspace(int64_t n);
hipError_t launch_filter_select(const FilterView& f, int key_bytes, const void* keys, const uint8_t* valid,
                                int64_t voff, int64_t n, uint32_t probe_base, void* out_keys, uint32_t* out_ids,
                                int64_t* d_count, void* workspace, hipStream_t s);

hipError_t launch_iota_u32(uint32_t* out, int64_t n, uint32_t base, hipStream_t s);
hipError_t launch_add_u32(uint32_t* a, int64_t n, uint32_t base, hipStream_t s);
hipError_t launch_widen_u32(const uint32_t* in, int64_t n, uint64_t* out, hipStream_t s);
int64_t merge_pairs_workspace(int64_t nrows);
hipError_t launch_merge_pairs(const uint64_t* b, const uint32_t* p, int64_t m, int64_t nrows, uint64_t* out_b,
                              uint32_t* out_p, int64_t cap, void* ws, hipStream_t s);

struct KeyCol {
    const void* values;
    const void* offsets;
    const uint8_t* valid;
    int64_t voff;
    int width;
    int offset_bytes;
};
constexpr int kMaxKeyCols = 16;
struct KeyCols {
    KeyCol c[kMaxKeyCols];
    int n;
};
hipError_t launch_composite_keys(const KeyCols& cols, int64_t n, int64_t* out_keys, uint64_t* out_valid,
                                 hipStream_t s);
int64_t equal_pairs_workspace(int64_t n);
hipError_t launch_equal_pairs(const KeyCols& bc, const KeyCols& pc, const uint64_t* bidx, const uint32_t* pidx,
                              int64_t n, uint64_t* out_b, uint32_t* out_p, int64_t* d_count, void* ws,
                              hipStream_t s);

hipError_t launch_gen_perm(int64_t* out, int64_t n, int64_t mul, int64_t range, hipStream_t s);
hipError_t launch_gen_uniform(int64_t* out, int64_t n, uint64_t seed, int64_t range,
                              hipStream_t s);

}
```

Measured before the change: 168,200 Mrows/s.

## Fuse build key min/max into partition pass via first-key anchored dense blocks

Removes the separate key min/max kernel before the speculative dense build. The partition kernel now bins keys into 8192-value blocks relative to an anchor taken from the first key, and records per-tile min/max as it goes. A single-block fold kernel then reduces the tile ranges and publishes them to the host mailbox. If any key falls outside the anchor window, a flag is set and the remaining tiles only compute min/max, falling back to the old path. The dense table is aligned to a block boundary, and a skip offset corrects the exported views. This saves one full read of the build keys in exchange for a more complex partition kernel and a slightly larger table.

```diff
diff --git a/datafusion-parallelism_amd/csrc/hj_api.cpp b/datafusion-parallelism_amd/csrc/hj_api.cpp
--- a/datafusion-parallelism_amd/csrc/hj_api.cpp
+++ b/datafusion-parallelism_amd/csrc/hj_api.cpp
@@ -67,6 +67,7 @@
     int64_t* h_minmax = nullptr;
     int64_t* d_mbox = nullptr;
     int64_t mb_seq = 0;
+    unsigned long long* d_aflag = nullptr;
 };
 std::mutex g_pool_mu;
 std::unordered_map<int, std::vector<BuildResources>> g_pool;
@@ -97,7 +98,9 @@
            hipEventCreateWithFlags(&r->evp, probe_ev_flags()) == hipSuccess &&
            hipHostMalloc((void**)&r->h_minmax, 4 * sizeof(int64_t), hipHostMallocCoherent | hipHostMallocMapped) ==
                hipSuccess &&
-           hipHostGetDevicePointer((void**)&r->d_mbox, r->h_minmax, 0) == hipSuccess;
+           hipHostGetDevicePointer((void**)&r->d_mbox, r->h_minmax, 0) == hipSuccess &&
+           hipMalloc((void**)&r->d_aflag, 64) == hipSuccess && hipMemset(r->d_aflag, 0, 64) == hipSuccess &&
+           hipStreamSynchronize(nullptr) == hipSuccess;
 }
 
 void release_resources(int dev, const BuildResources& r) {
@@ -282,6 +285,13 @@
     }();
     return v;
 }
+bool anchor_build_on() {
+    static const bool v = [] {
+        const char* e = getenv("DFP_HJ_ANCHOR_BUILD");
+        return !(e != nullptr && e[0] == '0');
+    }();
+    return v;
+}
 double load_factor() {
     const char* e = getenv("DFP_HJ_LOAD_FACTOR");
     double lf = e ? atof(e) : kDefaultLoadFactor;
@@ -334,6 +344,7 @@
     bool packed = false;
     int64_t dmin = 0;
     uint64_t drange = 0;
+    uint64_t dskip = 0;
     bool has_range = false;
     bool force_dense = false;
     int64_t range_lo = 0, range_hi = 0;
@@ -355,6 +366,7 @@
     std::mutex spec_mu;
     int64_t spec_seq = 0;
     uint32_t spec_cap = 0;
+    bool spec_anchor = false;
     const int64_t* spec_mm = nullptr;
     std::vector<Segment> spec_segs;
     bool mm_known = false;
@@ -469,6 +481,14 @@
     const ChunkGeom spec_g{0, 0, spec_cap << kDenseBlockShift, kDenseShift, 0, 1, packed_ok ? 1 : 0};
     const bool spec = minmax && spec_build_on() && !t->has_base && !t->force_dense && t->multi == nullptr &&
                       device_budget() <= 0 && frag_build_mode() && spec_cap > 0 && frag_build_ok(spec_g, ftiles);
+    const Segment* aseg = nullptr;
+    for (const Segment& sg : segs)
+        if (sg.n > 0) {
+            aseg = &sg;
+            break;
+        }
+    const bool anchor = spec && anchor_build_on() && aseg != nullptr && aseg->valid == nullptr;
+    t->dskip = 0;
     ChunkGeom g{};
     bool dense = false;
     if (need_range || (t->has_range && total > 0 && (build_mode() == 0 || t->force_dense))) {
@@ -480,11 +500,13 @@
         if (minmax) {
             int64_t* mb = t->res.h_minmax;
             const int64_t seq = ++t->res.mb_seq;
-            HIP_TRY(launch_key_minmax(t->key_bytes, segs.data(), d_segs, (int)segs.size(), by_arg ? ctr : nullptr,
-                                      total, d_minmax, t->res.d_mbox, seq, s));
+            if (!anchor)
+                HIP_TRY(launch_key_minmax(t->key_bytes, segs.data(), d_segs, (int)segs.size(), by_arg ? ctr : nullptr,
+                                          total, d_minmax, t->res.d_mbox, seq, s));
             if (spec) {
                 t->spec_seq = seq;
                 t->spec_cap = spec_cap;
+                t->spec_anchor = anchor;
                 t->spec_mm = d_minmax;
                 t->spec_segs = segs;
                 mm[0] = 1;
@@ -573,7 +595,7 @@
         uint64_t* ids32 = nullptr;
         BigSeg* fbig;
         const int64_t fbytes =
-            frag ? frag_build_scratch_bytes(g, ftiles, total) : hashed_frag_scratch_bytes(g, hftiles, total);
+            frag ? frag_build_scratch_bytes(g, ftiles, total, anchor) : hashed_frag_scratch_bytes(g, hftiles, total);
         if ((st = dev_alloc(t, t->scratch, &fscr, (size_t)fbytes)) != HJ_OK) return st;
         if ((st = dev_alloc(t, t->scratch, &p, sizeof(uint32_t) * (size_t)(frag ? ftiles : hftiles))) != HJ_OK)
             return st;
@@ -600,9 +622,13 @@
         if (frag) {
             HIP_TRY(launch_build_frag(t->key_bytes, segs.data(), (int)segs.size(), g, ftiles, fscr, d_tb, ids32,
                                       t->dense, t->dup_rows, fbig, ctr, d_segs, total, ids_as_rows, cus,
-                                      spec ? SpecGeo{(const long long*)d_minmax, (uint64_t)total, spec_cap}
+                                      spec ? SpecGeo{(const long long*)d_minmax, (uint64_t)total, spec_cap,
+                                                     anchor ? 1u : 0u}
                                            : SpecGeo{nullptr, 0, 0},
-                                      s));
+                                      s,
+                                      anchor ? AnchorArgs{aseg->keys, t->res.d_aflag, (long long*)d_minmax}
+                                             : AnchorArgs{},
+                                      t->res.d_mbox, t->spec_seq, by_arg));
             if (spec) t->spec_pending.store(true, std::memory_order_release);
             return HJ_OK;
         }
@@ -694,10 +720,11 @@
     int64_t* mb = t->res.h_minmax;
     HIP_TRY(wait_mailbox(mb, t->spec_seq, t->spec_mm, t->bstream));
     const int64_t mn = mb[0], mx = mb[1];
-    if (spec_dense_blocks(mn, mx, (uint64_t)t->total_rows, t->spec_cap) != 0) {
+    if (spec_dense_blocks(mn, mx, (uint64_t)t->total_rows, t->spec_cap, t->spec_anchor) != 0) {
         const uint64_t range = (uint64_t)mx - (uint64_t)mn + 1;
-        t->dmin = mn;
-        t->drange = range;
+        t->dskip = t->spec_anchor ? (uint64_t)mn - (uint64_t)dense_block_base(mn) : 0;
+        t->dmin = (int64_t)((uint64_t)mn - t->dskip);
+        t->drange = range + t->dskip;
         t->nchunks = (uint32_t)((range + (1u << kDenseShift) - 1) >> kDenseShift);
         t->spec_pending.store(false, std::memory_order_release);
         return HJ_OK;
@@ -1561,9 +1588,9 @@
     if (!refs || !nvalues || !key_min || !dup_rows || !dup_used || !packed) return fail(HJ_ERR_INVALID, "null out");
     if (t->multi != nullptr || t->dense == nullptr || t->ctr == nullptr || t->wrapped)
         return fail(HJ_ERR_INVALID, "hj_table_dense_piece: not a built direct-addressed single-device table");
-    *refs = t->dense;
-    *nvalues = t->drange;
-    *key_min = t->dmin;
+    *refs = t->dense + t->dskip;
+    *nvalues = t->drange - t->dskip;
+    *key_min = (int64_t)((uint64_t)t->dmin + t->dskip);
     *dup_rows = t->dup_rows;
     *dup_used = reinterpret_cast<const uint64_t*>(&t->ctr->dup_used);
     *packed = t->packed ? 1 : 0;
@@ -1576,7 +1603,8 @@
     if (st != HJ_OK) return st;
     if (t->multi != nullptr || t->dense == nullptr || t->ctr == nullptr || t->wrapped)
         return fail(HJ_ERR_INVALID, "hj_table_dense_export: not a built direct-addressed single-device table");
-    if (refs_dst != nullptr && (v0 > t->drange || n > t->drange - v0))
+    const uint64_t xrange = t->drange - t->dskip;
+    if (refs_dst != nullptr && (v0 > xrange || n > xrange - v0))
         return fail(HJ_ERR_INVALID, "hj_table_dense_export: refs range past the table's key range");
     if (dup_dst != nullptr && dup_n > (uint64_t)(2 * t->total_rows + 2))
         return fail(HJ_ERR_INVALID, "hj_table_dense_export: more segment words than the table holds");
@@ -1584,7 +1612,7 @@
     hipStream_t s = (hipStream_t)stream;
     if (s != t->bstream) HIP_TRY(hipStreamWaitEvent(s, t->res.ev1, 0));
     if (refs_dst != nullptr && n > 0)
-        HIP_TRY(hipMemcpyAsync(refs_dst, t->dense + v0, n * sizeof(uint32_t), hipMemcpyDeviceToDevice, s));
+        HIP_TRY(hipMemcpyAsync(refs_dst, t->dense + t->dskip + v0, n * sizeof(uint32_t), hipMemcpyDeviceToDevice, s));
     if (dup_dst != nullptr && dup_n > 0)
         HIP_TRY(hipMemcpyAsync(dup_dst, t->dup_rows, dup_n * sizeof(uint32_t), hipMemcpyDeviceToDevice, s));
     if (dup_used_dst != nullptr)
diff --git a/datafusion-parallelism_amd/csrc/hj_device.h b/datafusion-parallelism_amd/csrc/hj_device.h
--- a/datafusion-parallelism_amd/csrc/hj_device.h
+++ b/datafusion-parallelism_amd/csrc/hj_device.h
@@ -115,11 +115,25 @@
 constexpr uint64_t kDenseFactor = 8;
 constexpr uint64_t kDenseBlockValues = 8192;
 
+constexpr uint32_t kDenseBlockLog = 13;
+static_assert((1ull << kDenseBlockLog) == kDenseBlockValues, "block shift");
+constexpr int64_t kAnchorBias = 2047;
+constexpr int kAnchorHdr = 4;
+struct AnchorArgs {
+    const void* keys;
+    unsigned long long* flag;
+    long long* part;
+};
 struct SpecGeo {
     const long long* mm;
     uint64_t rows;
     uint32_t cap;
+    uint32_t anchor;
 };
+static_assert(sizeof(SpecGeo) == 24, "the probe's kernels take the same arguments as before the anchor build");
+__host__ __device__ inline int64_t dense_block_base(int64_t key) {
+    return (int64_t)((uint64_t)(key >> kDenseBlockLog) << kDenseBlockLog);
+}
 __host__ __device__ inline uint32_t spec_dense_blocks(int64_t mn, int64_t mx, uint64_t rows, uint32_t cap) {
     if (mn > mx) return 0u;
     const uint64_t range = (uint64_t)mx - (uint64_t)mn + 1;
@@ -127,5 +141,12 @@
     const uint64_t nblk = (range + kDenseBlockValues - 1) / kDenseBlockValues;
     return nblk <= cap ? (uint32_t)nblk : 0u;
 }
+__host__ __device__ inline uint32_t spec_dense_blocks(int64_t mn, int64_t mx, uint64_t rows, uint32_t cap,
+                                                      bool aligned) {
+    if (!aligned) return spec_dense_blocks(mn, mx, rows, cap);
+    if (spec_dense_blocks(mn, mx, rows, ~0u) == 0u) return 0u;
+    const uint64_t nblk = (uint64_t)((mx >> kDenseBlockLog) - (mn >> kDenseBlockLog)) + 1;
+    return nblk <= cap ? (uint32_t)nblk : 0u;
+}
 
 }
diff --git a/datafusion-parallelism_amd/csrc/hj_kernels.hip b/datafusion-parallelism_amd/csrc/hj_kernels.hip
--- a/datafusion-parallelism_amd/csrc/hj_kernels.hip
+++ b/datafusion-parallelism_amd/csrc/hj_kernels.hip
@@ -1196,7 +1196,40 @@
     __syncthreads();
 }
 
-template <typename K, bool HAS_VALID, int TL = kSlTileLog>
+template <typename K, bool HAS_VALID, int ROWS>
+__device__ __forceinline__ void anchor_tile_range(const void* __restrict__ keys, const uint8_t* __restrict__ valid,
+                                               int64_t voff, int64_t n, int64_t tile0, long long* s_red,
+                                               long long* __restrict__ part) {
+    long long mn = LLONG_MAX, mx = LLONG_MIN;
+    for (int i = threadIdx.x; i < ROWS; i += kSlThreads) {
+        const int64_t row = tile0 + i;
+        if (row < n && (!HAS_VALID || bit_valid(valid, voff, row))) {
+            const long long k = (long long)ld_key<K>(keys, row);
+            mn = min(mn, k);
+            mx = max(mx, k);
+        }
+    }
+#pragma unroll
+    for (int d = 32; d >= 1; d >>= 1) {
+        mn = min(mn, (long long)__shfl_xor(mn, d, 64));
+        mx = max(mx, (long long)__shfl_xor(mx, d, 64));
+    }
+    if ((threadIdx.x & 63) == 0) {
+        s_red[2 * (threadIdx.x >> 6)] = mn;
+        s_red[2 * (threadIdx.x >> 6) + 1] = mx;
+    }
+    __syncthreads();
+    if (threadIdx.x == 0) {
+        for (int w = 1; w < kSlThreads / 64; ++w) {
+            mn = min(mn, s_red[2 * w]);
+            mx = max(mx, s_red[2 * w + 1]);
+        }
+        part[0] = mn;
+        part[1] = mx;
+    }
+}
+
+template <typename K, bool HAS_VALID, int TL = kSlTileLog, bool ANCHOR = false>
 __global__ void __launch_bounds__(kSlThreads, TL == 14 ? 8 : 4)
 sl_partition_kernel(int64_t dmin, uint64_t drange, uint32_t wlog, uint32_t nslices, const void* __restrict__ keys,
                     const uint8_t* __restrict__ valid, int64_t voff, int64_t n, bool vec,
@@ -1209,7 +1242,27 @@
                     SpecGeo sg) {
     using T = SlT<TL>;
     __shared__ __attribute__((aligned(16))) uint32_t s_ent[T::kRows];
-    if (sg.mm != nullptr) {
+    static_assert(!ANCHOR || (TL == kSlTileLog && 2 * kAnchorBias + 2 == kSlHistBins), "anchor bins fill the histogram");
+    int64_t ablk = 0;
+    const AnchorArgs aa{ANCHOR ? (const void*)tent : nullptr, ANCHOR ? hdr : nullptr,
+                        ANCHOR ? reinterpret_cast<long long*>(tcnt) : nullptr};
+    if constexpr (ANCHOR) {
+        hdr = nullptr;
+        tcnt = nullptr;
+        tent = nullptr;
+        wcnt = nullptr;
+        const int64_t a0 = ((int64_t)ld_key<K>(aa.keys, 0) >> kDenseBlockLog) - kAnchorBias;
+        ablk = (int64_t)(((uint64_t)(uint32_t)__builtin_amdgcn_readfirstlane((int)(a0 >> 32)) << 32) |
+                         (uint32_t)__builtin_amdgcn_readfirstlane((int)a0));
+        nslices = kSlHistBins - 1;
+        if (__hip_atomic_load(aa.flag, __ATOMIC_RELAXED, __HIP_MEMORY_SCOPE_AGENT) != 0) {
+            anchor_tile_range<K, HAS_VALID, T::kRows>(keys, valid, voff, n, (int64_t)blockIdx.x * T::kRows,
+                                                      reinterpret_cast<long long*>(s_ent),
+                                                      aa.part + kAnchorHdr + 2 * ((int64_t)blockIdx.x + tile_off));
+            return;
+        }
+    }
+    if (!ANCHOR && sg.mm != nullptr) {
         const long long mn = sg.mm[0], mx = sg.mm[1];
         const uint32_t nb = spec_dense_blocks(mn, mx, sg.rows, sg.cap);
         if (nb == 0) return;
@@ -1227,6 +1280,12 @@
     const uint32_t ebase = (tent != nullptr && hdr == nullptr) ? tent[gtile] : 0u;
     for (uint32_t b = threadIdx.x; b < kSlHistBins; b += kSlThreads) s_hist[b] = 0;
     if (threadIdx.x < T::kRanges) s_wc[threadIdx.x] = 0;
+    uint32_t* s_code = s_ent + 64;
+    if (ANCHOR && threadIdx.x == 0) {
+        s_code[0] = 0xFFFFFFFFu;
+        s_code[1] = 0u;
+        s_code[2] = 0u;
+    }
     if (hdr != nullptr && blockIdx.x == 0 && threadIdx.x == 0) {
         hdr[0] = hdr[1] = 0;
         tcnt[gridDim.x] = 0;
@@ -1264,6 +1323,16 @@
 #pragma unroll
             for (int q = 0; q < 4; ++q) {
                 const int64_t row = tile0 + loc0 + q;
+                if constexpr (ANCHOR) {
+                    const uint64_t bin = (uint64_t)((k[q] >> kDenseBlockLog) - ablk);
+                    const bool valid_row = row < n && (!HAS_VALID || bit_valid(valid, voff, row));
+                    const bool ok = valid_row && bin <= (uint64_t)(2 * kAnchorBias);
+                    const uint32_t sl = (uint32_t)bin;
+                    const uint32_t off = (uint32_t)k[q] & (uint32_t)(kDenseBlockValues - 1);
+                    e[g][q] = (off << TL) | (uint32_t)(loc0 + q);
+                    sr[g][q] = ok ? (sl << TL) | atomicAdd(&s_hist[sl], 1u) : 0xFFFFFFFFu - (uint32_t)valid_row;
+                    continue;
+                }
                 const uint64_t idx = (uint64_t)k[q] - (uint64_t)dmin;
                 const bool ok = row < n && (!HAS_VALID || bit_valid(valid, voff, row)) && idx < drange;
                 const uint32_t sl = (uint32_t)(idx >> wlog);
@@ -1280,7 +1349,47 @@
     };
     if (vec && tile0 + T::kRows <= n && !(nt & 1)) groups(std::true_type{});
     else groups(std::false_type{});
-    __syncthreads();
+    if constexpr (ANCHOR) {
+        uint32_t cmin = 0xFFFFFFFFu, cmax = 0u;
+        bool far = false;
+#pragma unroll
+        for (int g = 0; g < T::kGroups; ++g)
+#pragma unroll
+            for (int q = 0; q < 4; ++q) {
+                const uint32_t code = ((sr[g][q] >> TL) << kDenseBlockLog) | (e[g][q] >> TL);
+                const bool ok = sr[g][q] < 0xFFFFFFFEu;
+                far |= sr[g][q] == 0xFFFFFFFEu;
+                cmin = min(cmin, ok ? code : 0xFFFFFFFFu);
+                cmax = max(cmax, ok ? code : 0u);
+            }
+        if (far) s_code[2] = 1u;
+#pragma unroll
+        for (int d = 32; d >= 1; d >>= 1) {
+            cmin = min(cmin, (uint32_t)__shfl_xor((int)cmin, d, 64));
+            cmax = max(cmax, (uint32_t)__shfl_xor((int)cmax, d, 64));
+        }
+        if ((threadIdx.x & 63) == 0) {
+            atomicMin(&s_code[0], cmin);
+            atomicMax(&s_code[1], cmax);
+        }
+    }
+    __syncthreads();
+    if constexpr (ANCHOR) {
+        long long* part = aa.part + kAnchorHdr + 2 * gtile;
+        if (s_code[2] != 0) {
+            if (threadIdx.x == 0) __hip_atomic_store(aa.flag, 1ull, __ATOMIC_RELAXED, __HIP_MEMORY_SCOPE_AGENT);
+            __syncthreads();
+            anchor_tile_range<K, HAS_VALID, T::kRows>(keys, valid, voff, n, tile0, reinterpret_cast<long long*>(s_hist),
+                                                      part);
+            return;
+        }
+        if (threadIdx.x == 0) {
+            const uint32_t lo = s_code[0], hi = s_code[1];
+            const uint64_t org = (uint64_t)ablk << kDenseBlockLog;
+            part[0] = lo <= hi ? (long long)(org + lo) : LLONG_MAX;
+            part[1] = lo <= hi ? (long long)(org + hi) : LLONG_MIN;
+        }
+    }
     const uint32_t my_wc = (wcnt != nullptr && threadIdx.x < T::kRanges) ? s_wc[threadIdx.x] : 0u;
     uint32_t tot;
     hist_excl_scan(s_hist, s_w, &tot);
@@ -1289,7 +1398,12 @@
         *wc = (uint16_t)((ebase ? *wc : 0u) + my_wc);
     }
     uint16_t* to = toff + gtile * (int64_t)nbins;
-    for (uint32_t b = threadIdx.x; b < nbins; b += kSlThreads) to[b] = (uint16_t)(ebase + s_hist[b]);
+    if constexpr (ANCHOR) {
+        const uint4 h = *reinterpret_cast<const uint4*>(s_hist + threadIdx.x * 4);
+        *reinterpret_cast<uint2*>(to + threadIdx.x * 4) = make_uint2(h.x | (h.y << 16), h.z | (h.w << 16));
+    } else {
+        for (uint32_t b = threadIdx.x; b < nbins; b += kSlThreads) to[b] = (uint16_t)(ebase + s_hist[b]);
+    }
     if (tile_base != nullptr && threadIdx.x == 0) tile_base[gtile] = (uint32_t)(row_base + tile0);
     if (tcnt != nullptr && threadIdx.x == 0) tcnt[gtile] = (ebase ? tcnt[gtile] : 0ull) + tot;
     if (tent != nullptr && threadIdx.x == 0) tent[gtile] = ebase + tot;
@@ -1330,10 +1444,15 @@
 sl_toff_transpose_kernel(const uint16_t* __restrict__ toff, uint32_t nbins, int64_t ntiles,
                          uint16_t* __restrict__ toffT, SpecGeo sg) {
     __shared__ uint16_t s_t[64][kSlTrChunk + 2];
+    uint32_t sbins = nbins, lo = 0;
     if (sg.mm != nullptr) {
-        const uint32_t nb = spec_dense_blocks(sg.mm[0], sg.mm[1], sg.rows, sg.cap);
+        const uint32_t nb = spec_dense_blocks(sg.mm[0], sg.mm[1], sg.rows, sg.cap, sg.anchor != 0);
         if (nb == 0) return;
-        nbins = nb + 1;
+        sbins = nbins = nb + 1;
+        if (sg.anchor) {
+            sbins = kSlHistBins;
+            lo = (uint32_t)sg.mm[2];
+        }
     }
     const uint32_t nch = (nbins + kSlTrChunk - 1) / kSlTrChunk;
     const int64_t b = blockIdx.x / nch;
@@ -1343,7 +1462,7 @@
     for (uint32_t i = threadIdx.x; i < 64 * kSlTrChunk; i += 256) {
         const uint32_t j = i / kSlTrChunk, c = i % kSlTrChunk;
         const int64_t t = b * 64 + j;
-        if (c < cw) s_t[j][c] = t < ntiles ? toff[t * nbins + c0 + c] : (uint16_t)0;
+        if (c < cw) s_t[j][c] = t < ntiles ? toff[t * sbins + lo + c0 + c] : (uint16_t)0;
     }
     __syncthreads();
     for (uint32_t i = threadIdx.x; i < 64 * kSlTrChunk; i += 256) {
@@ -1372,9 +1491,9 @@
     constexpr uint32_t NSUB = GV / kDenseSub;
     __shared__ uint32_t refs[GV];
     if (sg.mm != nullptr) {
-        const uint32_t nb = spec_dense_blocks(sg.mm[0], sg.mm[1], sg.rows, sg.cap);
+        const uint32_t nb = spec_dense_blocks(sg.mm[0], sg.mm[1], sg.rows, sg.cap, sg.anchor != 0);
         if (blockIdx.x >= nb) return;
-        g.dmin = sg.mm[0];
+        g.dmin = sg.anchor ? dense_block_base(sg.mm[0]) : sg.mm[0];
         nblk = nb;
     }
     __shared__ uint32_t d_off[kDenseSub], d_cur[kDenseSub], d_cnt[kDenseSub];
@@ -3472,6 +3591,48 @@
     }
 }
 
+template <typename K>
+__global__ void __launch_bounds__(1024)
+anchor_fold_kernel(long long* mm, unsigned ntiles, const void* __restrict__ akeys, unsigned long long* aflag,
+                   long long* mbox, long long seq, Segment* segs, SegArgs sa, int nseg, BuildCounters* ctr) {
+    __shared__ long long s_mn[16], s_mx[16];
+    if (ctr != nullptr) {
+        if (threadIdx.x < (unsigned)nseg) segs[threadIdx.x] = sa.s[threadIdx.x];
+        if (threadIdx.x == 0) *ctr = BuildCounters{};
+    }
+    long long mn = LLONG_MAX, mx = LLONG_MIN;
+    for (unsigned b = threadIdx.x; b < ntiles; b += blockDim.x) {
+        mn = min(mn, mm[kAnchorHdr + 2 * b]);
+        mx = max(mx, mm[kAnchorHdr + 2 * b + 1]);
+    }
+#pragma unroll
+    for (int d = 32; d >= 1; d >>= 1) {
+        mn = min(mn, (long long)__shfl_xor(mn, d, 64));
+        mx = max(mx, (long long)__shfl_xor(mx, d, 64));
+    }
+    if ((threadIdx.x & 63) == 0) {
+        s_mn[threadIdx.x >> 6] = mn;
+        s_mx[threadIdx.x >> 6] = mx;
+    }
+    __syncthreads();
+    if (threadIdx.x == 0) {
+        for (int w = 1; w < (int)(blockDim.x >> 6); ++w) {
+            mn = min(mn, s_mn[w]);
+            mx = max(mx, s_mx[w]);
+        }
+        const long long ablk = (long long)ld_key<K>(akeys, 0) >> kDenseBlockLog;
+        mm[0] = mn;
+        mm[1] = mx;
+        mm[2] = (mn >> kDenseBlockLog) - ablk + kAnchorBias;
+        *aflag = 0ull;
+        if (mbox != nullptr) {
+            mbox[0] = mn;
+            mbox[1] = mx;
+            __hip_atomic_store(&mbox[2], seq, __ATOMIC_RELEASE, __HIP_MEMORY_SCOPE_SYSTEM);
+        }
+    }
+}
+
 hipError_t launch_key_minmax(int key_bytes, const Segment* h_segs, Segment* d_segs, int nseg, BuildCounters* ctr,
                              int64_t total, int64_t* out, int64_t* mbox, int64_t seq, hipStream_t s) {
     const unsigned grid =
@@ -3506,9 +3667,10 @@
     return g.dense && dense_one_level(g.nchunks) && dense_blocks(g.nchunks) <= (uint32_t)kSlMaxSlices &&
            ftiles <= kFragMaxTiles;
 }
-int64_t frag_build_scratch_bytes(const ChunkGeom& g, int64_t ftiles, int64_t total) {
+int64_t frag_build_scratch_bytes(const ChunkGeom& g, int64_t ftiles, int64_t total, bool anchor) {
     const int64_t nbins = dense_blocks(g.nchunks) + 1;
-    return 2 * ftiles * kSlTile + 2 * ftiles * kSlTile + 2 * ftiles * nbins + 2 * ((ftiles + 63) & ~(int64_t)63) * nbins +
+    const int64_t tbins = anchor ? kSlHistBins : nbins;
+    return 2 * ftiles * kSlTile + 2 * ftiles * kSlTile + 2 * ftiles * tbins + 2 * ((ftiles + 63) & ~(int64_t)63) * nbins +
            16 * total + 6 * 256;
 }
 
@@ -3526,7 +3688,9 @@
 hipError_t launch_build_frag(int key_bytes, const Segment* h_segs, int nseg, const ChunkGeom& g, int64_t ftiles,
                              void* scratch, uint32_t* tile_base, const uint64_t* ids32, uint32_t* dense,
                              uint32_t* dup_rows, BigSeg* big, BuildCounters* ctr, const Segment* d_segs, int64_t total,
-                             bool ids_as_rows, int big_grid, const SpecGeo& spec, hipStream_t s) {
+                             bool ids_as_rows, int big_grid, const SpecGeo& spec, hipStream_t s, const AnchorArgs& aa,
+                             int64_t* mbox, int64_t seq, bool publish) {
+    const bool anchor = spec.mm != nullptr && spec.anchor != 0;
     const uint32_t nblk = dense_blocks(g.nchunks), nbins = nblk + 1;
     constexpr uint32_t GV = kDenseSub << kDenseBlockShift;
     const uint32_t wlog = 31 - __builtin_clz(GV);
@@ -3534,7 +3698,7 @@
     uintptr_t p = a256((uintptr_t)scratch);
     uint16_t* ko = (uint16_t*)p;   p = a256(p + 2 * ftiles * kSlTile);
     uint16_t* rl = (uint16_t*)p;   p = a256(p + 2 * ftiles * kSlTile);
-    uint16_t* toff = (uint16_t*)p; p = a256(p + 2 * ftiles * nbins);
+    uint16_t* toff = (uint16_t*)p; p = a256(p + 2 * ftiles * (anchor ? (uint32_t)kSlHistBins : nbins));
     uint16_t* toffT = (uint16_t*)p; p = a256(p + 2 * ((ftiles + 63) & ~(int64_t)63) * nbins);
     unsigned long long* spill = (unsigned long long*)p;
     int64_t t0 = 0;
@@ -3549,13 +3713,39 @@
                                                                    sg.voff, sg.n, vec, ko, rl, toff, 0, t0,          \
                                                                    sg.row_base, tile_base, nullptr, nullptr, nullptr, \
                                                                    nullptr, spec)
-        if (key_bytes == 8) {
+#define DFP_BLPA(KT, HV)                                                                                        \
+    sl_partition_kernel<KT, HV, kSlTileLog, true><<<(unsigned)nt, kSlThreads, 0, s>>>(                          \
+        0, 0, wlog, 0, sg.keys, sg.valid, sg.voff, sg.n, vec, ko, rl, toff, 0, t0, sg.row_base, tile_base, aa.flag, \
+        reinterpret_cast<unsigned long long*>(aa.part), (uint32_t*)const_cast<void*>(aa.keys), nullptr, spec)
+        if (anchor) {
+            if (key_bytes == 8) {
+                if (sg.valid) DFP_BLPA(int64_t, true); else DFP_BLPA(int64_t, false);
+            } else {
+                if (sg.valid) DFP_BLPA(int32_t, true); else DFP_BLPA(int32_t, false);
+            }
+        } else if (key_bytes == 8) {
             if (sg.valid) DFP_BLP(int64_t, true); else DFP_BLP(int64_t, false);
         } else {
             if (sg.valid) DFP_BLP(int32_t, true); else DFP_BLP(int32_t, false);
         }
 #undef DFP_BLP
+#undef DFP_BLPA
         t0 += nt;
+    }
+    if (anchor) {
+        SegArgs sa{};
+        if (publish) {
+            if (nseg > kArgSegs) return hipErrorInvalidValue;
+            for (int i = 0; i < nseg; ++i) sa.s[i] = h_segs[i];
+        }
+        if (key_bytes == 8)
+            anchor_fold_kernel<int64_t><<<1, 1024, 0, s>>>(aa.part, (unsigned)ftiles, aa.keys, aa.flag,
+                                                           (long long*)mbox, (long long)seq,
+                                                           const_cast<Segment*>(d_segs), sa, nseg, publish ? ctr : nullptr);
+        else
+            anchor_fold_kernel<int32_t><<<1, 1024, 0, s>>>(aa.part, (unsigned)ftiles, aa.keys, aa.flag,
+                                                           (long long*)mbox, (long long)seq,
+                                                           const_cast<Segment*>(d_segs), sa, nseg, publish ? ctr : nullptr);
     }
     sl_toff_transpose_kernel<<<(unsigned)((ftiles + 63) / 64 * ((nblk + kSlTrChunk) / kSlTrChunk)), 256, 0, s>>>(
         toff, nbins, ftiles, toffT, spec);
diff --git a/datafusion-parallelism_amd/csrc/hj_launch.h b/datafusion-parallelism_amd/csrc/hj_launch.h
--- a/datafusion-parallelism_amd/csrc/hj_launch.h
+++ b/datafusion-parallelism_amd/csrc/hj_launch.h
@@ -28,11 +28,13 @@
 int64_t frag_build_tiles(const int64_t* seg_n, int nseg, int tile_log = 14);
 int hashed_build_tile_log();
 bool frag_build_ok(const ChunkGeom& g, int64_t ftiles);
-int64_t frag_build_scratch_bytes(const ChunkGeom& g, int64_t ftiles, int64_t total);
+int64_t frag_build_scratch_bytes(const ChunkGeom& g, int64_t ftiles, int64_t total, bool anchor = false);
 hipError_t launch_build_frag(int key_bytes, const Segment* h_segs, int nseg, const ChunkGeom& g, int64_t ftiles,
                              void* scratch, uint32_t* tile_base, const uint64_t* ids32, uint32_t* dense,
                              uint32_t* dup_rows, BigSeg* big, BuildCounters* ctr, const Segment* d_segs, int64_t total,
-                             bool ids_as_rows, int big_grid, const SpecGeo& spec, hipStream_t s);
+                             bool ids_as_rows, int big_grid, const SpecGeo& spec, hipStream_t s,
+                             const AnchorArgs& aa = AnchorArgs{}, int64_t* mbox = nullptr, int64_t seq = 0,
+                             bool publish = false);
 bool hashed_frag_ok(const ChunkGeom& g, int64_t ftiles);
 int64_t hashed_frag_scratch_bytes(const ChunkGeom& g, int64_t ftiles, int64_t total);
 hipError_t launch_build_hashed_frag(int key_bytes, const Segment* h_segs, int nseg, const ChunkGeom& g, int64_t ftiles,
```

Result: faster. 172,600 Mrows/s (median of 6 runs) (+2.6%).
